# Vi-Sri/CerebralSignalNetworks

Measured on AMD Instinct MI355X. Metric: EEG-segments/sec training (128ch x 500, hidden=768), higher is better.
Workload: dtype bf16

## Files before the change

### cerebralsignalnetworks_amd/cabi.py

```python
import ctypes
import os

import torch

_HERE = os.path.dirname(os.path.abspath(__file__))
LIB_PATH = os.environ.get("CSN_LIB_PATH") or os.path.join(_HERE, "lib", "libcsn_hip.so")

CSN_F32, CSN_BF16 = 0, 1
STATUS_TIMEOUT, STATUS_NONFINITE, STATUS_STALE_SLOT = 1, 2, 4
ABI_VERSION = 6
LSTM_STATE = 0x100
GRAD_OVERWRITE, GRAD_ACCUMULATE = 0, 1

_c_void_p, _c_int, _c_i64, _c_size_t, _c_float = (ctypes.c_void_p, ctypes.c_int, ctypes.c_int64,
                                                  ctypes.c_size_t, ctypes.c_float)


class LstmDesc(ctypes.Structure):
    _fields_ = [("B", ctypes.c_int32), ("T", ctypes.c_int32), ("I", ctypes.c_int32),
                ("H", ctypes.c_int32), ("L", ctypes.c_int32), ("dtype", ctypes.c_int32)]


SIGNATURES = {
    "csn_abi_version": (_c_int, []),
    "csn_last_error": (ctypes.c_char_p, []),
    "csn_target_arch": (ctypes.c_char_p, []),
    "csn_eeg_bandpass_znorm": (_c_int, [_c_void_p, _c_int, _c_int, _c_int, ctypes.POINTER(ctypes.c_double), _c_int,
                                        _c_int, _c_void_p, _c_int, _c_int, _c_void_p]),
    "csn_eeg_filtfilt_scratch_bytes": (_c_size_t, [_c_int, _c_int, _c_int, _c_int]),
    "csn_eeg_filtfilt": (_c_int, [_c_void_p, _c_int, _c_int, _c_int, ctypes.POINTER(ctypes.c_double), _c_int,
                                  _c_void_p, _c_void_p, _c_void_p]),
    "csn_lstm_plan_create": (_c_int, [ctypes.POINTER(LstmDesc), _c_int, ctypes.POINTER(_c_void_p)]),
    "csn_lstm_plan_destroy": (None, [_c_void_p]),
    "csn_lstm_plan_workspace_bytes": (_c_size_t, [_c_void_p]),
    "csn_lstm_plan_path": (_c_int, [_c_void_p]),
    "csn_lstm_plan_dgates_copies": (_c_int, [_c_void_p]),
    "csn_lstm_plan_kernel_name": (ctypes.c_char_p, [_c_void_p, _c_int]),
    "csn_lstm_plan_set_grad_callback": (_c_int, [_c_void_p, _c_void_p, _c_void_p]),
    "csn_lstm_plan_set_grad_mode": (_c_int, [_c_void_p, _c_int]),
    "csn_lstm_plan_set_lengths": (_c_int, [_c_void_p, ctypes.POINTER(ctypes.c_int32)]),
    "csn_lstm_workspace_bytes": (_c_size_t, [ctypes.POINTER(LstmDesc), _c_int]),
    "csn_lstm_forward": (_c_int, [_c_void_p, _c_void_p, _c_i64, _c_i64,
                                  ctypes.POINTER(_c_void_p), ctypes.POINTER(_c_void_p),
                                  ctypes.POINTER(_c_void_p), ctypes.POINTER(_c_void_p),
                                  _c_void_p, _c_void_p,
                                  _c_void_p, _c_void_p, _c_void_p,
                                  _c_void_p, _c_void_p, _c_void_p]),
    "csn_lstm_backward": (_c_int, [_c_void_p, _c_void_p, _c_void_p,
                                   _c_void_p, _c_void_p,
                                   _c_void_p,
                                   ctypes.POINTER(_c_void_p), ctypes.POINTER(_c_void_p),
                                   ctypes.POINTER(_c_void_p), ctypes.POINTER(_c_void_p),
                                   _c_void_p, _c_void_p, _c_void_p, _c_void_p]),
    "csn_lstm_workspace_init": (_c_int, [_c_void_p, _c_void_p, _c_void_p]),
    "csn_lstm_status_clear": (_c_int, [_c_void_p, _c_void_p, _c_void_p]),
    "csn_lstm_status_read": (_c_int, [_c_void_p, _c_void_p, ctypes.POINTER(_c_int)]),
    "csn_lstm_status_raise": (_c_int, [_c_void_p, _c_void_p, _c_void_p]),
    "csn_lstm_profile_enable": (_c_int, [_c_void_p, _c_int]),
    "csn_lstm_profile_read": (_c_int, [_c_void_p, ctypes.POINTER(ctypes.c_double), ctypes.POINTER(_c_int),
                                       ctypes.POINTER(_c_int), ctypes.POINTER(ctypes.c_double), ctypes.POINTER(_c_int),
                                       ctypes.POINTER(_c_int)]),
    "csn_gemm_nt": (_c_int, [_c_void_p, _c_void_p, _c_void_p, _c_void_p, _c_i64, _c_i64, _c_i64,
                             _c_int, _c_int, _c_int, _c_void_p]),
    "csn_gemm_tn_scratch_bytes": (_c_size_t, [_c_i64, _c_i64, _c_i64]),
    "csn_gemm_tn": (_c_int, [_c_void_p, _c_void_p, _c_void_p, _c_i64, _c_i64, _c_i64, _c_int, _c_void_p, _c_void_p]),
    "csn_lstm_cell_forward": (_c_int, [_c_void_p, _c_void_p, _c_void_p, _c_i64, _c_void_p, _c_void_p, _c_void_p,
                                       _c_void_p, _c_int, _c_int, _c_int, _c_void_p]),
    "csn_lstm_cell_backward": (_c_int, [_c_void_p, _c_void_p, _c_void_p, _c_i64, _c_void_p, _c_void_p, _c_void_p,
                                        _c_void_p, _c_void_p, _c_int, _c_int, _c_int, _c_void_p]),
    "csn_cosine_loss_scratch_bytes": (_c_size_t, [_c_int]),
    "csn_cosine_loss": (_c_int, [_c_void_p, _c_void_p, _c_int, _c_int, _c_void_p, _c_void_p, _c_float, _c_void_p, _c_void_p]),
    "csn_rmsprop_step": (_c_int, [_c_void_p, _c_void_p, _c_void_p, _c_i64, _c_float, _c_float, _c_float, _c_void_p]),
    "csn_barlow_offdiag_sqsum": (_c_int, [_c_void_p, _c_int, _c_void_p, _c_void_p]),
    "csn_l2_topk_scratch_bytes": (_c_size_t, [_c_i64, _c_i64]),
    "csn_l2_topk": (_c_int, [_c_void_p, _c_void_p, _c_i64, _c_i64, _c_int, _c_int, _c_void_p, _c_void_p,
                             _c_void_p, _c_void_p]),
}


GRAD_READY_FN = ctypes.CFUNCTYPE(None, ctypes.c_void_p, ctypes.c_int)


class CsnError(RuntimeError):
    pass


_lib = None


def load():
    global _lib
    if _lib is not None:
        return _lib
    if not os.path.exists(LIB_PATH):
        raise CsnError(f"{LIB_PATH} not found: build it with `python -c 'import __graft_entry__ as g; g.build()'` "
                       "(there is no CPU fallback)")
    lib = ctypes.CDLL(LIB_PATH, mode=ctypes.RTLD_LOCAL)
    for name, (res, args) in SIGNATURES.items():
        fn = getattr(lib, name)
        fn.restype, fn.argtypes = res, args
    if lib.csn_abi_version() != ABI_VERSION:
        raise CsnError(f"libcsn_hip.so ABI {lib.csn_abi_version()} != binding ABI {ABI_VERSION}")
    _lib = lib
    return lib


def _check(rc):
    if rc != 0:
        raise CsnError(f"libcsn_hip status {rc}: {load().csn_last_error().decode()}")


def _ptr(t):
    return None if t is None else ctypes.c_void_p(t.data_ptr())


def _stream():
    return ctypes.c_void_p(torch.cuda.current_stream().cuda_stream)


def _dt(dtype):
    if dtype in (torch.float32, "f32", "float32", CSN_F32):
        return CSN_F32
    if dtype in (torch.bfloat16, "bf16", "bfloat16", CSN_BF16):
        return CSN_BF16
    raise CsnError(f"unsupported dtype {dtype}")


def torch_dtype(code):
    return torch.bfloat16 if code == CSN_BF16 else torch.float32


def _need_cuda(*ts):
    for t in ts:
        if t is not None and not t.is_cuda:
            raise CsnError("libcsn_hip needs device tensors (no CPU fallback)")


def eeg_bandpass_znorm(x_bct, sos, ddof=0, out_dtype=torch.float32, time_major=False):
    import numpy as np
    _need_cuda(x_bct)
    x = x_bct.contiguous()
    if x.dtype != torch.float32:
        raise CsnError("eeg_bandpass_znorm expects float32 input")
    B, C, T = x.shape
    sos = np.ascontiguousarray(np.asarray(sos, dtype=np.float64).reshape(-1, 6)) if sos is not None else np.zeros((0, 6))
    y = torch.empty((T, B, C) if time_major else (B, T, C), dtype=out_dtype, device=x.device)
    with torch.cuda.device(x.device):
        _check(load().csn_eeg_bandpass_znorm(_ptr(x), B, C, T, sos.ctypes.data_as(ctypes.POINTER(ctypes.c_double)),
                                             sos.shape[0], int(ddof), _ptr(y), _dt(out_dtype), int(time_major), _stream()))
    return y


def eeg_filtfilt(x_stc, sos):
    import numpy as np
    _need_cuda(x_stc)
    x = x_stc.float().contiguous()
    S, T, C = x.shape
    sos = np.ascontiguousarray(np.asarray(sos, dtype=np.float64).reshape(-1, 6))
    lib = load()
    scratch = torch.empty(max(1, lib.csn_eeg_filtfilt_scratch_bytes(S, T, C, sos.shape[0])), dtype=torch.uint8,
                          device=x.device)
    y = torch.empty_like(x)
    with torch.cuda.device(x.device):
        _check(lib.csn_eeg_filtfilt(_ptr(x), S, T, C, sos.ctypes.data_as(ctypes.POINTER(ctypes.c_double)), sos.shape[0],
                                    _ptr(y), _ptr(scratch), _stream()))
    return y


def gemm_nt(a, bt, bias=None, out_dtype=torch.float32, out=None, accumulate=False):
    _need_cuda(a, bt)
    a, bt = a.contiguous(), bt.contiguous()
    M, K = a.shape
    N = bt.shape[0]
    assert bt.shape[1] == K and a.dtype == bt.dtype
    c = out if out is not None else torch.empty((M, N), dtype=out_dtype, device=a.device)
    _check(load().csn_gemm_nt(_ptr(a), _ptr(bt), _ptr(bias), _ptr(c), M, N, K, _dt(a.dtype), _dt(c.dtype),
                              int(accumulate), _stream()))
    return c


def gemm_tn(a_km, b_kn):
    _need_cuda(a_km, b_kn)
    a, b = a_km.contiguous(), b_kn.contiguous()
    K, M = a.shape
    N = b.shape[1]
    assert b.shape[0] == K and a.dtype == b.dtype
    lib = load()
    scratch = torch.empty(max(1, lib.csn_gemm_tn_scratch_bytes(M, N, K)), dtype=torch.uint8, device=a.device)
    c = torch.empty((M, N), dtype=torch.float32, device=a.device)
    _check(lib.csn_gemm_tn(_ptr(a), _ptr(b), _ptr(c), M, N, K, _dt(a.dtype), _ptr(scratch), _stream()))
    return c


def lstm_cell_forward(h_prev, w_hh, xproj, c_prev, want_gates=True):
    _need_cuda(w_hh, xproj)
    B, G = xproj.shape
    H = G // 4
    dt = w_hh.dtype
    gates = torch.empty((B, G), dtype=dt, device=xproj.device) if want_gates else None
    c_out = torch.empty((B, H), dtype=torch.float32, device=xproj.device)
    h_out = torch.empty((B, H), dtype=dt, device=xproj.device)
    _check(load().csn_lstm_cell_forward(_ptr(h_prev), _ptr(w_hh), _ptr(xproj), G, _ptr(c_prev), _ptr(gates),
                                        _ptr(c_out), _ptr(h_out), B, H, _dt(dt), _stream()))
    return h_out, c_out, gates


def lstm_cell_backward(dgates_next, w_hh_t, dy, gates, c, c_prev, dc_carry):
    _need_cuda(gates, c, dc_carry)
    B, G = gates.shape
    H = G // 4
    out = torch.empty_like(gates)
    _check(load().csn_lstm_cell_backward(_ptr(dgates_next), _ptr(w_hh_t), _ptr(dy), H, _ptr(gates), _ptr(c),
                                         _ptr(c_prev), _ptr(dc_carry), _ptr(out), B, H, _dt(gates.dtype), _stream()))
    return out


def _ptr_array(tensors):
    arr = (ctypes.c_void_p * len(tensors))()
    for i, t in enumerate(tensors):
        arr[i] = t.data_ptr()
    return arr


class LstmPlan:

    def __init__(self, B, T, I, H, L, dtype, device, training=True, state=False):
        self.desc = LstmDesc(B, T, I, H, L, _dt(dtype))
        self.training = bool(training)
        self.state = bool(state)
        self.device = torch.device(device)
        lib = load()
        handle = _c_void_p()
        with torch.cuda.device(self.device):
            _check(lib.csn_lstm_plan_create(ctypes.byref(self.desc), int(self.training) | (LSTM_STATE if self.state else 0),
                                            ctypes.byref(handle)))
        self._plan = handle
        nbytes = lib.csn_lstm_plan_workspace_bytes(self._plan)
        self.workspace = torch.empty(nbytes + 256, dtype=torch.uint8, device=self.device)
        off = (-self.workspace.data_ptr()) % 256
        self._ws_ptr = ctypes.c_void_p(self.workspace.data_ptr() + off)
        self.busy = False
        with torch.cuda.device(self.device):
            _check(lib.csn_lstm_workspace_init(self._plan, self._ws_ptr, _stream()))

    def __del__(self):
        plan, self._plan = getattr(self, "_plan", None), None
        if plan and _lib is not None:
            _lib.csn_lstm_plan_destroy(plan)

    def key(self):
        d = self.desc
        return (d.B, d.T, d.I, d.H, d.L, d.dtype, self.training) + ((True,) if self.state else ())

    def path(self):
        return load().csn_lstm_plan_path(self._plan)

    def kernel_names(self):
        lib = load()
        return tuple((lib.csn_lstm_plan_kernel_name(self._plan, k) or b"").decode() for k in (0, 1))

    def set_grad_callback(self, fn):
        if getattr(self, "_grad_cb_fn", None) is fn and (fn is None or getattr(self, "_grad_cb", None) is not None):
            return
        self._grad_cb_fn = fn
        self._grad_cb = GRAD_READY_FN(lambda _user, layer: fn(int(layer))) if fn is not None else None
        _check(load().csn_lstm_plan_set_grad_callback(self._plan, ctypes.cast(self._grad_cb, _c_void_p) if fn is not None
                                                      else None, None))

    def set_grad_mode(self, accumulate):
        _check(load().csn_lstm_plan_set_grad_mode(self._plan, GRAD_ACCUMULATE if accumulate else GRAD_OVERWRITE))

    def set_lengths(self, lengths):
        if lengths is None:
            _check(load().csn_lstm_plan_set_lengths(self._plan, None))
            return
        vals = [int(v) for v in (lengths.tolist() if isinstance(lengths, torch.Tensor) else lengths)]
        if len(vals) != self.desc.B:
            raise CsnError(f"LSTM lengths: {len(vals)} entries for a batch of {self.desc.B}")
        _check(load().csn_lstm_plan_set_lengths(self._plan, (ctypes.c_int32 * len(vals))(*vals)))

    def dgates_copies(self):
        return load().csn_lstm_plan_dgates_copies(self._plan)

    def forward(self, x_bti, w_ih, w_hh, b_ih, b_hh, want_all=False, h0=None, c0=None, want_state=False):
        d = self.desc
        _need_cuda(x_bti)
        if x_bti.dtype != torch.float32 or x_bti.stride(2) != 1:
            x_bti = x_bti.float().contiguous()
        assert x_bti.shape == (d.B, d.T, d.I), (tuple(x_bti.shape), (d.B, d.T, d.I))
        y_last = torch.empty((d.B, d.H), dtype=torch.float32, device=x_bti.device)
        y_all = torch.empty((d.B, d.T, d.H), dtype=torch.float32, device=x_bti.device) if want_all else None
        ws = [[p.detach() for p in group] for group in (w_ih, w_hh, b_ih, b_hh)]
        for group in ws:
            for p in group:
                assert p.dtype == torch.float32 and p.is_contiguous() and p.is_cuda
        h0, c0 = self._state_in(h0), self._state_in(c0)
        h_n = torch.empty((d.L, d.B, d.H), dtype=torch.float32, device=x_bti.device) if want_state else None
        c_n = torch.empty((d.L, d.B, d.H), dtype=torch.float32, device=x_bti.device) if want_state else None
        with torch.cuda.device(self.device):
            _check(load().csn_lstm_forward(self._plan, _ptr(x_bti), x_bti.stride(0), x_bti.stride(1),
                                           _ptr_array(ws[0]), _ptr_array(ws[1]), _ptr_array(ws[2]), _ptr_array(ws[3]),
                                           _ptr(h0), _ptr(c0), self._ws_ptr, _ptr(y_last), _ptr(y_all),
                                           _ptr(h_n), _ptr(c_n), _stream()))
        if want_state:
            return y_last, y_all, h_n, c_n
        return y_last, y_all

    def _state_in(self, t):
        if t is None:
            return None
        d = self.desc
        t = t.detach()
        if tuple(t.shape) != (d.L, d.B, d.H):
            raise CsnError(f"LSTM state must be [L, B, H] = {[d.L, d.B, d.H]}, got {list(t.shape)}")
        return t.to(device=self.device, dtype=torch.float32).contiguous()

    def backward(self, dy_last, dy_all, grads, dx=None, dh_n=None, dc_n=None, dh0=None, dc0=None):
        if dy_last is not None:
            dy_last = dy_last.float().contiguous()
        if dy_all is not None:
            dy_all = dy_all.float().contiguous()
        dh_n, dc_n = self._state_in(dh_n), self._state_in(dc_n)
        for out in (dh0, dc0):
            if out is not None:
                assert out.dtype == torch.float32 and out.is_contiguous() and out.shape == (self.desc.L, self.desc.B,
                                                                                            self.desc.H)
        with torch.cuda.device(self.device):
            _check(load().csn_lstm_backward(self._plan, _ptr(dy_last), _ptr(dy_all), _ptr(dh_n), _ptr(dc_n), self._ws_ptr,
                                            _ptr_array(grads[0]), _ptr_array(grads[1]), _ptr_array(grads[2]),
                                            _ptr_array(grads[3]), _ptr(dx), _ptr(dh0), _ptr(dc0), _stream()))

    def clear_status(self):
        with torch.cuda.device(self.device):
            _check(load().csn_lstm_status_clear(self._plan, self._ws_ptr, _stream()))

    def inject_timeout(self):
        with torch.cuda.device(self.device):
            _check(load().csn_lstm_status_raise(self._plan, self._ws_ptr, _stream()))

    def status(self, clear=False):
        out = _c_int(0)
        _check(load().csn_lstm_status_read(self._plan, self._ws_ptr, ctypes.byref(out)))
        if clear and out.value != 0:
            self.clear_status()
        return out.value

    def profile_enable(self, on=True):
        _check(load().csn_lstm_profile_enable(self._plan, int(on)))

    def profile_read(self):
        fm, bm = ctypes.c_double(), ctypes.c_double()
        fl, fc, bl, bc = _c_int(), _c_int(), _c_int(), _c_int()
        _check(load().csn_lstm_profile_read(self._plan, ctypes.byref(fm), ctypes.byref(fl), ctypes.byref(fc),
                                            ctypes.byref(bm), ctypes.byref(bl), ctypes.byref(bc)))
        return dict(fwd_ms=fm.value, fwd_launches=fl.value, fwd_cells=fc.value,
                    bwd_ms=bm.value, bwd_launches=bl.value, bwd_cells=bc.value)


def cosine_loss(student, teacher, want_grad=True, grad_scale=1.0):
    _need_cuda(student, teacher)
    s, t = student.float().contiguous(), teacher.float().contiguous()
    B, D = s.shape
    loss = torch.empty(1, dtype=torch.float32, device=s.device)
    ds = torch.empty_like(s) if want_grad else None
    lib = load()
    scratch = torch.empty(lib.csn_cosine_loss_scratch_bytes(B) // 8, dtype=torch.float64, device=s.device)
    with torch.cuda.device(s.device):
        _check(lib.csn_cosine_loss(_ptr(s), _ptr(t), B, D, _ptr(loss), _ptr(ds), float(grad_scale), _ptr(scratch), _stream()))
    return loss, ds


def rmsprop_step(params_flat, grads_flat, square_avg_flat, lr, alpha=0.99, eps=1e-8):
    _need_cuda(params_flat, grads_flat, square_avg_flat)
    n = params_flat.numel()
    assert grads_flat.numel() == n and square_avg_flat.numel() == n
    assert params_flat.dtype == grads_flat.dtype == square_avg_flat.dtype == torch.float32
    with torch.cuda.device(params_flat.device):
        _check(load().csn_rmsprop_step(_ptr(params_flat), _ptr(grads_flat), _ptr(square_avg_flat), n, float(lr), float(alpha),
                                       float(eps), _stream()))


def barlow_offdiag_sqsum(c):
    _need_cuda(c)
    if c.dim() != 2 or c.shape[0] != c.shape[1]:
        raise CsnError(f"barlow_offdiag_sqsum expects a square matrix, got shape {tuple(c.shape)}")
    c = c.float().contiguous()
    out = torch.empty(2, dtype=torch.float32, device=c.device)
    with torch.cuda.device(c.device):
        _check(load().csn_barlow_offdiag_sqsum(_ptr(c), c.shape[0], _ptr(out), _stream()))
    return out


def l2_topk(gallery, query, k):
    _need_cuda(gallery, query)
    g, q = gallery.float().contiguous(), query.float().contiguous()
    Ng, D = g.shape
    Nq = q.shape[0]
    lib = load()
    scratch = torch.empty(lib.csn_l2_topk_scratch_bytes(Ng, Nq), dtype=torch.uint8, device=g.device)
    idx = torch.empty((Nq, k), dtype=torch.int64, device=g.device)
    dist = torch.empty((Nq, k), dtype=torch.float32, device=g.device)
    _check(lib.csn_l2_topk(_ptr(g), _ptr(q), Ng, Nq, D, k, _ptr(idx), _ptr(dist), _ptr(scratch), _stream()))
    return dist, idx
```

### cerebralsignalnetworks_amd/csrc/csn_common.h

```cpp
#pragma once
#include <hip/hip_runtime.h>
#include <stdint.h>
#include <stdio.h>
#include <stdlib.h>
#include <atomic>
#include <string>

#include "../../include/csn_hip.h"

namespace csn {

typedef __bf16 bf16_t;
typedef __attribute__((ext_vector_type(8))) __bf16 bf16x8;
typedef __attribute__((ext_vector_type(4))) __bf16 bf16x4;
typedef __attribute__((ext_vector_type(4))) float f32x4;
typedef __attribute__((ext_vector_type(4))) short s16x4;

void set_error(const std::string& msg);
int fail(int status, const char* fmt, ...);

#define CSN_HIP_CHECK(expr)                                                              \
  do {                                                                                   \
    hipError_t _e = (expr);                                                              \
    if (_e != hipSuccess)                                                                \
      return ::csn::fail(CSN_ERR_HIP, "%s failed: %s (%s:%d)", #expr, hipGetErrorString(_e), \
                         __FILE__, __LINE__);                                            \
  } while (0)

#define CSN_LAUNCH_CHECK()                                                               \
  do {                                                                                   \
    hipError_t _e = hipGetLastError();                                                   \
    if (_e != hipSuccess)                                                                \
      return ::csn::fail(CSN_ERR_HIP, "kernel launch failed: %s (%s:%d)",                \
                         hipGetErrorString(_e), __FILE__, __LINE__);                     \
  } while (0)

#define CSN_REQUIRE(cond, ...)                                                           \
  do {                                                                                   \
    if (!(cond)) return ::csn::fail(CSN_ERR_INVALID_ARGUMENT, __VA_ARGS__);              \
  } while (0)

struct Options {
  bool cell_v1, no_persist, no_persist_bwd, persist_streams, no_xcd_local, no_rotate, no_fuse_x, no_beside,
      no_side_stream, gemm_slot, fwd_ksplit, fwd_nsplit, fwd_flags, bwd_flags, dpoll_no_hint, fwd_hint, gemm_no_dma, gemm_no_256, gemm_generic, gemm_lds64, tn_no_tr, tn_no_stagger, filter_v1, tags_no_rearm, gemm_no_192;
  int chunk;
  int tn_stages;
  int fwd_nk;
};
static inline Options options_from_env() {
  auto on = [](const char* name) { return getenv(name) != nullptr; };
  auto num = [](const char* name, int dflt) {
    const char* e = getenv(name);
    return e ? atoi(e) : dflt;
  };
  Options o{};
  o.cell_v1 = on("CSN_CELL_V1");
  o.no_persist = on("CSN_NO_PERSIST");
  o.no_persist_bwd = on("CSN_NO_PERSIST_BWD");
  o.persist_streams = on("CSN_PERSIST_STREAMS");
  o.no_xcd_local = on("CSN_NO_XCD_LOCAL");
  o.no_rotate = on("CSN_NO_ROTATE");
  o.no_fuse_x = on("CSN_NO_FUSE_X");
  o.no_beside = on("CSN_NO_BESIDE");
  o.no_side_stream = on("CSN_NO_SIDE_STREAM");
  o.gemm_slot = on("CSN_GEMM_SLOT");
  o.fwd_ksplit = on("CSN_FWD_KSPLIT");
  o.fwd_nsplit = on("CSN_FWD_NSPLIT");
  o.fwd_flags = on("CSN_FWD_FLAGS");
  o.bwd_flags = on("CSN_BWD_FLAGS");
  o.dpoll_no_hint = on("CSN_DPOLL_NO_HINT");
  o.fwd_hint = on("CSN_FWD_HINT");
  o.tn_no_stagger = on("CSN_TN_NO_STAGGER");
  o.gemm_no_dma = on("CSN_GEMM_NO_DMA");
  o.gemm_no_256 = on("CSN_GEMM_NO_256");
  o.gemm_no_192 = on("CSN_GEMM_NO_192");
  o.gemm_generic = on("CSN_GEMM_GENERIC");
  o.gemm_lds64 = on("CSN_GEMM_LDS64");
  o.tn_no_tr = on("CSN_TN_NO_TR");
  o.filter_v1 = on("CSN_FILTER_V1");
#ifdef CSN_SLAB_TAGS
  o.tags_no_rearm = on("CSN_TAGS_NO_REARM");
#endif
  o.chunk = num("CSN_LSTM_CHUNK", 32);
  if (o.chunk < 1) o.chunk = 1;
  o.tn_stages = num("CSN_TN_STAGES", 4);
  o.fwd_nk = num("CSN_FWD_NK", 1);
  return o;
}

static inline hipStream_t as_stream(csnStream_t s) { return reinterpret_cast<hipStream_t>(s); }
template <auto Kernel>
static int ensure_dyn_lds(int bytes) {
  static std::atomic<unsigned> done{0u};
  int dev = 0;
  CSN_HIP_CHECK(hipGetDevice(&dev));
  const unsigned bit = 1u << (dev & 31);
  if ((done.load(std::memory_order_acquire) & bit) == 0u) {
    CSN_HIP_CHECK(hipFuncSetAttribute(reinterpret_cast<const void*>(Kernel), hipFuncAttributeMaxDynamicSharedMemorySize, bytes));
    done.fetch_or(bit, std::memory_order_release);
  }
  return CSN_OK;
}

static inline size_t align_up(size_t v, size_t a) { return (v + a - 1) / a * a; }
static inline size_t dtype_size(int dtype) { return dtype == CSN_BF16 ? 2 : 4; }

__device__ __forceinline__ float to_f32(float v) { return v; }
__device__ __forceinline__ float to_f32(bf16_t v) { return (float)v; }
template <typename T> __device__ __forceinline__ T from_f32(float v);
template <> __device__ __forceinline__ float from_f32<float>(float v) { return v; }
template <> __device__ __forceinline__ bf16_t from_f32<bf16_t>(float v) { return (bf16_t)v; }

__device__ __forceinline__ float sigmoid_f32(float x) { return 1.0f / (1.0f + expf(-x)); }
__device__ __forceinline__ float tanh_f32(float x) { return tanhf(x); }

struct CellFwdOne {
  const void* h_prev; const void* w_hh; const float* xproj; int64_t xproj_ld; const float* c_prev;
  void* gates_out; float* c_out; void* h_out;
};
struct CellFwdBatch { CellFwdOne p[4]; };
struct CellBwdOne {
  const void* dg_next; const void* w_hh_t; const float* dy; int64_t dy_ld; const void* gates; const float* c;
  const float* c_prev; float* dc_carry; void* dg_out;
};
struct CellBwdBatch { CellBwdOne p[4]; };
struct CellMask {
  const int* lengths;
  int t[4];
};
struct CellNoMask {};
template <bool MASK> struct CellMaskArg { typedef CellNoMask type; };
template <> struct CellMaskArg<true> { typedef CellMask type; };
int launch_cell_fwd_batch(const CellFwdBatch& b, int np, int B, int H, int dtype, hipStream_t st);
int launch_cell_bwd_batch(const CellBwdBatch& b, int np, int B, int H, int dtype, hipStream_t st,
                          const CellMask* mask = nullptr);

int launch_cast_strided(const float* src, int64_t s0, int64_t s1, int64_t n0, int64_t n1, int64_t n2,
                        void* dst, int dtype, hipStream_t st);
int launch_transpose_cast(const float* src, int64_t R, int64_t C, void* dst, int dtype, hipStream_t st);
int launch_cast(const float* src, void* dst, int64_t n, int dtype, hipStream_t st);
int launch_upcast(const void* src, int dtype, float* dst, int64_t n, hipStream_t st);
int launch_add_vec(const float* a, const float* b, float* out, int64_t n, hipStream_t st);
int launch_reduce_slabs(const float* slabs, int64_t stride, int S, float* out, float* out2, int64_t n, int accumulate,
                        hipStream_t st);
size_t colsum_scratch_bytes(int64_t N);
int launch_colsum(const void* X, int64_t R, int64_t N, int dtype, float* out, float* out2, int accumulate, void* scratch,
                  hipStream_t st);
int colsum_chunks();
int launch_colsum_partial(const void* X, int64_t R, int64_t N, int dtype, void* scratch, hipStream_t st);
int launch_gemm_nt_beside(const void* A, const void* Bt, const float* bias, float* C, int64_t M, int64_t N, int64_t K,
                          int max_wgs, hipStream_t st);
int launch_gemm_tn_slabs(const void* A, const void* B, float* slabs, int64_t M, int64_t N, int64_t K, int dtype,
                         hipStream_t st, int* S_out, float* colsum, int* colsum_done, const Options& opt);
int gemm_nt(const void* A, const void* Bt, const float* bias, void* C, int64_t M, int64_t N, int64_t K, int dtype,
            int out_dtype, int accumulate, hipStream_t st, const Options& opt);
size_t gemm_tn_scratch_bytes(int64_t M, int64_t N, int64_t K, const Options& opt);

}
```

### cerebralsignalnetworks_amd/csrc/lstm.hip

```cpp
#include <algorithm>
#include <cstring>
#include <vector>

#include "csn_common.h"
#include "lstm_cell_blk.h"
#include "lstm_cell_common.h"
#include "lstm_f32_persist.h"

namespace csn {

int launch_cell_fwd(const void* h_prev, const void* w_hh, const float* xproj, int64_t xproj_ld, const float* c_prev,
                    void* gates_out, float* c_out, void* h_out, int B, int H, int dtype, hipStream_t st);
int launch_cell_bwd(const void* dg_next, const void* w_hh_t, const float* dy, int64_t dy_ld, const void* gates,
                    const float* c, const float* c_prev, float* dc_carry, void* dg_out, int B, int H, int dtype,
                    hipStream_t st);

struct LayerWs {
  size_t wih, whh, whht, wiht, whh_blk, whht_blk, bias, xproj, gates, c_all, h_all, dgates, dx, dc_carry, hblk[2],
      dgblk[2], h_blk_all, counters, dg_blk_all, bflags;
};
struct WsLayout {
  LayerWs layer[8];
  size_t x_c, x_blk, wih0_blk, dy_tm, tn_scratch, colsum, status, agree, agree_b, zeros_bh, f32_bias_part, total;
  size_t zero_fwd, zero_fwd_bytes, zero_bwd, zero_bwd_bytes;
  bool fuse_x;
  bool il, persist, persist_bwd;
  bool fwd_ns;
  bool f32_persist;
};

static bool whole_chip() {
  int dev = 0, cus = 0;
  if (hipGetDevice(&dev) != hipSuccess) return false;
  return hipDeviceGetAttribute(&cus, hipDeviceAttributeMultiprocessorCount, dev) == hipSuccess && cus >= 256;
}

static WsLayout make_layout(const csnLstmDesc& d, int training, const Options& opt) {
  WsLayout w{};
  w.il = cell_blk_supported(d.H, d.dtype, opt);
  const bool slabs_fit = ((size_t)d.T + 1) * (((size_t)d.B + 63) / 64 * 64) * (size_t)d.H * 8 < ((size_t)1 << 32);
  w.fwd_ns = w.il && fwd_ns_supported(d.B, d.H, d.dtype, opt) && d.L <= 4;
  w.persist = w.fwd_ns || (w.il && slabs_fit && fwd_persist_supported(d.B, d.H, d.dtype, opt) && d.L <= 4);
  w.persist_bwd = w.persist && slabs_fit && training && bwd_persist_supported(d.B, d.H, d.dtype, opt);
  size_t off = 0;
  const size_t es = dtype_size(d.dtype);
  auto take = [&](size_t bytes) {
    size_t o = off;
    off += align_up(bytes, 256);
    return o;
  };
  const size_t TB = (size_t)d.T * d.B, H = d.H, G = 4 * (size_t)d.H;
  const size_t Bpad = ((size_t)d.B + 63) / 64 * 64;
  size_t tn_bytes = 0;
  for (int l = 0; l < d.L; ++l) {
    const size_t I = l == 0 ? d.I : d.H;
    LayerWs& L = w.layer[l];
    L.wih = take(G * I * es);
    L.wiht = take(G * I * es);
    L.bias = take(G * 4);
    if (w.il) {
      L.whh_blk = take(G * H * 2);
      L.whht_blk = take(G * H * 2);
      L.hblk[0] = take(Bpad * H * 2);
      L.hblk[1] = take(Bpad * H * 2);
      if (w.persist) L.h_blk_all = take(((size_t)(d.T < 3 ? 3 : d.T) + 1) * Bpad * H * 2);
    } else {
      L.whh = take(G * H * es);
      L.whht = take(G * H * es);
    }
    L.xproj = take(TB * G * 4);
    L.gates = take(TB * G * es);
    L.c_all = take((TB + d.B) * H * 4);
    L.h_all = take((TB + d.B) * H * es);
    if (training) {
      L.dgates = take(TB * G * es);
      L.dx = take(TB * I * 4);
      if (!w.persist_bwd) L.dc_carry = take((size_t)d.B * H * 4);
      if (w.il) {
        L.dgblk[0] = take(Bpad * G * 2);
        L.dgblk[1] = take(Bpad * G * 2);
      }
      if (w.persist_bwd) L.dg_blk_all = take((size_t)(d.T < 4 ? 4 : d.T) * Bpad * G * 2);
    }
    size_t a = gemm_tn_scratch_bytes(G, I, TB, opt), b = gemm_tn_scratch_bytes(G, H, TB, opt);
    if (a > tn_bytes) tn_bytes = a;
    if (b > tn_bytes) tn_bytes = b;
  }
  w.x_c = take(TB * d.I * es);
  w.status = take(256);
  w.fuse_x = w.persist && !opt.no_fuse_x &&
             (w.fwd_ns ? d.I == 128 : (d.I % 32 == 0 && d.I <= 128 && d.H != 512));
  if (w.fuse_x) {
    w.x_blk = take((size_t)d.T * Bpad * d.I * 2);
    w.wih0_blk = take(G * d.I * 2);
  }
  if (w.persist_bwd) w.zeros_bh = take((size_t)d.B * H * 4);
  w.f32_persist = !w.il && d.dtype == CSN_F32 && !opt.no_persist && !opt.cell_v1 && f32_persist_supported(d.B, d.H) && whole_chip();
  if (w.f32_persist) {
    const size_t MTt = Bpad / 64;
    w.zero_fwd = off;
    for (int l = 0; l < d.L; ++l) w.layer[l].counters = take(((size_t)d.T + 1) * MTt * kF32FlagLine * 4);
    w.zero_fwd_bytes = off - w.zero_fwd;
    for (int l = 0; l < d.L; ++l) w.layer[l].h_blk_all = take(((size_t)d.T + 1) * Bpad * H * 4);
    if (training) {
      for (int l = 0; l < d.L; ++l) w.layer[l].dg_blk_all = take((size_t)d.T * Bpad * G * 4);
      w.zeros_bh = take((size_t)d.B * H * 4);
      w.f32_bias_part = take(MTt * 4 * G * 4);
      w.zero_bwd = off;
      for (int l = 0; l < d.L; ++l) w.layer[l].bflags = take((size_t)d.T * MTt * kF32FlagLine * 4);
      w.zero_bwd_bytes = off - w.zero_bwd;
    }
  }
  if (w.persist) {
    w.zero_fwd = off;
    for (int l = 0; l < d.L; ++l) w.layer[l].counters = take(((size_t)d.T + 1) * (Bpad / 64) * 4 * kPersistFlagLine * 4);
    w.agree = take(((size_t)d.T + 8) * 8 * sizeof(unsigned long long));
    w.zero_fwd_bytes = off - w.zero_fwd;
  }
  if (w.persist_bwd) {
    w.zero_bwd = off;
    for (int l = 0; l < d.L; ++l) {
      w.layer[l].dc_carry = take((size_t)d.B * H * 4);
      w.layer[l].bflags = take((size_t)d.T * (Bpad / 64) * kPersistFlagLine * 4);
    }
    w.agree_b = take(((size_t)d.T + 8) * 8 * sizeof(unsigned long long));
    w.zero_bwd_bytes = off - w.zero_bwd;
  }
  if (training) {
    w.dy_tm = take(TB * H * 4);
    w.tn_scratch = take(tn_bytes);
    w.colsum = take(colsum_scratch_bytes(G));
  }
  w.total = off;
  return w;
}

static int check_desc(const char* fn, const csnLstmDesc* d) {
  CSN_REQUIRE(d != nullptr, "%s: null descriptor", fn);
  CSN_REQUIRE(d->B > 0 && d->T > 0 && d->I > 0 && d->H > 0, "%s: bad shape B=%d T=%d I=%d H=%d", fn, d->B, d->T,
              d->I, d->H);
  CSN_REQUIRE(d->L >= 1 && d->L <= 8, "%s: L=%d outside 1..8", fn, d->L);
  CSN_REQUIRE(d->H % 32 == 0, "%s: H=%d must be a multiple of 32", fn, d->H);
  CSN_REQUIRE(d->dtype == CSN_F32 || d->dtype == CSN_BF16, "%s: bad dtype %d", fn, d->dtype);
  return CSN_OK;
}

template <typename T>
__global__ void gather_y_all_kernel(const T* __restrict__ h_all, float* __restrict__ y, int B, int Tn, int H) {
  const int64_t total = (int64_t)B * Tn * H;
  const int64_t stride = (int64_t)gridDim.x * blockDim.x;
  for (int64_t i = (int64_t)blockIdx.x * blockDim.x + threadIdx.x; i < total; i += stride) {
    const int64_t h = i % H, r = i / H, t = r % Tn, b = r / Tn;
    y[i] = to_f32(h_all[((t + 1) * B + b) * (int64_t)H + h]);
  }
}

__global__ void bt_to_tb_kernel(const float* __restrict__ src, float* __restrict__ dst, int B, int Tn, int H) {
  const int64_t total = (int64_t)B * Tn * H;
  const int64_t stride = (int64_t)gridDim.x * blockDim.x;
  for (int64_t i = (int64_t)blockIdx.x * blockDim.x + threadIdx.x; i < total; i += stride) {
    const int64_t h = i % H, r = i / H, b = r % B, t = r / B;
    dst[i] = src[(b * Tn + t) * (int64_t)H + h];
  }
}

__global__ void tb_to_bt_kernel(const float* __restrict__ src, float* __restrict__ dst, int B, int Tn, int H) {
  const int64_t total = (int64_t)B * Tn * H;
  const int64_t stride = (int64_t)gridDim.x * blockDim.x;
  for (int64_t i = (int64_t)blockIdx.x * blockDim.x + threadIdx.x; i < total; i += stride) {
    const int64_t h = i % H, r = i / H, t = r % Tn, b = r / Tn;
    dst[i] = src[(t * B + b) * (int64_t)H + h];
  }
}

__global__ void add_rows_kernel(const float* __restrict__ src, float* __restrict__ dst, int64_t n) {
  const int64_t stride = (int64_t)gridDim.x * blockDim.x;
  for (int64_t i = (int64_t)blockIdx.x * blockDim.x + threadIdx.x; i < n; i += stride) dst[i] += src[i];
}

template <typename T>
__global__ void mask_tm_kernel(T* __restrict__ buf, const int* __restrict__ len, int B, int Tn, int W) {
  const int64_t total = (int64_t)B * Tn * W;
  const int64_t stride = (int64_t)gridDim.x * blockDim.x;
  for (int64_t i = (int64_t)blockIdx.x * blockDim.x + threadIdx.x; i < total; i += stride) {
    const int64_t r = i / W, b = r % B, t = r / B;
    if (t >= len[b]) buf[i] = from_f32<T>(0.f);
  }
}
__global__ void mask_x_blk_kernel(bf16_t* __restrict__ x_blk, const int* __restrict__ len, int B, int64_t Bpad, int Tn, int I) {
  const int64_t per_t = Bpad * I / 8, kblocks = I >> 5;
  const int64_t stride = (int64_t)gridDim.x * blockDim.x;
  for (int64_t ci = (int64_t)blockIdx.x * blockDim.x + threadIdx.x; ci < per_t * Tn; ci += stride) {
    const int64_t t = ci / per_t, c = ci % per_t, blk = c >> 6, lane = c & 63;
    const int64_t r = (blk / kblocks) * 16 + (lane & 15);
    if (r < B && t >= len[r]) *reinterpret_cast<uint4*>(x_blk + ci * 8) = make_uint4(0u, 0u, 0u, 0u);
  }
}
template <typename T>
__global__ void gather_state_kernel(const T* __restrict__ all, const int* __restrict__ len, float* __restrict__ out, int B, int H) {
  const int64_t total = (int64_t)B * H;
  const int64_t stride = (int64_t)gridDim.x * blockDim.x;
  for (int64_t i = (int64_t)blockIdx.x * blockDim.x + threadIdx.x; i < total; i += stride) {
    const int64_t b = i / H;
    out[i] = to_f32(all[(int64_t)len[b] * B * H + i]);
  }
}
template <typename T>
__global__ void gather_y_all_len_kernel(const T* __restrict__ h_all, float* __restrict__ y, const int* __restrict__ len, int B, int Tn, int H) {
  const int64_t total = (int64_t)B * Tn * H;
  const int64_t stride = (int64_t)gridDim.x * blockDim.x;
  for (int64_t i = (int64_t)blockIdx.x * blockDim.x + threadIdx.x; i < total; i += stride) {
    const int64_t h = i % H, r = i / H, t = r % Tn, b = r / Tn;
    y[i] = t < len[b] ? to_f32(h_all[((t + 1) * B + b) * (int64_t)H + h]) : 0.f;
  }
}
__global__ void bt_to_tb_len_kernel(const float* __restrict__ src, float* __restrict__ dst, const int* __restrict__ len, int B, int Tn, int Te, int H) {
  const int64_t total = (int64_t)B * Te * H;
  const int64_t stride = (int64_t)gridDim.x * blockDim.x;
  for (int64_t i = (int64_t)blockIdx.x * blockDim.x + threadIdx.x; i < total; i += stride) {
    const int64_t h = i % H, r = i / H, b = r % B, t = r / B;
    dst[i] = (src != nullptr && t < len[b]) ? src[(b * Tn + t) * (int64_t)H + h] : 0.f;
  }
}
__global__ void add_at_end_kernel(const float* __restrict__ src, float* __restrict__ dst_tm, const int* __restrict__ len, int t_lo, int t_hi, int B, int H) {
  const int64_t total = (int64_t)B * H;
  const int64_t stride = (int64_t)gridDim.x * blockDim.x;
  for (int64_t i = (int64_t)blockIdx.x * blockDim.x + threadIdx.x; i < total; i += stride) {
    const int t = len[i / H] - 1;
    if (t >= t_lo && t <= t_hi) dst_tm[(int64_t)t * B * H + i] += src[i];
  }
}
__global__ void add_rows_len0_kernel(const float* __restrict__ src, float* __restrict__ dst, const int* __restrict__ len, int B, int H) {
  const int64_t total = (int64_t)B * H;
  const int64_t stride = (int64_t)gridDim.x * blockDim.x;
  for (int64_t i = (int64_t)blockIdx.x * blockDim.x + threadIdx.x; i < total; i += stride)
    if (len[i / H] == 0) dst[i] += src[i];
}
__global__ void tb_to_bt_len_kernel(const float* __restrict__ src, float* __restrict__ dst, int B, int Tn, int Te, int H) {
  const int64_t total = (int64_t)B * Tn * H;
  const int64_t stride = (int64_t)gridDim.x * blockDim.x;
  for (int64_t i = (int64_t)blockIdx.x * blockDim.x + threadIdx.x; i < total; i += stride) {
    const int64_t h = i % H, r = i / H, t = r % Tn, b = r / Tn;
    dst[i] = t < Te ? src[(t * B + b) * (int64_t)H + h] : 0.f;
  }
}

template <typename T, bool BLK>
__global__ void __launch_bounds__(256) lstm_dh0_kernel(const T* __restrict__ dg, const T* __restrict__ wt, int B, int H,
                                                       float* __restrict__ out) {
  __shared__ float As[32][33];
  __shared__ float Ws[32][65];
  const int64_t G = 4 * (int64_t)H;
  const int tx = threadIdx.x & 15, ty = threadIdx.x >> 4;
  const int b0 = blockIdx.y * 32, j0 = blockIdx.x * 64;
  float acc[2][4] = {{0.f, 0.f, 0.f, 0.f}, {0.f, 0.f, 0.f, 0.f}};
  for (int64_t k0 = 0; k0 < G; k0 += 32) {
    for (int i = threadIdx.x; i < 32 * 32; i += 256) {
      const int r = i >> 5, k = i & 31;
      As[r][k] = b0 + r < B ? to_f32(dg[(int64_t)(b0 + r) * G + k0 + k]) : 0.f;
    }
    for (int i = threadIdx.x; i < 64 * 32; i += 256) {
      const int j = i >> 5, k = i & 31;
      float v = 0.f;
      if (j0 + j < H) v = to_f32(wt[BLK ? blk_offset(j0 + j, k0 + k, G) : (int64_t)(j0 + j) * G + k0 + k]);
      Ws[k][j] = v;
    }
    __syncthreads();
#pragma unroll 8
    for (int k = 0; k < 32; ++k) {
      const float a0 = As[ty][k], a1 = As[ty + 16][k];
#pragma unroll
      for (int c = 0; c < 4; ++c) {
        const float wv = Ws[k][tx + 16 * c];
        acc[0][c] = fmaf(a0, wv, acc[0][c]);
        acc[1][c] = fmaf(a1, wv, acc[1][c]);
      }
    }
    __syncthreads();
  }
#pragma unroll
  for (int r = 0; r < 2; ++r)
#pragma unroll
    for (int c = 0; c < 4; ++c) {
      const int b = b0 + ty + 16 * r, j = j0 + tx + 16 * c;
      if (b < B && j < H) out[(int64_t)b * H + j] = acc[r][c];
    }
}

__global__ void sum_rows_kernel(const float* __restrict__ part, int P, int64_t n, float* out, float* out2, int accumulate) {
  const int64_t i = (int64_t)blockIdx.x * blockDim.x + threadIdx.x;
  if (i >= n) return;
  float s = 0.f;
  for (int p = 0; p < P; ++p) s += part[(int64_t)p * n + i];
  out[i] = accumulate ? out[i] + s : s;
  out2[i] = accumulate ? out2[i] + s : s;
}

static inline unsigned grid_for(int64_t n) {
  int64_t g = (n + 255) / 256;
  return (unsigned)(g < 1 ? 1 : (g > 2048 ? 2048 : g));
}

struct SideCtx {
  hipStream_t side = nullptr;
  hipStream_t layer[8] = {nullptr};
  std::vector<hipEvent_t> events;
  size_t next = 0;
};

static int side_ctx(SideCtx& c) {
  if (c.side == nullptr) {
    CSN_HIP_CHECK(hipStreamCreateWithFlags(&c.side, hipStreamNonBlocking));
    for (int l = 1; l < 8; ++l) CSN_HIP_CHECK(hipStreamCreateWithFlags(&c.layer[l], hipStreamNonBlocking));
  }
  c.next = 0;
  return CSN_OK;
}
static int next_event(SideCtx* c, hipEvent_t* ev) {
  if (c->next == c->events.size()) {
    hipEvent_t e;
    CSN_HIP_CHECK(hipEventCreateWithFlags(&e, hipEventDisableTiming));
    c->events.push_back(e);
  }
  *ev = c->events[c->next++];
  return CSN_OK;
}
static int hand_off(SideCtx* c, hipStream_t from, hipStream_t to) {
  hipEvent_t ev;
  if (int rc = next_event(c, &ev)) return rc;
  CSN_HIP_CHECK(hipEventRecord(ev, from));
  CSN_HIP_CHECK(hipStreamWaitEvent(to, ev, 0));
  return CSN_OK;
}

struct Prof {
  bool on = false;
  hipEvent_t ev[4] = {nullptr, nullptr, nullptr, nullptr};
  int launches[2] = {0, 0}, cells[2] = {0, 0};
  bool have[2] = {false, false};
  std::vector<hipEvent_t> pair[2];
  size_t pairs_used[2] = {0, 0};
};
static int prof_mark(Prof& g_prof, int which, hipStream_t st) {
  if (!g_prof.on) return CSN_OK;
  if ((which & 1) == 0) g_prof.pairs_used[which >> 1] = 0;
  if (g_prof.ev[which] == nullptr) CSN_HIP_CHECK(hipEventCreate(&g_prof.ev[which]));
  CSN_HIP_CHECK(hipEventRecord(g_prof.ev[which], st));
  return CSN_OK;
}

static int prof_pair(Prof& g_prof, int k, bool end, hipStream_t st) {
  if (!g_prof.on) return CSN_OK;
  const size_t i = 2 * g_prof.pairs_used[k] + (end ? 1 : 0);
  while (g_prof.pair[k].size() <= i) {
    hipEvent_t e;
    CSN_HIP_CHECK(hipEventCreate(&e));
    g_prof.pair[k].push_back(e);
  }
  CSN_HIP_CHECK(hipEventRecord(g_prof.pair[k][i], st));
  if (end) ++g_prof.pairs_used[k];
  return CSN_OK;
}

}

struct csnLstmPlan {
  csnLstmDesc d;
  int training;
  int state;
  bool state_seen = false;
  int device;
  csn::Options opt;
  csn::WsLayout w;
  csn::SideCtx sc;
  csn::Prof prof;
  int dgates_copies = 0;
  csnGradReadyFn grad_cb = nullptr;
  void* grad_cb_user = nullptr;
  int grad_accumulate = 0;
  std::vector<int32_t> lengths;
  int t_eff = 0;
  int T_full = 0;
  const int* dlen = nullptr;
  int32_t* len_dev = nullptr;
  int32_t* len_pin = nullptr;
  hipEvent_t len_ev = nullptr;
  void grads_ready(int layer) const {
    if (grad_cb != nullptr) grad_cb(grad_cb_user, layer);
  }
};

using namespace csn;
typedef csnLstmPlan Plan;

extern "C" int csn_lstm_plan_create(const csnLstmDesc* d, int training, csnLstmPlan** out) {
  if (int rc = check_desc("csn_lstm_plan_create", d)) return rc;
  CSN_REQUIRE(out != nullptr, "csn_lstm_plan_create: null output pointer");
  Plan* P = new Plan();
  P->d = *d;
  P->state = (training & CSN_LSTM_STATE) != 0;
  P->training = (training & ~CSN_LSTM_STATE) != 0;
  if (hipGetDevice(&P->device) != hipSuccess) {
    delete P;
    return fail(CSN_ERR_HIP, "csn_lstm_plan_create: hipGetDevice failed");
  }
  P->opt = options_from_env();
  if (P->state && d->dtype == CSN_F32) P->opt.no_persist = true;
  {
    const unsigned long long Bp = ((unsigned long long)d->B + 63) / 64 * 64;
    const unsigned long long per_step = std::max({(unsigned long long)d->B * d->H * 16ull, Bp * (unsigned long long)d->I * 2ull, Bp * (unsigned long long)d->H * 2ull});
    const unsigned long long cmax = ((1ull << 32) - 1ull) / per_step;
    if (cmax >= 3 && (unsigned long long)P->opt.chunk > cmax - 2) P->opt.chunk = (int)(cmax - 2);
  }
  P->w = make_layout(*d, P->training, P->opt);
  P->T_full = d->T;
  *out = P;
  return CSN_OK;
}

extern "C" void csn_lstm_plan_destroy(csnLstmPlan* P) {
  if (P == nullptr) return;
  int cur = 0;
  const bool switched = hipGetDevice(&cur) == hipSuccess && cur != P->device && hipSetDevice(P->device) == hipSuccess;
  for (hipEvent_t e : P->sc.events) (void)hipEventDestroy(e);
  if (P->sc.side) (void)hipStreamDestroy(P->sc.side);
  for (int l = 1; l < 8; ++l)
    if (P->sc.layer[l]) (void)hipStreamDestroy(P->sc.layer[l]);
  for (int i = 0; i < 4; ++i)
    if (P->prof.ev[i]) (void)hipEventDestroy(P->prof.ev[i]);
  for (int k = 0; k < 2; ++k)
    for (hipEvent_t e : P->prof.pair[k]) (void)hipEventDestroy(e);
  if (P->len_ev) (void)hipEventDestroy(P->len_ev);
  if (P->len_pin) (void)hipHostFree(P->len_pin);
  if (P->len_dev) (void)hipFree(P->len_dev);
  if (switched) (void)hipSetDevice(cur);
  delete P;
}

extern "C" size_t csn_lstm_plan_workspace_bytes(const csnLstmPlan* P) { return P ? P->w.total : 0; }

extern "C" int csn_lstm_plan_path(const csnLstmPlan* P) {
  if (P == nullptr) return -1;
  return P->w.f32_persist ? 4 : (P->w.persist_bwd ? 3 : (P->w.persist ? 2 : (P->w.il ? 1 : 0)));
}

extern "C" int csn_lstm_plan_dgates_copies(const csnLstmPlan* P) { return P == nullptr ? -1 : P->dgates_copies; }

static bool bwd_grouped(const csnLstmPlan* P) {
  if (!P->w.persist_bwd) return false;
  const int MTg = (P->d.B + 63) / 64, nchg = (P->d.T + P->opt.chunk - 1) / P->opt.chunk;
  const int slots = P->d.L < nchg ? P->d.L : nchg;
  return slots <= 4 && slots * MTg <= 8 && !P->opt.persist_streams;
}

extern "C" const char* csn_lstm_plan_kernel_name(const csnLstmPlan* P, int which) {
  if (P == nullptr) return nullptr;
  const bool ks = (P->d.dtype == CSN_F32 ? P->d.H % 128 == 0 : P->d.H % 256 == 0);
  if (P->w.f32_persist) return which == 0 ? "lstm_fwd_f32_persist_kernel" : (which == 1 ? "lstm_bwd_f32_persist_kernel" : nullptr);
  if (which == 0) {
    if (P->w.fwd_ns) return "lstm_fwd_ns_kernel";
    if (P->w.persist) return "lstm_fwd_persist_kernel";
    if (P->w.il) return "lstm_cell_fwd_il_kernel";
    return ks ? "lstm_cell_fwd_ks_kernel" : "lstm_cell_fwd_kernel";
  }
  if (which == 1) {
    if (bwd_grouped(P)) return "lstm_bwd_persist_kernel";
    if (P->w.il) return "lstm_cell_bwd_il_kernel";
    return ks ? "lstm_cell_bwd_ks_kernel" : "lstm_cell_bwd_kernel";
  }
  return nullptr;
}

extern "C" int csn_lstm_plan_set_grad_callback(csnLstmPlan* P, csnGradReadyFn fn, void* user) {
  CSN_REQUIRE(P != nullptr, "csn_lstm_plan_set_grad_callback: null plan");
  P->grad_cb = fn;
  P->grad_cb_user = fn ? user : nullptr;
  return CSN_OK;
}

extern "C" int csn_lstm_plan_set_grad_mode(csnLstmPlan* P, int mode) {
  CSN_REQUIRE(P != nullptr, "csn_lstm_plan_set_grad_mode: null plan");
  CSN_REQUIRE(mode == CSN_GRAD_OVERWRITE || mode == CSN_GRAD_ACCUMULATE, "csn_lstm_plan_set_grad_mode: unknown mode %d", mode);
  P->grad_accumulate = mode == CSN_GRAD_ACCUMULATE;
  return CSN_OK;
}

extern "C" int csn_lstm_plan_set_lengths(csnLstmPlan* P, const int32_t* lengths) {
  CSN_REQUIRE(P != nullptr, "csn_lstm_plan_set_lengths: null plan");
  CSN_REQUIRE(P->state, "csn_lstm_plan_set_lengths: the plan was created without CSN_LSTM_STATE");
  if (lengths == nullptr) {
    P->lengths.clear();
    P->t_eff = 0;
    return CSN_OK;
  }
  int longest = 0;
  for (int b = 0; b < P->d.B; ++b) {
    CSN_REQUIRE(lengths[b] >= 0 && lengths[b] <= P->d.T, "csn_lstm_plan_set_lengths: lengths[%d] = %d outside [0, %d]", b,
                (int)lengths[b], P->d.T);
    longest = std::max(longest, (int)lengths[b]);
  }
  P->lengths.assign(lengths, lengths + P->d.B);
  P->t_eff = longest;
  return CSN_OK;
}

struct EffectiveT {
  csnLstmDesc& d;
  const int T;
  EffectiveT(csnLstmDesc& d_, int Te) : d(d_), T(d_.T) { d.T = Te; }
  ~EffectiveT() { d.T = T; }
};
static int upload_lengths(csnLstmPlan* P, hipStream_t st) {
  P->dlen = nullptr;
  if (P->lengths.empty()) return CSN_OK;
  const size_t bytes = (size_t)P->d.B * 4;
  if (P->len_pin == nullptr) {
    CSN_HIP_CHECK(hipMalloc((void**)&P->len_dev, bytes));
    CSN_HIP_CHECK(hipHostMalloc((void**)&P->len_pin, bytes, hipHostMallocDefault));
    CSN_HIP_CHECK(hipEventCreateWithFlags(&P->len_ev, hipEventDisableTiming));
  } else {
    CSN_HIP_CHECK(hipEventSynchronize(P->len_ev));
  }
  memcpy(P->len_pin, P->lengths.data(), bytes);
  CSN_HIP_CHECK(hipMemcpyAsync(P->len_dev, P->len_pin, bytes, hipMemcpyHostToDevice, st));
  CSN_HIP_CHECK(hipEventRecord(P->len_ev, st));
  P->dlen = P->len_dev;
  return CSN_OK;
}
static int emit_dx(const csnLstmPlan& P, const float* dx_tm, float* dx, int64_t I, hipStream_t st) {
  const int B = P.d.B, T = P.d.T;
  if (P.dlen != nullptr) tb_to_bt_len_kernel<<<csn::grid_for((int64_t)P.T_full * B * I), 256, 0, st>>>(dx_tm, dx, B, P.T_full, T, (int)I);
  else csn::tb_to_bt_kernel<<<csn::grid_for((int64_t)T * B * I), 256, 0, st>>>(dx_tm, dx, B, T, (int)I);
  CSN_LAUNCH_CHECK();
  return CSN_OK;
}
static int add_dh_n_rows(const csnLstmPlan& P, const float* dh_below, float* dx_tm, int t_lo, int t_hi, hipStream_t st) {
  const int B = P.d.B, H = P.d.H, T = P.d.T;
  if (P.dlen != nullptr) {
    add_at_end_kernel<<<csn::grid_for((int64_t)B * H), 256, 0, st>>>(dh_below, dx_tm, P.dlen, t_lo, t_hi, B, H);
  } else {
    if (t_hi != T - 1) return CSN_OK;
    csn::add_rows_kernel<<<csn::grid_for((int64_t)B * H), 256, 0, st>>>(dh_below, dx_tm + (size_t)(T - 1) * B * H, (int64_t)B * H);
  }
  CSN_LAUNCH_CHECK();
  return CSN_OK;
}

extern "C" int csn_lstm_profile_enable(csnLstmPlan* P, int on) {
  CSN_REQUIRE(P != nullptr, "csn_lstm_profile_enable: null plan");
  P->prof.on = on != 0;
  P->prof.have[0] = P->prof.have[1] = false;
  return CSN_OK;
}

extern "C" int csn_lstm_profile_read(csnLstmPlan* P, double* fwd_ms, int* fwd_launches, int* fwd_cells, double* bwd_ms,
                                     int* bwd_launches, int* bwd_cells) {
  CSN_REQUIRE(P && fwd_ms && fwd_launches && fwd_cells && bwd_ms && bwd_launches && bwd_cells,
              "csn_lstm_profile_read: null pointer");
  Prof& g_prof = P->prof;
  *fwd_ms = *bwd_ms = 0.0;
  *fwd_launches = *fwd_cells = *bwd_launches = *bwd_cells = 0;
  for (int k = 0; k < 2; ++k) {
    if (!g_prof.have[k]) continue;
    float ms = 0.f;
    CSN_HIP_CHECK(hipEventSynchronize(g_prof.ev[2 * k + 1]));
    if (g_prof.pairs_used[k] > 0) {
      for (size_t i = 0; i < g_prof.pairs_used[k]; ++i) {
        float one = 0.f;
        CSN_HIP_CHECK(hipEventElapsedTime(&one, g_prof.pair[k][2 * i], g_prof.pair[k][2 * i + 1]));
        ms += one;
      }
    } else {
      CSN_HIP_CHECK(hipEventElapsedTime(&ms, g_prof.ev[2 * k], g_prof.ev[2 * k + 1]));
    }
    (k == 0 ? *fwd_ms : *bwd_ms) = ms;
    (k == 0 ? *fwd_launches : *bwd_launches) = g_prof.launches[k];
    (k == 0 ? *fwd_cells : *bwd_cells) = g_prof.cells[k];
  }
  return CSN_OK;
}

extern "C" int csn_lstm_workspace_init(const csnLstmPlan* P, void* workspace, csnStream_t stream) {
  CSN_REQUIRE(P && workspace, "csn_lstm_workspace_init: null pointer");
  CSN_REQUIRE((reinterpret_cast<uintptr_t>(workspace) & 255) == 0, "csn_lstm_workspace_init: workspace must be 256-B aligned");
  hipStream_t st = as_stream(stream);
  char* ws = (char*)workspace;
  const WsLayout& w = P->w;
  const size_t es = dtype_size(P->d.dtype);
  CSN_HIP_CHECK(hipMemsetAsync(ws + w.status, 0, 256, st));
  for (int l = 0; l < P->d.L; ++l) {
    CSN_HIP_CHECK(hipMemsetAsync(ws + w.layer[l].h_all, 0, (size_t)P->d.B * P->d.H * es, st));
    CSN_HIP_CHECK(hipMemsetAsync(ws + w.layer[l].c_all, 0, (size_t)P->d.B * P->d.H * 4, st));
  }
  if (w.persist_bwd || (w.f32_persist && P->training))
    CSN_HIP_CHECK(hipMemsetAsync(ws + w.zeros_bh, 0, (size_t)P->d.B * P->d.H * 4, st));
  return CSN_OK;
}

extern "C" int csn_lstm_status_clear(const csnLstmPlan* P, void* workspace, csnStream_t stream) {
// ... 363 lines not shown
      CSN_HIP_CHECK(hipMemsetAsync(ws + L.c_all, 0, (size_t)B * H * 4, st));
      if (h0) {
        if ((rc = launch_blockify_x(h0 + (size_t)l * B * H, H, 0, B, 1, H, ws + L.hblk[0], st))) return rc;
        if ((rc = launch_cast(h0 + (size_t)l * B * H, ws + L.h_all, (int64_t)B * H, CSN_BF16, st))) return rc;
      }
      if (c0)
        CSN_HIP_CHECK(hipMemcpyAsync(ws + L.c_all, c0 + (size_t)l * B * H, (size_t)B * H * 4, hipMemcpyDeviceToDevice, st));
    }
  }
  if (w.fuse_x) {
    job(kPrepBlockifyX, x, nullptr, ws + w.x_blk, B, T, d->I, xsb, xst, (int64_t)Bpad, 0, 0, (int64_t)T * Bpad * d->I / 8);
    job(kPrepBlockify, w_ih[0], nullptr, ws + w.wih0_blk, G, d->I, 0, d->I, 1, H, 1, 0, G * d->I / 8);
  }
  if (prep_rc != CSN_OK) return prep_rc;
  if ((rc = launch_prep_multi(pa, st))) return rc;
  if ((rc = mask_x(P, ws, st))) return rc;
  if (!w.fuse_x) {
    if ((rc = gemm_nt(ws + w.x_c, ws + w.layer[0].wih, (const float*)(ws + w.layer[0].bias), ws + w.layer[0].xproj,
                          TB, G, d->I, CSN_BF16, CSN_F32, 0, st, P.opt)))
      return rc;
  }
  if (w.persist) return forward_persist(P, ws, h0, c0, training, st, sc, side);
  if (NL > 1 && (rc = hand_off(sc, st, side))) return rc;

  const int nch = (T + Cz - 1) / Cz;
  std::vector<hipEvent_t> xproj_ready((size_t)NL * nch, nullptr);
  const int D = T + lag * (NL - 1);
  int n_launch = 0, n_cells = 0;
  if ((rc = prof_mark(g_prof, 0, st))) return rc;
  for (int dg = 0; dg < D; ++dg) {
    CellFwdArgs a{};
    a.B = B;
    a.H = H;
    int np = 0;
    for (int l = 0; l < NL; ++l) {
      const int t = dg - lag * l;
      if (t < 0 || t >= T) continue;
      const LayerWs& L = w.layer[l];
      if (np == 4) {
        if ((rc = launch_cell_fwd_il(a, np, st, P.opt.fwd_nk))) return rc;
        ++n_launch;
        n_cells += np;
        np = 0;
      }
      if (l > 0 && t % Cz == 0) CSN_HIP_CHECK(hipStreamWaitEvent(st, xproj_ready[(size_t)l * nch + t / Cz], 0));
      CellFwdProb& P = a.p[np++];
      P.h_prev_blk = (t == 0 && !h0) ? nullptr : (const bf16_t*)(ws + L.hblk[t & 1]);
      P.w_blk = (const bf16_t*)(ws + L.whh_blk);
      P.xproj = (const float*)(ws + L.xproj) + (size_t)t * B * G;
      P.c_prev = (t == 0 && !c0) ? nullptr : (const float*)(ws + L.c_all) + (size_t)t * B * H;
      P.gates_out = training ? (bf16_t*)(ws + L.gates) + (size_t)t * B * G : nullptr;
      P.c_out = (float*)(ws + L.c_all) + (size_t)(t + 1) * B * H;
      P.h_out = (bf16_t*)(ws + L.h_all) + (size_t)(t + 1) * B * H;
      P.h_out_blk = (bf16_t*)(ws + L.hblk[(t + 1) & 1]);
    }
    if (np == 0) continue;
    if ((rc = launch_cell_fwd_il(a, np, st, P.opt.fwd_nk))) return rc;
    ++n_launch;
    n_cells += np;
    for (int l = 0; l + 1 < NL; ++l) {
      const int t = dg - lag * l;
      if (t < 0 || t >= T) continue;
      if ((t + 1) % Cz != 0 && t != T - 1) continue;
      const int c = t / Cz, t0 = c * Cz, nsteps = t - t0 + 1;
      if ((rc = hand_off(sc, st, side))) return rc;
      const LayerWs& Ln = w.layer[l + 1];
      rc = gemm_nt((const bf16_t*)(ws + w.layer[l].h_all) + (size_t)(t0 + 1) * B * H, ws + Ln.wih,
                       (const float*)(ws + Ln.bias), (float*)(ws + Ln.xproj) + (size_t)t0 * B * G,
                       (int64_t)nsteps * B, G, H, CSN_BF16, CSN_F32, 0, side, P.opt);
      if (rc) return rc;
      hipEvent_t ev;
      if ((rc = next_event(sc, &ev))) return rc;
      CSN_HIP_CHECK(hipEventRecord(ev, side));
      xproj_ready[(size_t)(l + 1) * nch + c] = ev;
    }
  }
  if ((rc = prof_mark(g_prof, 1, st))) return rc;
  g_prof.launches[0] = n_launch;
  g_prof.cells[0] = n_cells;
  g_prof.have[0] = g_prof.on;
  return CSN_OK;
}

static int forward_persist(Plan& P, char* ws, const float* h0, const float* c0, int training, hipStream_t st, SideCtx* sc,
                           hipStream_t side) {
  const csnLstmDesc* d = &P.d;
  const WsLayout& w = P.w;
  Prof& g_prof = P.prof;
  const int B = d->B, T = d->T, H = d->H, NL = d->L;
  const int64_t G = 4 * (int64_t)H;
  const int Bpad = (B + 63) / 64 * 64, MT = Bpad / 64;
  const int Cz = P.opt.chunk;
  const int nch = (T + Cz - 1) / Cz;
  int rc;
  CSN_HIP_CHECK(hipMemsetAsync(ws + w.zero_fwd, 0, w.zero_fwd_bytes, st));
  auto fill_slot = [&](PersistFwdSlot& S, int l, int c) {
    const LayerWs& L = w.layer[l];
    S.w_blk = (const bf16_t*)(ws + L.whh_blk);
    S.xproj = (const float*)(ws + L.xproj);
    S.gates = training ? (bf16_t*)(ws + L.gates) : nullptr;
    S.c_all = (float*)(ws + L.c_all);
    S.h_all = (bf16_t*)(ws + L.h_all);
    S.h_blk_all = (bf16_t*)(ws + L.h_blk_all);
    S.flags = (unsigned*)(ws + L.counters);
    S.x_blk = nullptr;
    S.wih_blk = nullptr;
    S.bias = nullptr;
    S.I = 0;
    if (l == 0 && w.fuse_x) {
      S.x_blk = (const bf16_t*)(ws + w.x_blk);
      S.wih_blk = (const bf16_t*)(ws + w.wih0_blk);
      S.bias = (const float*)(ws + L.bias);
      S.I = d->I;
    }
    S.t0 = c * Cz;
    S.nsteps = (S.t0 + Cz <= T) ? Cz : T - S.t0;
  };
  auto xproj_gemm = [&](int l, int c, hipStream_t on) {
    const LayerWs& L = w.layer[l];
    const LayerWs& Ln = w.layer[l + 1];
    const int t0 = c * Cz, nsteps = (t0 + Cz <= T) ? Cz : T - t0;
    return gemm_nt((const bf16_t*)(ws + L.h_all) + (size_t)(t0 + 1) * B * H, ws + Ln.wih,
                       (const float*)(ws + Ln.bias), (float*)(ws + Ln.xproj) + (size_t)t0 * B * G,
                       (int64_t)nsteps * B, G, H, CSN_BF16, CSN_F32, 0, on, P.opt);
  };
  PersistFwdArgs a{};
  a.error_flag = (unsigned*)(ws + w.status);
  a.B = B; a.H = H; a.T = T; a.Bpad = Bpad; a.MT = MT;
  a.rotate = !P.opt.no_rotate;
  a.data_polls = (!w.fwd_ns && !P.opt.fwd_flags) ? (P.opt.fwd_hint && !P.opt.dpoll_no_hint ? 1 : 2) : 0;
#ifdef CSN_SLAB_TAGS
  if (a.data_polls && P.opt.tags_no_rearm) a.data_polls |= 4;
#endif
  if (a.data_polls)
    for (int l = 0; l < NL; ++l)
      CSN_HIP_CHECK(hipMemsetAsync(ws + w.layer[l].h_blk_all, 0xff, (size_t)4 * Bpad * H * 2, st));
  a.state = (h0 || c0) ? 1 : 0;
  if (a.state) P.state_seen = true;
  for (int l = 0; l < NL && P.state_seen; ++l) {
    const LayerWs& L = w.layer[l];
    if (h0) {
      if ((rc = launch_blockify_x(h0 + (size_t)l * B * H, H, 0, B, 1, H, ws + L.h_blk_all, st))) return rc;
      if ((rc = launch_cast(h0 + (size_t)l * B * H, ws + L.h_all, (int64_t)B * H, CSN_BF16, st))) return rc;
    } else {
      if (a.state) CSN_HIP_CHECK(hipMemsetAsync(ws + L.h_blk_all, 0, (size_t)Bpad * H * 2, st));
      CSN_HIP_CHECK(hipMemsetAsync(ws + L.h_all, 0, (size_t)B * H * 2, st));
    }
    if (c0)
      CSN_HIP_CHECK(hipMemcpyAsync(ws + L.c_all, c0 + (size_t)l * B * H, (size_t)B * H * 4, hipMemcpyDeviceToDevice, st));
    else
      CSN_HIP_CHECK(hipMemsetAsync(ws + L.c_all, 0, (size_t)B * H * 4, st));
  }
  int n_launch = 0;

  const int max_slots = NL < nch ? NL : nch;
  const int fwd_slices = w.fwd_ns ? fwd_ns_slices(H) : fwd_persist_slices(H);
  auto launch_fwd = [&](const PersistFwdArgs& args, hipStream_t on) {
    return w.fwd_ns ? launch_fwd_ns(args, on) : launch_fwd_persist(args, on);
  };
  const bool grouped = max_slots <= 4 && max_slots * MT <= 8 && fwd_slices <= 32 &&
                       !P.opt.persist_streams;
  if (grouped) {
    const int ndiag = nch + NL - 1;
    const bool try_local = !P.opt.no_xcd_local;
    if ((rc = prof_mark(g_prof, 0, st))) return rc;
    for (int dg = 0; dg < ndiag; ++dg) {
      int lay[4], chk[4], ns = 0;
      for (int l = 0; l < NL; ++l) {
        const int c = dg - l;
        if (c < 0 || c >= nch) continue;
        lay[ns] = l;
        chk[ns] = c;
        fill_slot(a.slot[ns], l, c);
        ++ns;
      }
      a.nslots = ns;
      a.xcd_groups = 1;
      a.agree = try_local ? (unsigned long long*)(ws + w.agree) + (size_t)dg * 8 : nullptr;
      if ((rc = prof_pair(g_prof, 0, false, st))) return rc;
      if ((rc = launch_fwd(a, st))) return rc;
      if ((rc = prof_pair(g_prof, 0, true, st))) return rc;
      ++n_launch;
      for (int i = 0; i < ns; ++i)
        if (lay[i] + 1 < NL && (rc = xproj_gemm(lay[i], chk[i], st))) return rc;
    }
    if ((rc = prof_mark(g_prof, 1, st))) return rc;
    g_prof.launches[0] = n_launch;
    g_prof.cells[0] = T * NL;
    g_prof.have[0] = g_prof.on;
    return CSN_OK;
  }

  if (NL * fwd_slices * MT > 256) side = st;
  hipStream_t ls[8];
  ls[0] = st;
  for (int l = 1; l < NL; ++l) {
    ls[l] = (side == st) ? st : sc->layer[l];
    if (ls[l] != st && (rc = hand_off(sc, st, ls[l]))) return rc;
  }
  if (side != st && (rc = hand_off(sc, st, side))) return rc;
  const bool gemm_slot = P.opt.gemm_slot;
  if ((rc = prof_mark(g_prof, 0, st))) return rc;
  a.nslots = 1;
  a.xcd_groups = 0;
  a.agree = nullptr;
  for (int c = 0; c < nch; ++c) {
    for (int l = 0; l < NL; ++l) {
      fill_slot(a.slot[0], l, c);
      if ((rc = launch_fwd(a, ls[l]))) return rc;
      ++n_launch;
      if (l + 1 < NL) {
        if ((rc = hand_off(sc, ls[l], side))) return rc;
        if ((rc = xproj_gemm(l, c, side))) return rc;
        if (side != ls[l + 1] && (rc = hand_off(sc, side, ls[l + 1]))) return rc;
        if (gemm_slot && side != ls[l] && (rc = hand_off(sc, side, ls[l]))) return rc;
      }
    }
  }
  for (int l = 1; l < NL; ++l)
    if (ls[l] != st && (rc = hand_off(sc, ls[l], st))) return rc;
  if (side != st && (rc = hand_off(sc, side, st))) return rc;
  if ((rc = prof_mark(g_prof, 1, st))) return rc;
  g_prof.launches[0] = n_launch;
  g_prof.cells[0] = T * NL;
  g_prof.have[0] = g_prof.on;
  return CSN_OK;
}

static int backward_persist(Plan& P, char* ws, const float* dy_last, const float* dy_tm, const float* dh_n,
                            const float* dc_n, float* const* dw_ih, float* const* dw_hh, float* const* db_ih,
                            float* const* db_hh, float* dx, hipStream_t st);

static int backward_il(Plan& P, char* ws, const float* dy_last, const float* dy_tm, const float* dh_n, const float* dc_n,
                       float* const* dw_ih, float* const* dw_hh, float* const* db_ih, float* const* db_hh, float* dx,
                       csnStream_t stream) {
  const csnLstmDesc* d = &P.d;
  const WsLayout& w = P.w;
  Prof& g_prof = P.prof;
  hipStream_t st = as_stream(stream);
  if (bwd_grouped(&P)) return backward_persist(P, ws, dy_last, dy_tm, dh_n, dc_n, dw_ih, dw_hh, db_ih, db_hh, dx, st);
  SideCtx* sc = &P.sc;
  int rc;
  if ((rc = side_ctx(P.sc))) return rc;
  hipStream_t side = P.opt.no_side_stream ? st : sc->side;
  const int B = d->B, T = d->T, H = d->H, NL = d->L;
  const int64_t G = 4 * (int64_t)H, TB = (int64_t)T * B;
  const size_t Bpad = ((size_t)B + 63) / 64 * 64;
  const int Cz = P.opt.chunk, lag = 2 * Cz;
  const int nch = (T + Cz - 1) / Cz;
  const bool state = P.state != 0;

  for (int l = 0; l < NL; ++l) {
    const LayerWs& L = w.layer[l];
    if (dc_n)
      CSN_HIP_CHECK(hipMemcpyAsync(ws + L.dc_carry, dc_n + (size_t)l * B * H, (size_t)B * H * 4, hipMemcpyDeviceToDevice, st));
    else
      CSN_HIP_CHECK(hipMemsetAsync(ws + L.dc_carry, 0, (size_t)B * H * 4, st));
    CSN_HIP_CHECK(hipMemsetAsync(ws + L.dgblk[0], 0, Bpad * G * 2, st));
    CSN_HIP_CHECK(hipMemsetAsync(ws + L.dgblk[1], 0, Bpad * G * 2, st));
  }
  if ((rc = hand_off(sc, st, side))) return rc;

  auto weight_grads = [&](int l) -> int {
    const LayerWs& L = w.layer[l];
    const int64_t I = l == 0 ? d->I : H;
    const void* inp = l == 0 ? (const void*)(ws + w.x_c)
                             : (const void*)((const bf16_t*)(ws + w.layer[l - 1].h_all) + (size_t)B * H);
    float* slabs = (float*)(ws + w.tn_scratch);
    const int acc = P.grad_accumulate;
    int S = 1, r;
    int cs_done = 0, S_cs = 1;
    if ((r = launch_gemm_tn_slabs(ws + L.dgates, ws + L.h_all, slabs, G, H, TB, CSN_BF16, side, &S, (float*)(ws + w.colsum), &cs_done, P.opt))) return r;
    S_cs = S;
    if ((r = launch_reduce_slabs_unperm(slabs, G * H, S, H, H, dw_hh[l], nullptr, acc, side))) return r;
    if ((r = launch_gemm_tn_slabs(ws + L.dgates, inp, slabs, G, I, TB, CSN_BF16, side, &S, nullptr, nullptr, P.opt))) return r;
    if ((r = launch_reduce_slabs_unperm(slabs, G * I, S, H, I, dw_ih[l], nullptr, acc, side))) return r;
    if (!cs_done) {
      if ((r = launch_colsum_partial(ws + L.dgates, TB, G, CSN_BF16, ws + w.colsum, side))) return r;
      S_cs = colsum_chunks();
    }
    if ((r = launch_reduce_slabs_unperm((const float*)(ws + w.colsum), G, S_cs, H, 1, db_ih[l], db_hh[l], acc, side)))
      return r;
    return CSN_OK;
  };

  std::vector<hipEvent_t> dx_ready((size_t)NL * nch, nullptr);
  const int D = T + lag * (NL - 1);
  int n_launch = 0, n_cells = 0;
  if ((rc = prof_mark(g_prof, 2, st))) return rc;
  for (int dg = 0; dg < D; ++dg) {
    CellBwdArgs a{};
    a.B = B;
    a.H = H;
    CellMask mask{P.dlen, {0, 0, 0, 0}};
    const CellMask* mk = P.dlen ? &mask : nullptr;
    int np = 0;
    for (int l = NL - 1; l >= 0; --l) {
      const int r = dg - lag * (NL - 1 - l);
      if (r < 0 || r >= T) continue;
      const int t = T - 1 - r;
      const LayerWs& L = w.layer[l];
      const bool top = (l == NL - 1);
      if (np == 4) {
        if ((rc = launch_cell_bwd_il(a, np, st, mk))) return rc;
        ++n_launch;
        n_cells += np;
        np = 0;
      }
      mask.t[np] = t;
      if (!top && r % Cz == 0) CSN_HIP_CHECK(hipStreamWaitEvent(st, dx_ready[(size_t)(l + 1) * nch + r / Cz], 0));
      CellBwdProb& P = a.p[np++];
      P.dg_next_blk = (t == T - 1) ? nullptr : (const bf16_t*)(ws + L.dgblk[(t + 1) & 1]);
      P.wt_blk = (const bf16_t*)(ws + L.whht_blk);
      if (top) {
        P.dy = dy_tm ? dy_tm + (size_t)t * B * H : (t == T - 1 ? dy_last : nullptr);
      } else {
        P.dy = (const float*)(ws + w.layer[l + 1].dx) + (size_t)t * B * H;
      }
      P.dy_ld = H;
      P.gates = (const bf16_t*)(ws + L.gates) + (size_t)t * B * G;
      P.c = (const float*)(ws + L.c_all) + (size_t)(t + 1) * B * H;
      P.c_prev = (t == 0 && !state) ? nullptr : (const float*)(ws + L.c_all) + (size_t)t * B * H;
      P.dc_carry = (float*)(ws + L.dc_carry);
      P.dg_out = (bf16_t*)(ws + L.dgates) + (size_t)t * B * G;
      P.dg_out_blk = (bf16_t*)(ws + L.dgblk[t & 1]);
    }
    if (np == 0) continue;
    if ((rc = launch_cell_bwd_il(a, np, st, mk))) return rc;
    ++n_launch;
    n_cells += np;
    for (int l = NL - 1; l >= 0; --l) {
      const int r = dg - lag * (NL - 1 - l);
      if (r < 0 || r >= T) continue;
      const bool chunk_end = ((r + 1) % Cz == 0) || r == T - 1;
      if (!chunk_end) continue;
      const LayerWs& L = w.layer[l];
      const int64_t I = l == 0 ? d->I : H;
      const int cr = r / Cz;
      const int t_lo = T - 1 - r, t_hi = T - 1 - cr * Cz;
      const bool last = (r == T - 1);
      if (l > 0 || last) {
        if ((rc = hand_off(sc, st, side))) return rc;
      }
      if (l > 0) {
        rc = gemm_nt((const bf16_t*)(ws + L.dgates) + (size_t)t_lo * B * G, ws + L.wiht, nullptr,
                         (float*)(ws + L.dx) + (size_t)t_lo * B * I, (int64_t)(t_hi - t_lo + 1) * B, I, G, CSN_BF16,
                         CSN_F32, 0, side, P.opt);
        if (rc) return rc;
        if (dh_n && (rc = add_dh_n_rows(P, dh_n + (size_t)(l - 1) * B * H, (float*)(ws + L.dx), t_lo, t_hi, side))) return rc;
        hipEvent_t ev;
        if ((rc = next_event(sc, &ev))) return rc;
        CSN_HIP_CHECK(hipEventRecord(ev, side));
        dx_ready[(size_t)l * nch + cr] = ev;
      } else if (last && dx != nullptr) {
        rc = gemm_nt(ws + L.dgates, ws + L.wiht, nullptr, ws + L.dx, TB, I, G, CSN_BF16, CSN_F32, 0,
                         side, P.opt);
        if (rc) return rc;
        if ((rc = emit_dx(P, (const float*)(ws + L.dx), dx, I, side))) return rc;
      }
      if (last && (rc = weight_grads(l))) return rc;
    }
  }
  if ((rc = prof_mark(g_prof, 3, st))) return rc;
  g_prof.launches[1] = n_launch;
  g_prof.cells[1] = n_cells;
  g_prof.have[1] = g_prof.on;
  if ((rc = hand_off(sc, side, st))) return rc;
  for (int l = NL - 1; l >= 0; --l) P.grads_ready(l);
  return CSN_OK;
}

static int backward_persist(Plan& P, char* ws, const float* dy_last, const float* dy_tm, const float* dh_n,
                            const float* dc_n, float* const* dw_ih, float* const* dw_hh, float* const* db_ih,
                            float* const* db_hh, float* dx, hipStream_t st) {
  const csnLstmDesc* d = &P.d;
  const WsLayout& w = P.w;
  Prof& g_prof = P.prof;
  const int B = d->B, T = d->T, H = d->H, NL = d->L;
  const int64_t G = 4 * (int64_t)H, TB = (int64_t)T * B;
  const int Bpad = (B + 63) / 64 * 64, MT = Bpad / 64;
  const int Cz = P.opt.chunk;
  const int nch = (T + Cz - 1) / Cz;
  const bool beside = NL > 1 && NL <= 4 && bwd_persist_slices(H) <= 28 && G % 64 == 0 && !P.opt.no_beside;
  const int lag = beside ? 2 : 1;
  const int ndiag = nch + lag * (NL - 1);
  int rc;
  CSN_HIP_CHECK(hipMemsetAsync(ws + w.zero_bwd, 0, w.zero_bwd_bytes, st));
  if (dc_n)
    for (int l = 0; l < NL; ++l)
      CSN_HIP_CHECK(hipMemcpyAsync(ws + w.layer[l].dc_carry, dc_n + (size_t)l * B * H, (size_t)B * H * 4,
                                   hipMemcpyDeviceToDevice, st));
  struct DhAdd { int l, t_lo, t_hi; };
  auto add_dh_n = [&](const DhAdd& q) -> int {
    return add_dh_n_rows(P, dh_n + (size_t)(q.l - 1) * B * H, (float*)(ws + w.layer[q.l].dx), q.t_lo, q.t_hi, st);
  };
  const bool try_local = !P.opt.no_xcd_local;

  auto weight_grads = [&](int l) -> int {
    const LayerWs& L = w.layer[l];
    const int64_t I = l == 0 ? d->I : H;
    const void* inp = l == 0 ? (const void*)(ws + w.x_c)
                             : (const void*)((const bf16_t*)(ws + w.layer[l - 1].h_all) + (size_t)B * H);
    float* slabs = (float*)(ws + w.tn_scratch);
    const int acc = P.grad_accumulate;
    int S = 1, r;
    int cs_done = 0, S_cs = 1;
    if ((r = launch_gemm_tn_slabs(ws + L.dgates, ws + L.h_all, slabs, G, H, TB, CSN_BF16, st, &S, (float*)(ws + w.colsum), &cs_done, P.opt))) return r;
    S_cs = S;
    if ((r = launch_reduce_slabs_unperm(slabs, G * H, S, H, H, dw_hh[l], nullptr, acc, st))) return r;
    if ((r = launch_gemm_tn_slabs(ws + L.dgates, inp, slabs, G, I, TB, CSN_BF16, st, &S, nullptr, nullptr, P.opt))) return r;
    if ((r = launch_reduce_slabs_unperm(slabs, G * I, S, H, I, dw_ih[l], nullptr, acc, st))) return r;
    if (!cs_done) {
      if ((r = launch_colsum_partial(ws + L.dgates, TB, G, CSN_BF16, ws + w.colsum, st))) return r;
      S_cs = colsum_chunks();
    }
    if ((r = launch_reduce_slabs_unperm((const float*)(ws + w.colsum), G, S_cs, H, 1, db_ih[l], db_hh[l], acc, st))) return r;
    return CSN_OK;
  };
  PersistBwdArgs a{};
  a.error_flag = (unsigned*)(ws + w.status);
  a.B = B; a.H = H; a.T = T; a.Bpad = Bpad; a.MT = MT;
  a.xcd_groups = 1;
  a.grid_slices = 32;
  a.rotate = !P.opt.no_rotate;
  a.data_polls = P.opt.bwd_flags ? 0 : (P.opt.dpoll_no_hint ? 2 : 1);
#ifdef CSN_SLAB_TAGS
  if (a.data_polls && P.opt.tags_no_rearm) a.data_polls |= 4;
#endif
  P.dgates_copies = 2;
  if (a.data_polls)
    for (int l = 0; l < NL; ++l) CSN_HIP_CHECK(hipMemsetAsync(ws + w.layer[l].dg_blk_all, 0xff, (size_t)4 * Bpad * G * 2, st));
  int n_launch = 0;
  BesideGemm pending[3];
  DhAdd pending_add[3] = {{0, 0, 0}, {0, 0, 0}, {0, 0, 0}};
  int npending = 0;
  if ((rc = prof_mark(g_prof, 2, st))) return rc;
  for (int dg = 0; dg < ndiag; ++dg) {
    int lay[4], chk[4], ns = 0;
    for (int l = NL - 1; l >= 0; --l) {
      const int c = dg - lag * (NL - 1 - l);
      if (c < 0 || c >= nch) continue;
      const LayerWs& L = w.layer[l];
      PersistBwdSlot& S = a.slot[ns];
      S.wt_blk = (const bf16_t*)(ws + L.whht_blk);
      S.gates = (const bf16_t*)(ws + L.gates);
      S.c_all = (const float*)(ws + L.c_all);
      if (l == NL - 1) {
        S.dy = dy_tm;
        S.dy_last = dy_tm ? nullptr : dy_last;
      } else {
        S.dy = (const float*)(ws + w.layer[l + 1].dx);
        S.dy_last = nullptr;
      }
      S.zeros = (const float*)(ws + w.zeros_bh);
      S.dc_carry = (float*)(ws + L.dc_carry);
      S.dgates = (bf16_t*)(ws + L.dgates);
      S.dg_blk_all = (bf16_t*)(ws + L.dg_blk_all);
      S.flags = (unsigned*)(ws + L.bflags);
      S.t_hi = T - 1 - c * Cz;
      S.nsteps = (c * Cz + Cz <= T) ? Cz : T - c * Cz;
      lay[ns] = l;
      chk[ns] = c;
      ++ns;
    }
    if (ns == 0) {
      for (int i = 0; i < npending; ++i) {
        const BesideGemm& g = pending[i];
        if ((rc = gemm_nt(g.A, g.Bt, nullptr, g.C, g.M, g.N, g.K, CSN_BF16, CSN_F32, 0, st, P.opt))) return rc;
        if (pending_add[i].l && (rc = add_dh_n(pending_add[i]))) return rc;
      }
      npending = 0;
      continue;
    }
    a.nslots = ns;
    a.ngemm = npending;
    DhAdd launch_adds[3];
    int nadds = 0;
    for (int i = 0; i < npending; ++i) {
      a.gemm[i] = pending[i];
      if (pending_add[i].l) launch_adds[nadds++] = pending_add[i];
    }
    npending = 0;
    a.agree = try_local ? (unsigned long long*)(ws + w.agree_b) + (size_t)dg * 8 : nullptr;
    if ((rc = prof_pair(g_prof, 1, false, st))) return rc;
    if ((rc = launch_bwd_persist(a, st, P.dlen))) return rc;
    if ((rc = prof_pair(g_prof, 1, true, st))) return rc;
    ++n_launch;
    for (int i = 0; i < nadds; ++i)
      if ((rc = add_dh_n(launch_adds[i]))) return rc;
    for (int i = 0; i < ns; ++i) {
      const int l = lay[i];
      if (l == 0) continue;
      const LayerWs& L = w.layer[l];
      const int t_hi = T - 1 - chk[i] * Cz, t_lo = t_hi - a.slot[i].nsteps + 1;
      const bf16_t* Ag = (const bf16_t*)(ws + L.dgates) + (size_t)t_lo * B * G;
      float* Cg = (float*)(ws + L.dx) + (size_t)t_lo * B * H;
      const int64_t Mg = (int64_t)(t_hi - t_lo + 1) * B;
      const DhAdd add{(dh_n && (chk[i] == 0 || P.dlen)) ? l : 0, t_lo, t_hi};
      if (beside) {
        pending_add[npending] = add;
        pending[npending++] = BesideGemm{Ag, (const bf16_t*)(ws + L.wiht), Cg, (int)Mg, H, (int)G};
      } else {
        if ((rc = gemm_nt(Ag, ws + L.wiht, nullptr, Cg, Mg, H, G, CSN_BF16, CSN_F32, 0, st, P.opt))) return rc;
        if (add.l && (rc = add_dh_n(add))) return rc;
      }
    }
  }
  if ((rc = prof_mark(g_prof, 3, st))) return rc;
  g_prof.launches[1] = n_launch;
  g_prof.cells[1] = T * NL;
  g_prof.have[1] = g_prof.on;

  if (dx != nullptr) {
    const LayerWs& L = w.layer[0];
    if ((rc = gemm_nt(ws + L.dgates, ws + L.wiht, nullptr, ws + L.dx, TB, d->I, G, CSN_BF16, CSN_F32, 0,
                          st, P.opt)))
      return rc;
    if ((rc = emit_dx(P, (const float*)(ws + L.dx), dx, d->I, st))) return rc;
  }
  for (int l = NL - 1; l >= 0; --l) {
    if ((rc = weight_grads(l))) return rc;
    P.grads_ready(l);
  }
  return CSN_OK;
}

static int check_state_args(const Plan& P, const char* fn, const void* const* ptrs, const char* const* names, int n) {
  for (int i = 0; i < n; ++i) {
    if (ptrs[i] == nullptr) continue;
    CSN_REQUIRE(P.state, "%s: %s given, but the plan was created without CSN_LSTM_STATE", fn, names[i]);
    CSN_REQUIRE((reinterpret_cast<uintptr_t>(ptrs[i]) & 15) == 0, "%s: %s must be 16-B aligned", fn, names[i]);
  }
  return CSN_OK;
}

extern "C" int csn_lstm_forward(csnLstmPlan* Pp, const float* x, int64_t x_stride_b, int64_t x_stride_t,
                                const float* const* w_ih, const float* const* w_hh, const float* const* b_ih,
                                const float* const* b_hh, const float* h0, const float* c0, void* workspace,
                                float* y_last, float* y_all, float* h_n, float* c_n, csnStream_t stream) {
  CSN_REQUIRE(Pp != nullptr, "csn_lstm_forward: null plan");
  Plan& P = *Pp;
  const csnLstmDesc* d = &P.d;
  CSN_REQUIRE(x && w_ih && w_hh && b_ih && b_hh && workspace, "csn_lstm_forward: null pointer");
  CSN_REQUIRE((reinterpret_cast<uintptr_t>(workspace) & 255) == 0, "csn_lstm_forward: workspace must be 256-B aligned");
  CSN_REQUIRE(y_last || y_all || h_n || c_n, "csn_lstm_forward: no output requested");
  {
    const void* ptrs[4] = {h0, c0, h_n, c_n};
    const char* names[4] = {"h0", "c0", "h_n", "c_n"};
    if (int rc = check_state_args(P, "csn_lstm_forward", ptrs, names, 4)) return rc;
  }
  for (int l = 0; l < d->L; ++l)
    CSN_REQUIRE(w_ih[l] && w_hh[l] && b_ih[l] && b_hh[l], "csn_lstm_forward: null parameter pointer, layer %d", l);
  int dev = -1;
  CSN_HIP_CHECK(hipGetDevice(&dev));
  CSN_REQUIRE(dev == P.device, "csn_lstm_forward: plan was created on device %d, current device is %d", P.device, dev);
  hipStream_t st = as_stream(stream);
  const WsLayout& w = P.w;
  const int training = P.training;
  char* ws = (char*)workspace;
  const int B = d->B, T = d->T, H = d->H, dt = d->dtype;
  const size_t es = dtype_size(dt);
  int rc;
  if ((rc = upload_lengths(Pp, st))) return rc;
  if (P.dlen != nullptr) {
    if (P.t_eff > 0) {
      EffectiveT scope(P.d, P.t_eff);
      rc = w.il ? forward_il(P, ws, x, x_stride_b, x_stride_t, w_ih, w_hh, b_ih, b_hh, h0, c0, training, stream)
                : forward_v1(P, ws, x, x_stride_b, x_stride_t, w_ih, w_hh, b_ih, b_hh, h0, c0, training, stream);
      if (rc) return rc;
    } else {
      for (int l = 0; l < d->L; ++l) {
        const LayerWs& L = w.layer[l];
        if (h0) {
          if ((rc = launch_cast(h0 + (size_t)l * B * H, ws + L.h_all, (int64_t)B * H, dt, st))) return rc;
        } else {
          CSN_HIP_CHECK(hipMemsetAsync(ws + L.h_all, 0, (size_t)B * H * es, st));
        }
        if (c0)
          CSN_HIP_CHECK(hipMemcpyAsync(ws + L.c_all, c0 + (size_t)l * B * H, (size_t)B * H * 4, hipMemcpyDeviceToDevice, st));
        else
          CSN_HIP_CHECK(hipMemsetAsync(ws + L.c_all, 0, (size_t)B * H * 4, st));
      }
      if (h0 || c0) P.state_seen = true;
      P.prof.have[0] = false;
    }
    const unsigned gbh = grid_for((int64_t)B * H);
    auto gather_h = [&](const LayerWs& L, float* out) {
      if (dt == CSN_BF16) gather_state_kernel<bf16_t><<<gbh, 256, 0, st>>>((const bf16_t*)(ws + L.h_all), P.dlen, out, B, H);
      else gather_state_kernel<float><<<gbh, 256, 0, st>>>((const float*)(ws + L.h_all), P.dlen, out, B, H);
    };
    for (int l = 0; l < d->L; ++l) {
      const LayerWs& L = w.layer[l];
      if (h_n) gather_h(L, h_n + (size_t)l * B * H);
      if (c_n) gather_state_kernel<float><<<gbh, 256, 0, st>>>((const float*)(ws + L.c_all), P.dlen, c_n + (size_t)l * B * H, B, H);
    }
    const LayerWs& top = w.layer[d->L - 1];
    if (y_last) gather_h(top, y_last);
    if (y_all) {
      const int64_t n = (int64_t)T * B * H;
      if (dt == CSN_BF16)
        gather_y_all_len_kernel<bf16_t><<<grid_for(n), 256, 0, st>>>((const bf16_t*)(ws + top.h_all), y_all, P.dlen, B, T, H);
      else
        gather_y_all_len_kernel<float><<<grid_for(n), 256, 0, st>>>((const float*)(ws + top.h_all), y_all, P.dlen, B, T, H);
    }
    CSN_LAUNCH_CHECK();
    return CSN_OK;
  }
  if (w.il)
    rc = forward_il(P, ws, x, x_stride_b, x_stride_t, w_ih, w_hh, b_ih, b_hh, h0, c0, training, stream);
  else if (w.f32_persist)
    rc = forward_f32p(P, ws, x, x_stride_b, x_stride_t, w_ih, w_hh, b_ih, b_hh, training, stream);
  else
    rc = forward_v1(P, ws, x, x_stride_b, x_stride_t, w_ih, w_hh, b_ih, b_hh, h0, c0, training, stream);
  if (rc) return rc;
  for (int l = 0; l < d->L && (h_n || c_n); ++l) {
    const LayerWs& L = w.layer[l];
    if (h_n && (rc = launch_upcast(ws + L.h_all + (size_t)T * B * H * es, dt, h_n + (size_t)l * B * H, (int64_t)B * H, st)))
      return rc;
    if (c_n)
      CSN_HIP_CHECK(hipMemcpyAsync(c_n + (size_t)l * B * H, ws + L.c_all + (size_t)T * B * H * 4, (size_t)B * H * 4,
                                   hipMemcpyDeviceToDevice, st));
  }
  const LayerWs& top = w.layer[d->L - 1];
  if (y_last)
    if ((rc = launch_upcast(ws + top.h_all + (size_t)T * B * H * es, dt, y_last, (int64_t)B * H, st))) return rc;
  if (y_all) {
    const int64_t n = (int64_t)T * B * H;
    if (dt == CSN_BF16)
// ... 151 lines not shown
```

### cerebralsignalnetworks_amd/csrc/lstm_bwd_persist.hip

```cpp
#include "csn_common.h"
#include "lstm_cell_common.h"
#include "lstm_cell_blk.h"
#include "gemm_beside.h"

#ifdef CSN_PSTAMPS
#ifndef CSN_STAMP_BLOCK
#define CSN_STAMP_BLOCK 11
#endif
__device__ unsigned long long g_bstamps[16];
#define CSN_BSTAMP(i)                                                          \
  do {                                                                         \
    __builtin_amdgcn_sched_barrier(0);                                         \
    if (tid == 0 && blockIdx.x == CSN_STAMP_BLOCK) {                           \
      const unsigned long long now_ = wall_clock64();                          \
      atomicAdd(&g_bstamps[i], now_ - last_);                                  \
      last_ = now_;                                                            \
    }                                                                          \
    __builtin_amdgcn_sched_barrier(0);                                         \
  } while (0)
#else
#define CSN_BSTAMP(i)
#endif

namespace csn {

typedef __attribute__((ext_vector_type(4))) unsigned u32x4;

static constexpr unsigned long long kBwdSpinTimeoutTicks = 20000000ull;

static constexpr int kBwdRedTile = 68;
__device__ __forceinline__ int bwd_red_pos(int r, int q) { return (r >> 1) + 8 * (r & 1) + 17 * q; }

typedef __attribute__((ext_vector_type(4))) unsigned bu32x4;

__device__ __forceinline__ bf16x8 bload_sc1_b128(__amdgpu_buffer_rsrc_t rsrc, unsigned byte_off, int soff = 0) {
  bu32x4 v = __builtin_amdgcn_raw_buffer_load_b128(rsrc, (int)byte_off, soff, 16);
  union { bu32x4 u; bf16x8 b; } cvt;
  cvt.u = v;
  return cvt.b;
}
template <bool WT>
__device__ __forceinline__ void bstore_b128(__amdgpu_buffer_rsrc_t rsrc, unsigned byte_off, const bf16x8& v, int soff = 0) {
  union { bu32x4 u; bf16x8 b; } cvt;
  cvt.b = v;
  __builtin_amdgcn_raw_buffer_store_b128(cvt.u, rsrc, (int)byte_off, soff, WT ? 16 : 0);
}

struct PersistLens { const int* lengths; };
struct PersistNoLens {};
template <bool MASK> struct PersistLensArg { typedef PersistNoLens type; };
template <> struct PersistLensArg<true> { typedef PersistLens type; };

template <int NUT, int KS, bool DPOLL, bool MASK = false>
__global__ void __launch_bounds__(256) lstm_bwd_persist_kernel(PersistBwdArgs a, typename PersistLensArg<MASK>::type lens) {
#ifndef CSN_BWD_RING
#define CSN_BWD_RING 5
#endif
  constexpr int RING = KS >= 32 ? 3 : (KS < CSN_BWD_RING ? KS : CSN_BWD_RING);
  constexpr int NT = 4 * NUT;
  constexpr int QPR = 4 * NUT;
  constexpr int NPAIR = 64 * QPR;
  constexpr int NPASS = NPAIR / 256;
  static_assert(NPAIR % 256 == 0, "tile must split evenly over the 256 threads");
  extern __shared__ __attribute__((aligned(16))) float4 red[];
  const int B = a.B, H = a.H, MT = a.MT, T = a.T;
  const int tid = threadIdx.x, lane = tid & 63, wave = tid >> 6;
#ifdef CSN_PSTAMPS
  const unsigned long long t_entry_ = wall_clock64();
#endif
  const int nslices = H / (16 * NUT);
  int grp, slice;
  if (a.xcd_groups) {
    grp = blockIdx.x & 7;
    slice = blockIdx.x >> 3;
    const int ngroups = a.nslots * MT, gs = a.grid_slices;
    if (grp >= ngroups || slice >= nslices) {
      if (a.ngemm > 0) {
        const int idle_here = gs - nslices;
        const unsigned base = grp <= ngroups ? (unsigned)(grp * idle_here)
                                             : (unsigned)(ngroups * idle_here + (grp - ngroups) * gs);
        const unsigned worker = base + (unsigned)(grp < ngroups ? slice - nslices : slice);
        const unsigned nworkers = (unsigned)(ngroups * idle_here + (8 - ngroups) * gs);
        for (int i = 0; i < a.ngemm; ++i) beside_gemm_tiles(a.gemm[i], reinterpret_cast<char*>(red), worker, nworkers);
      }
      return;
    }
  } else {
    grp = blockIdx.x / nslices;
    slice = blockIdx.x % nslices;
  }
  const PersistBwdSlot& S = a.slot[grp / MT];
  const int mt = grp % MT;
  const int u0 = slice * 16 * NUT, m0 = mt * 64;
  const int K = 4 * H, kblocks = K >> 5;
  const int ks_beg = wave * KS;
  const size_t slab = (size_t)a.Bpad * K;
  const bf16_t* const wt_blk = S.wt_blk;
  const bf16_t* const gates = S.gates;
  const float* const c_all = S.c_all;
  const float* const dy = S.dy;
  const float* const dy_last = S.dy_last;
  bf16_t* const dgates = S.dgates;
  bf16_t* const dg_blk_all = S.dg_blk_all;
  unsigned* const flags = S.flags + (size_t)mt * kPersistFlagLine;
  const size_t flag_step = (size_t)MT * kPersistFlagLine;
  const int t_hi = S.t_hi, nsteps = S.nsteps;
  constexpr bool dpoll = DPOLL;

  bool local = false;
  if (a.xcd_groups && a.agree != nullptr) {
    if (tid == 0) {
      const unsigned xcc = __builtin_amdgcn_s_getreg(6164) & 7u;
      const unsigned long long mine = 1ull | (1ull << (8 + 6 * xcc));
      __hip_atomic_fetch_add(a.agree + grp, mine, __ATOMIC_RELAXED, __HIP_MEMORY_SCOPE_AGENT);
      const unsigned long long t_begin = wall_clock64();
      unsigned long long v;
      while (((v = __hip_atomic_load(a.agree + grp, __ATOMIC_RELAXED, __HIP_MEMORY_SCOPE_AGENT)) & 0xffull) <
             (unsigned long long)nslices) {
        __builtin_amdgcn_s_sleep(1);
        if (__hip_atomic_load(a.error_flag, __ATOMIC_RELAXED, __HIP_MEMORY_SCOPE_AGENT) != 0u) break;
        if (wall_clock64() - t_begin > kBwdSpinTimeoutTicks) {
          __hip_atomic_store(a.error_flag, 1u, __ATOMIC_RELAXED, __HIP_MEMORY_SCOPE_AGENT);
          break;
        }
      }
      ((__attribute__((address_space(3))) int*)(__attribute__((address_space(3))) void*)red)[0] = (int)(((v >> (8 + 6 * xcc)) & 63ull) == (unsigned long long)nslices);
    }
    __syncthreads();
    local = ((__attribute__((address_space(3))) int*)(__attribute__((address_space(3))) void*)red)[0] != 0;
    __syncthreads();
  }

  const int rot = a.rotate ? (slice * KS) / nslices : 0;
  bf16x8 wreg[KS][NUT];
#pragma unroll
  for (int kb = 0; kb < KS; ++kb) {
    const int kk = (kb + rot) % KS;
#pragma unroll
    for (int ut = 0; ut < NUT; ++ut)
      wreg[kb][ut] = *reinterpret_cast<const bf16x8*>(wt_blk + ((int64_t)((u0 >> 4) + ut) * kblocks + ks_beg + kk) * 512 + lane * 8);
  }

  int prow[NPASS], puq[NPASS], prl[NPASS], pjq[NPASS];
  bool pok[NPASS];
  float4 dcn[NPASS], cc[NPASS];
  int plen[NPASS];
#pragma unroll
  for (int ps = 0; ps < NPASS; ++ps) {
    const int p = tid + ps * 256;
    prl[ps] = p / QPR;
    pjq[ps] = p % QPR;
    prow[ps] = m0 + prl[ps];
    puq[ps] = u0 + 4 * pjq[ps];
    pok[ps] = prow[ps] < B;
    dcn[ps] = make_float4(0.f, 0.f, 0.f, 0.f);
    cc[ps] = make_float4(0.f, 0.f, 0.f, 0.f);
    plen[ps] = 0;
    if constexpr (MASK) {
      if (pok[ps]) plen[ps] = lens.lengths[prow[ps]];
    }
    if (pok[ps]) {
      dcn[ps] = *reinterpret_cast<const float4*>(S.dc_carry + (size_t)prow[ps] * H + puq[ps]);
      cc[ps] = *reinterpret_cast<const float4*>(c_all + ((size_t)(t_hi + 1) * B + prow[ps]) * H + puq[ps]);
    }
  }

  bf16x8 gt_n[NPASS][2];
  float4 cpv_n[NPASS], dy_n[NPASS];
  auto request_saved = [&](int t) {
#pragma unroll
    for (int ps = 0; ps < NPASS; ++ps) {
      cpv_n[ps] = make_float4(0.f, 0.f, 0.f, 0.f);
      dy_n[ps] = make_float4(0.f, 0.f, 0.f, 0.f);
      if (pok[ps]) {
        const bf16x8* gp = reinterpret_cast<const bf16x8*>(gates + ((size_t)t * B + prow[ps]) * K + 4 * (size_t)puq[ps]);
        gt_n[ps][0] = nt_load(gp);
        gt_n[ps][1] = nt_load(gp + 1);
        cpv_n[ps] = nt_load(reinterpret_cast<const float4*>(c_all + ((size_t)t * B + prow[ps]) * H + puq[ps]));
        const float* dsrc = dy != nullptr ? dy + (size_t)t * B * H : ((dy_last != nullptr && t == T - 1) ? dy_last : S.zeros);
        dy_n[ps] = nt_load(reinterpret_cast<const float4*>(dsrc + (size_t)prow[ps] * H + puq[ps]));
      }
    }
  };
  request_saved(t_hi);
  const __amdgpu_buffer_rsrc_t ring_rsrc = __builtin_amdgcn_make_buffer_rsrc(
      (void*)dg_blk_all, 0, (int)((size_t)4 * slab * 2), 0x00020000);
  const int slab_bytes = (int)(slab * 2);
#ifdef CSN_PSTAMPS
  unsigned long long last_ = wall_clock64();
  if (tid == 0 && blockIdx.x == CSN_STAMP_BLOCK) atomicAdd(&g_bstamps[6], last_ - t_entry_);
#endif

  auto arm_region = [&](int arm_off) {
    const bf16x8 sent = __builtin_bit_cast(bf16x8, (u32x4){0xffffffffu, 0xffffffffu, 0xffffffffu, 0xffffffffu});
#pragma unroll
    for (int ps = 0; ps < NPASS; ++ps) {
      const unsigned o0 = (unsigned)(blk_offset(prow[ps], 4 * (int64_t)puq[ps], K) * 2);
      const unsigned o1 = (unsigned)(blk_offset(prow[ps], 4 * (int64_t)puq[ps] + 8, K) * 2);
      if (local) {
        bstore_b128<false>(ring_rsrc, o0, sent, arm_off);
        bstore_b128<false>(ring_rsrc, o1, sent, arm_off);
      } else {
        bstore_b128<true>(ring_rsrc, o0, sent, arm_off);
        bstore_b128<true>(ring_rsrc, o1, sent, arm_off);
      }
    }
  };
  for (int s = 0; s < nsteps; ++s) {
    const int t = t_hi - s;
    bf16x8 gt[NPASS][2];
    float4 cpv[NPASS], dyv[NPASS];
#pragma unroll
    for (int ps = 0; ps < NPASS; ++ps) {
      gt[ps][0] = gt_n[ps][0];
      gt[ps][1] = gt_n[ps][1];
      cpv[ps] = cpv_n[ps];
      dyv[ps] = dy_n[ps];
    }

    f32x4 acc[4][NUT];
#pragma unroll
    for (int rg = 0; rg < 4; ++rg)
#pragma unroll
      for (int ut = 0; ut < NUT; ++ut) acc[rg][ut] = (f32x4){0.f, 0.f, 0.f, 0.f};

    if (t < T - 1) {
      {
        const int npw = nslices >> 2;
        const unsigned* fl;
        if constexpr (dpoll) {
          const int pi = lane < 4 * npw ? lane >> 2 : 0, pw = lane & 3;
          const int pp = 64 * pw + 63 + (NPASS - 1) * 256;
          const int64_t prow_w = m0 + pp / QPR, pcol_w = 4 * (int64_t)((wave * npw + pi) * 16 * NUT + 4 * (pp % QPR)) + 8;
          fl = reinterpret_cast<const unsigned*>(dg_blk_all + (size_t)((t + 1) & 3) * slab + blk_offset(prow_w, pcol_w, K));
        } else {
          fl = flags + (size_t)(t + 1) * flag_step + wave * npw + (lane < npw ? lane : 0);
        }
        const unsigned not_yet = dpoll ? 0xffffffffu : 0u;
        const unsigned long long t_begin = wall_clock64();
        while (!(dpoll && CSN_DPOLL_MODE(a.data_polls) == 2) && !__all(__hip_atomic_load(fl, __ATOMIC_RELAXED, __HIP_MEMORY_SCOPE_AGENT) != not_yet)) {
          __builtin_amdgcn_s_sleep(1);
          if (__hip_atomic_load(a.error_flag, __ATOMIC_RELAXED, __HIP_MEMORY_SCOPE_AGENT) != 0u) break;
          if (wall_clock64() - t_begin > kBwdSpinTimeoutTicks) {
            __hip_atomic_store(a.error_flag, 1u, __ATOMIC_RELAXED, __HIP_MEMORY_SCOPE_AGENT);
            break;
          }
        }
      }
      CSN_BSTAMP(0);
      const __amdgpu_buffer_rsrc_t slabs_rsrc = dpoll ? ring_rsrc : __builtin_amdgcn_make_buffer_rsrc(
          (void*)(dg_blk_all + (size_t)(t + 1) * slab), 0, slab_bytes, 0x00020000);
      const int src_off = dpoll ? __builtin_amdgcn_readfirstlane(((t + 1) & 3) * slab_bytes) : 0;
      int rot_t = rot;
      asm volatile("" : "+s"(rot_t));
      const unsigned base = (unsigned)((((size_t)(m0 >> 4) * kblocks + ks_beg) * 512 + lane * 8) * 2);
      const unsigned long long t_phase = wall_clock64();
      bool again = false;
      int redone = 0;
      bool proven = false;
      do {
        if (again) {
          __builtin_amdgcn_s_sleep(1);
#pragma unroll
          for (int rg = 0; rg < 4; ++rg)
#pragma unroll
            for (int ut = 0; ut < NUT; ++ut) acc[rg][ut] = (f32x4){0.f, 0.f, 0.f, 0.f};
        }
        bf16x8 df[RING][4];
        int kbo = rot_t * 1024;
        auto issue_group = [&](int slot) {
#pragma unroll
          for (int rg = 0; rg < 4; ++rg)
            df[slot][rg] = bload_sc1_b128(slabs_rsrc, base + (unsigned)(rg * kblocks) * 1024u, src_off + kbo);
          kbo = kbo + 1024 == KS * 1024 ? 0 : kbo + 1024;
        };
#pragma unroll
        for (int kb = 0; kb < RING; ++kb) {
          issue_group(kb);
          __builtin_amdgcn_sched_barrier(0);
        }
#ifdef CSN_SLAB_TAGS
        bool stale = false;
#ifdef CSN_SLAB_TAGS_DUMP
        int stale_kb = -1;
        unsigned stale_u0 = 0;
#endif
#endif
#pragma unroll
        for (int kb = 0; kb < KS; ++kb) {
#ifdef CSN_SLAB_TAGS
          if constexpr (dpoll) {
            const unsigned want = (unsigned)(((t + 1) >> 2) & 1);
#pragma unroll
            for (int rg = 0; rg < 4; ++rg) {
              const u32x4 u = __builtin_bit_cast(u32x4, df[kb % RING][rg]);
              const bool bad = u[0] != 0xffffffffu && (u[0] & 1u) != want;
#ifdef CSN_SLAB_TAGS_DUMP
              if (bad && stale_kb < 0) { stale_kb = kb * 4 + rg; stale_u0 = u[0]; }
#endif
              stale |= bad;
            }
          }
#endif
#pragma unroll
          for (int rg = 0; rg < 4; ++rg)
#pragma unroll
            for (int ut = 0; ut < NUT; ++ut)
              acc[rg][ut] = __builtin_amdgcn_mfma_f32_16x16x32_bf16(wreg[kb][ut], df[kb % RING][rg], acc[rg][ut], 0, 0, 0);
          __builtin_amdgcn_sched_barrier(0);
          if (kb + RING < KS) {
            issue_group(kb % RING);
            __builtin_amdgcn_sched_barrier(0);
          }
        }
#ifdef CSN_SLAB_TAGS
        if (__any(stale) && lane == 0) __hip_atomic_store(a.error_flag + 2, 1u, __ATOMIC_RELAXED, __HIP_MEMORY_SCOPE_AGENT);
#ifdef CSN_SLAB_TAGS_DUMP
        if (stale) {
          if (atomicCAS(a.error_flag + 7, 0u, 1u) == 0u) {
            unsigned* dbg = a.error_flag + 8;
            dbg[0] = (unsigned)t; dbg[1] = (unsigned)s; dbg[2] = (unsigned)grp; dbg[3] = (unsigned)slice; dbg[4] = (unsigned)wave;
            dbg[5] = (unsigned)lane; dbg[6] = (unsigned)stale_kb; dbg[7] = stale_u0; dbg[8] = (unsigned)local; dbg[9] = (unsigned)redone;
            dbg[10] = 0u; dbg[11] = (unsigned)(((t + 1) >> 2) & 1); dbg[12] = (unsigned)rot_t; dbg[13] = (unsigned)nsteps;
            dbg[14] = __builtin_amdgcn_s_getreg(6164) & 7u; dbg[15] = (unsigned)__popcll(__ballot(stale));
          }
        }
#endif
#endif
        again = false;
        if constexpr (dpoll) {
          float chk = 0.f;
#pragma unroll
          for (int rg = 0; rg < 4; ++rg)
#pragma unroll
            for (int ut = 0; ut < NUT; ++ut) chk += (acc[rg][ut][0] + acc[rg][ut][1]) + (acc[rg][ut][2] + acc[rg][ut][3]);
          if (__builtin_expect(!__all(chk == chk), 0)) {
#ifdef CSN_PSTAMPS
            if (lane == 0) atomicAdd(&g_bstamps[8 + wave], 1ull);
#endif
            if (proven) {
              if (lane == 0) __hip_atomic_store(a.error_flag + 1, 1u, __ATOMIC_RELAXED, __HIP_MEMORY_SCOPE_AGENT);
            } else {
              if (++redone >= 2) {
                bool sentinel = false;
                int kbo2 = rot_t * 1024;
#pragma unroll 1
                for (int kb = 0; kb < KS; ++kb) {
#pragma unroll
                  for (int rg = 0; rg < 4; ++rg) {
                    const u32x4 u = __builtin_bit_cast(u32x4, bload_sc1_b128(slabs_rsrc, base + (unsigned)(rg * kblocks) * 1024u, src_off + kbo2));
                    sentinel |= (u[0] == 0xffffffffu) | (u[3] == 0xffffffffu);
                  }
                  kbo2 = kbo2 + 1024 == KS * 1024 ? 0 : kbo2 + 1024;
                }
                proven = !__any(sentinel);
              }
              again = __hip_atomic_load(a.error_flag, __ATOMIC_RELAXED, __HIP_MEMORY_SCOPE_AGENT) == 0u;
              if (wall_clock64() - t_phase > kBwdSpinTimeoutTicks) {
                __hip_atomic_store(a.error_flag, 1u, __ATOMIC_RELAXED, __HIP_MEMORY_SCOPE_AGENT);
                again = false;
              }
            }
          }
        }
      } while (again);
    }
    if (s + 1 < nsteps) request_saved(t - 1);
    __builtin_amdgcn_sched_barrier(0);
    CSN_BSTAMP(1);

#pragma unroll
    for (int rg = 0; rg < 4; ++rg)
#pragma unroll
      for (int ut = 0; ut < NUT; ++ut)
        red[(wave * NT + rg * NUT + ut) * kBwdRedTile + bwd_red_pos(lane & 15, lane >> 4)] = make_float4(acc[rg][ut][0], acc[rg][ut][1], acc[rg][ut][2], acc[rg][ut][3]);
    __syncthreads();
    CSN_BSTAMP(2);

    if (dpoll && !CSN_DPOLL_NO_REARM(a.data_polls)) {
      arm_region(__builtin_amdgcn_readfirstlane(((t + 2) & 3) * slab_bytes));
      __builtin_amdgcn_sched_barrier(0);
    }

    const __amdgpu_buffer_rsrc_t slabs_rsrc = dpoll ? ring_rsrc : __builtin_amdgcn_make_buffer_rsrc(
        (void*)(dg_blk_all + (size_t)t * slab), 0, slab_bytes, 0x00020000);
    const int dst_off = dpoll ? __builtin_amdgcn_readfirstlane((t & 3) * slab_bytes) : 0;
#pragma unroll
    for (int ps = 0; ps < NPASS; ++ps) {
      if (!pok[ps]) {
        if (dpoll) {
#ifdef CSN_SLAB_TAGS
          const unsigned ztag = (unsigned)((t >> 2) & 1);
#else
          const unsigned ztag = 0u;
#endif
          const bf16x8 z = __builtin_bit_cast(bf16x8, (u32x4){ztag, 0u, 0u, 0u});
          const unsigned z0 = (unsigned)(blk_offset(prow[ps], 4 * (int64_t)puq[ps], K) * 2);
          const unsigned z1 = (unsigned)(blk_offset(prow[ps], 4 * (int64_t)puq[ps] + 8, K) * 2);
          if (local) {
            bstore_b128<false>(slabs_rsrc, z0, z, dst_off);
            bstore_b128<false>(slabs_rsrc, z1, z, dst_off);
          } else {
            bstore_b128<true>(slabs_rsrc, z0, z, dst_off);
            bstore_b128<true>(slabs_rsrc, z1, z, dst_off);
          }
        }
        continue;
      }
      const int rl = prl[ps], jq = pjq[ps], row = prow[ps], uq = puq[ps];
      const int idx = ((rl >> 4) * NUT + (jq >> 2)) * kBwdRedTile + bwd_red_pos(rl & 15, jq & 3);
      float4 sm = red[idx];
#pragma unroll
      for (int w2 = 1; w2 < 4; ++w2) {
        const float4 v = red[w2 * NT * kBwdRedTile + idx];
        sm.x += v.x; sm.y += v.y; sm.z += v.z; sm.w += v.w;
      }
      const float dh[4] = {sm.x + dyv[ps].x, sm.y + dyv[ps].y, sm.z + dyv[ps].z, sm.w + dyv[ps].w};
      const float cv[4] = {cc[ps].x, cc[ps].y, cc[ps].z, cc[ps].w};
      const float cpr[4] = {cpv[ps].x, cpv[ps].y, cpv[ps].z, cpv[ps].w};
      const float dcv[4] = {dcn[ps].x, dcn[ps].y, dcn[ps].z, dcn[ps].w};
      float out[16], dcarry[4];
#pragma unroll
      for (int q = 0; q < 4; ++q) {
        const bf16x8& g8 = gt[ps][q >> 1];
        const float gi = (float)g8[(q & 1) * 4 + 0], gf = (float)g8[(q & 1) * 4 + 1];
        const float gg = (float)g8[(q & 1) * 4 + 2], go = (float)g8[(q & 1) * 4 + 3];
        const float tc = fast_tanh(cv[q]);
        const float d_o = dh[q] * tc;
        const float dc = dh[q] * go * (1.0f - tc * tc) + dcv[q];
        out[4 * q + 0] = dc * gg * gi * (1.0f - gi);
        out[4 * q + 1] = dc * cpr[q] * gf * (1.0f - gf);
        out[4 * q + 2] = dc * gi * (1.0f - gg * gg);
        out[4 * q + 3] = d_o * go * (1.0f - go);
        dcarry[q] = dc * gf;
      }
      if constexpr (MASK) {
        const bool dead = t >= plen[ps];
#pragma unroll
        for (int e = 0; e < 16; ++e) out[e] = dead ? 0.f : out[e];
#pragma unroll
        for (int q = 0; q < 4; ++q) dcarry[q] = dead ? dcv[q] : dcarry[q];
      }
      bf16x8 lo, hi;
#pragma unroll
      for (int e = 0; e < 8; ++e) { lo[e] = (bf16_t)out[e]; hi[e] = (bf16_t)out[8 + e]; }
      const unsigned o0 = (unsigned)(blk_offset(row, 4 * (int64_t)uq, K) * 2);
      const unsigned o1 = (unsigned)(blk_offset(row, 4 * (int64_t)uq + 8, K) * 2);
#ifdef CSN_SLAB_TAGS
      {
        u32x4 ul = __builtin_bit_cast(u32x4, lo), uh = __builtin_bit_cast(u32x4, hi);
        const unsigned tag = (unsigned)((t >> 2) & 1);
        ul[0] = (ul[0] & ~1u) | tag;
        uh[0] = (uh[0] & ~1u) | tag;
        lo = __builtin_bit_cast(bf16x8, ul);
        hi = __builtin_bit_cast(bf16x8, uh);
      }
#endif
      if (local) {
        bstore_b128<false>(slabs_rsrc, o0, lo, dst_off);
        bstore_b128<false>(slabs_rsrc, o1, hi, dst_off);
      } else {
        bstore_b128<true>(slabs_rsrc, o0, lo, dst_off);
        bstore_b128<true>(slabs_rsrc, o1, hi, dst_off);
      }
      bf16x8* op = reinterpret_cast<bf16x8*>(dgates + ((size_t)t * B + row) * K + 4 * (size_t)uq);
      nt_store(op, lo);
      nt_store(op + 1, hi);
      dcn[ps] = make_float4(dcarry[0], dcarry[1], dcarry[2], dcarry[3]);
      cc[ps] = cpv[ps];
    }
    CSN_BSTAMP(3);
    if (!dpoll) asm volatile("s_waitcnt vmcnt(0)" ::: "memory");
    __syncthreads();
    CSN_BSTAMP(4);
    if (!dpoll && tid == 0) {
      unsigned* fl = flags + (size_t)t * flag_step + slice;
      if (local) *fl = 1u;
      else __hip_atomic_store(fl, 1u, __ATOMIC_RELAXED, __HIP_MEMORY_SCOPE_AGENT);
    }
    CSN_BSTAMP(5);
  }

#pragma unroll
  for (int ps = 0; ps < NPASS; ++ps)
    if (pok[ps]) *reinterpret_cast<float4*>(S.dc_carry + (size_t)prow[ps] * H + puq[ps]) = dcn[ps];
}

bool bwd_persist_supported(int B, int H, int dtype, const Options& opt) {
  if (dtype != CSN_BF16 || opt.no_persist || opt.no_persist_bwd) return false;
  return H == 128 || H == 256 || H == 384 || H == 512 || H == 768 || H == 1024;
}
int bwd_persist_slices(int H) { return H / 32; }

template <int NUT, int KS>
static int launch_bwd_persist_t(const PersistBwdArgs& a, hipStream_t st, const int* lengths) {
  size_t lds = (size_t)4 * 4 * NUT * kBwdRedTile * sizeof(float4);
  if (lengths != nullptr) {
    if (int rc = ensure_dyn_lds<&lstm_bwd_persist_kernel<NUT, KS, false, true>>((int)kBesideLdsBytes)) return rc;
    if (int rc = ensure_dyn_lds<&lstm_bwd_persist_kernel<NUT, KS, true, true>>((int)kBesideLdsBytes)) return rc;
  } else {
    if (int rc = ensure_dyn_lds<&lstm_bwd_persist_kernel<NUT, KS, false>>((int)kBesideLdsBytes)) return rc;
    if (int rc = ensure_dyn_lds<&lstm_bwd_persist_kernel<NUT, KS, true>>((int)kBesideLdsBytes)) return rc;
  }
  const unsigned nslices = (unsigned)(a.H / (16 * NUT));
  PersistBwdArgs b = a;
  if (b.xcd_groups) {
    if (b.ngemm > 0) {
      lds = kBesideLdsBytes;
      if (b.grid_slices < (int)nslices) b.grid_slices = (int)nslices;
    } else {
      b.grid_slices = (int)nslices;
    }
  }
  const unsigned grid = b.xcd_groups ? 8u * (unsigned)b.grid_slices : nslices * (unsigned)(b.MT * b.nslots);
  if (lengths != nullptr) {
    const PersistLens pl{lengths};
    if (b.data_polls) lstm_bwd_persist_kernel<NUT, KS, true, true><<<dim3(grid), 256, lds, st>>>(b, pl);
    else lstm_bwd_persist_kernel<NUT, KS, false, true><<<dim3(grid), 256, lds, st>>>(b, pl);
  } else if (b.data_polls) lstm_bwd_persist_kernel<NUT, KS, true><<<dim3(grid), 256, lds, st>>>(b, PersistNoLens{});
  else lstm_bwd_persist_kernel<NUT, KS, false><<<dim3(grid), 256, lds, st>>>(b, PersistNoLens{});
  CSN_LAUNCH_CHECK();
  return CSN_OK;
}

int launch_bwd_persist(const PersistBwdArgs& a, hipStream_t st, const int* lengths) {
  CSN_REQUIRE(a.nslots >= 1 && a.nslots <= 4 && a.MT >= 1, "launch_bwd_persist: bad slot count");
  const int ns = bwd_persist_slices(a.H);
  CSN_REQUIRE(ns % 4 == 0 && ns <= kPersistFlagLine, "launch_bwd_persist: H=%d gives %d slices", a.H, ns);
  if (a.xcd_groups) CSN_REQUIRE(a.nslots * a.MT <= 8, "launch_bwd_persist: groups do not fit 8 XCDs");
  CSN_REQUIRE(a.ngemm >= 0 && a.ngemm <= 3 && (a.ngemm == 0 || a.xcd_groups), "launch_bwd_persist: bad GEMM list");
  for (int i = 0; i < a.ngemm; ++i)
    CSN_REQUIRE(a.gemm[i].K % 64 == 0 && a.gemm[i].N % 4 == 0 && a.gemm[i].M > 0, "launch_bwd_persist: GEMM %d shape", i);
  switch (a.H) {
    case 1024: return launch_bwd_persist_t<2, 32>(a, st, lengths);
    case 768: return launch_bwd_persist_t<2, 24>(a, st, lengths);
    case 512: return launch_bwd_persist_t<2, 16>(a, st, lengths);
    case 384: return launch_bwd_persist_t<2, 12>(a, st, lengths);
    case 256: return launch_bwd_persist_t<2, 8>(a, st, lengths);
    case 128: return launch_bwd_persist_t<2, 4>(a, st, lengths);
  }
  return fail(CSN_ERR_UNSUPPORTED, "launch_bwd_persist: no kernel for H=%d", a.H);
}

}

#ifdef CSN_PSTAMPS
extern "C" int csn_debug_read_bstamps(unsigned long long* out) {
  unsigned long long z[16] = {0};
  if (hipMemcpyFromSymbol(out, HIP_SYMBOL(g_bstamps), sizeof(z)) != hipSuccess) return 1;
  if (hipMemcpyToSymbol(HIP_SYMBOL(g_bstamps), z, sizeof(z)) != hipSuccess) return 1;
  return 0;
}
#endif
```

### cerebralsignalnetworks_amd/csrc/lstm_cell_blk.h

```cpp
#pragma once
#include "csn_common.h"

#ifdef CSN_SLAB_TAGS
#define CSN_DPOLL_MODE(x) ((x) & 3)
#define CSN_DPOLL_NO_REARM(x) (((x) & 4) != 0)
#else
#define CSN_DPOLL_MODE(x) (x)
#define CSN_DPOLL_NO_REARM(x) false
#endif

namespace csn {

struct CellFwdProb {
  const bf16_t* h_prev_blk;
  const bf16_t* w_blk;
  const float* xproj;
  const float* c_prev;
  bf16_t* gates_out;
  float* c_out;
  bf16_t* h_out;
  bf16_t* h_out_blk;
};
struct CellFwdArgs {
  CellFwdProb p[4];
  int B, H;
};

struct CellBwdProb {
  const bf16_t* dg_next_blk;
  const bf16_t* wt_blk;
  const float* dy;
  int64_t dy_ld;
  const bf16_t* gates;
  const float* c;
  const float* c_prev;
  float* dc_carry;
  bf16_t* dg_out;
  bf16_t* dg_out_blk;
};
struct CellBwdArgs {
  CellBwdProb p[4];
  int B, H;
};

struct PersistFwdSlot {
  const bf16_t* w_blk;
  const float* xproj;
  bf16_t* gates;
  float* c_all;
  bf16_t* h_all;
  bf16_t* h_blk_all;
  unsigned* flags;
  const bf16_t* x_blk;
  const bf16_t* wih_blk;
  const float* bias;
  int I;
  int t0, nsteps;
};
struct BesideGemm {
  const bf16_t* A;
  const bf16_t* Bt;
  float* C;
  int M, N, K;
};
static constexpr int kPersistFlagLine = 32;
struct PersistFwdArgs {
  PersistFwdSlot slot[4];
  int nslots;
  int data_polls;
  int xcd_groups;
  int rotate;
  unsigned long long* agree;
  unsigned* error_flag;
  int B, H, T, Bpad, MT;
  int state;
};
bool fwd_persist_supported(int B, int H, int dtype, const Options& opt);
bool fwd_ns_supported(int B, int H, int dtype, const Options& opt);
int fwd_ns_slices(int H);
int launch_fwd_ns(const PersistFwdArgs& a, hipStream_t st);
int fwd_persist_slices(int H);
int launch_fwd_persist(const PersistFwdArgs& a, hipStream_t st);

struct PersistBwdSlot {
  const bf16_t* wt_blk;
  const bf16_t* gates;
  const float* c_all;
  const float* dy;
  const float* dy_last;
  const float* zeros;
  float* dc_carry;
  bf16_t* dgates;
  bf16_t* dg_blk_all;
  unsigned* flags;
  int t_hi, nsteps;
};
struct PersistBwdArgs {
  PersistBwdSlot slot[4];
  int nslots;
  BesideGemm gemm[3];
  int ngemm;
  int grid_slices;
  int xcd_groups;
  int rotate;
  int data_polls;
  unsigned long long* agree;
  unsigned* error_flag;
  int B, H, T, Bpad, MT;
};
bool bwd_persist_supported(int B, int H, int dtype, const Options& opt);
int bwd_persist_slices(int H);
int launch_bwd_persist(const PersistBwdArgs& a, hipStream_t st, const int* lengths = nullptr);

enum { kPrepBlockify = 0, kPrepPermRows, kPrepTransPerm, kPrepBias, kPrepCastX, kPrepBlockifyX };
static constexpr int kPrepMaxJobs = 32;
struct PrepJob {
  int kind;
  const float* a;
  const float* b;
  void* dst;
  int64_t n0, n1, n2, s0, s1, H;
  int perm_r, perm_k;
  int64_t work;
  unsigned blk_begin, blk_count;
};
struct PrepArgs {
  PrepJob job[kPrepMaxJobs];
  int njobs;
};
int launch_prep_multi(PrepArgs& A, hipStream_t st);

bool cell_blk_supported(int H, int dtype, const Options& opt);
int launch_cell_fwd_il(const CellFwdArgs& a, int nprob, hipStream_t st, int max_nk);
int launch_cell_bwd_il(const CellBwdArgs& a, int nprob, hipStream_t st, const CellMask* mask = nullptr);
int launch_blockify_x(const float* x, int64_t xsb, int64_t xst, int B, int T, int I, void* dst, hipStream_t st);
int launch_blockify(const float* src, int64_t ld_r, int64_t ld_k, int64_t R, int64_t K, int perm_r, int perm_k,
                    int64_t H, void* dst, hipStream_t st);
int launch_permute_rows_cast(const float* src, int64_t H, int64_t I, void* dst, hipStream_t st);
int launch_transpose_perm_cast(const float* src, int64_t H, int64_t I, void* dst, hipStream_t st);
int launch_bias_perm_sum(const float* a, const float* b, int64_t H, float* dst, hipStream_t st);
int launch_reduce_slabs_unperm(const float* slabs, int64_t slab_stride, int S, int64_t H, int64_t C, float* out,
                               float* out2, int accumulate, hipStream_t st);

}
```

### cerebralsignalnetworks_amd/csrc/lstm_fwd_ns.hip

```cpp
#include <algorithm>

#include "csn_common.h"
#include "lstm_cell_common.h"
#include "lstm_cell_blk.h"
#include "lstm_ns_util.h"

#ifdef CSN_PSTAMPS
#ifndef CSN_STAMP_BLOCK
#define CSN_STAMP_BLOCK 11
#endif
__device__ unsigned long long g_nstamps[16];
#define CSN_NSTAMP(i)                                                          \
  do {                                                                         \
    __builtin_amdgcn_sched_barrier(0);                                         \
    if (tid == 0 && blockIdx.x == CSN_STAMP_BLOCK) {                           \
      const unsigned long long now_ = wall_clock64();                          \
      atomicAdd(&g_nstamps[i], now_ - last_);                                  \
      last_ = now_;                                                            \
    }                                                                          \
    __builtin_amdgcn_sched_barrier(0);                                         \
  } while (0)
#else
#define CSN_NSTAMP(i)
#endif
// ... 276 lines not shown
#pragma unroll
      for (int rg = 0; rg < 4; ++rg)
#pragma unroll
        for (int j = 0; j < 2; ++j) {
          const f32x4 v = acc[rg][j];
          const float gi = fast_sigmoid(v[0]), gf = fast_sigmoid(v[1]), gg = fast_tanh(v[2]), go = fast_sigmoid(v[3]);
          const int row = rg * 16 + (lane & 15), unit = 8 * wave + 4 * j + (lane >> 4);
          float cprev;
          if constexpr (CLDS) cprev = *reinterpret_cast<const float*>(sc + row * 144 + unit * 4);
          else cprev = cst[rg][j];
          const float cn = gf * cprev + gi * gg;
          const float hn = go * fast_tanh(cn);
          if constexpr (!CLDS) cst[rg][j] = cn;
          *reinterpret_cast<bf16x4*>(sg + row * 288 + unit * 8) = (bf16x4){(bf16_t)gi, (bf16_t)gf, (bf16_t)gg, (bf16_t)go};
          *reinterpret_cast<float*>(sc + row * 144 + unit * 4) = cn;
          *reinterpret_cast<bf16_t*>(sh + row * 80 + unit * 2) = (bf16_t)hn;
        }
      CSN_NSTAMP(2);
      __syncthreads();
      {
        const int rg = tid >> 6, r15 = tid & 15, q = (tid >> 4) & 3;
        const nu32x4 v = *reinterpret_cast<const nu32x4*>(sh + (rg * 16 + r15) * 80 + q * 16);
        const unsigned hoff = (unsigned)(((size_t)(t + 1 - t_first) * slab + ((size_t)((m0 >> 4) + rg) * KB + slice) * 512) * 2) + (unsigned)(tid & 63) * 16u;
        if (local) ns_store_b128<false>(hdst_rsrc, hoff, v);
        else ns_store_b128<true>(hdst_rsrc, hoff, v);
      }
      {
        const int row = tid >> 2, q = tid & 3;
        if (m0 + row < B)
          nt_store(reinterpret_cast<nu32x4*>(h_all + ((size_t)(t + 1) * B + m0 + row) * H + u0 + 8 * q),
                   *reinterpret_cast<const nu32x4*>(sh + row * 80 + q * 16));
      }
#pragma unroll
      for (int k = 0; k < 2; ++k) {
        const int idx = tid + 256 * k, row = idx >> 3, ch = idx & 7;
        if (m0 + row < B)
          nt_store(reinterpret_cast<nu32x4*>(c_all + ((size_t)(t + 1) * B + m0 + row) * H + u0 + 4 * ch),
                   *reinterpret_cast<const nu32x4*>(sc + row * 144 + ch * 16));
      }
      if (gates != nullptr) {
#pragma unroll
        for (int k = 0; k < 4; ++k) {
          const int idx = tid + 256 * k, row = idx >> 4, ch = idx & 15;
          if (m0 + row < B)
            nt_store(reinterpret_cast<nu32x4*>(gates + ((size_t)t * B + m0 + row) * 4 * H + 4 * (size_t)u0 + 8 * ch),
                     *reinterpret_cast<const nu32x4*>(sg + row * 288 + ch * 16));
        }
      }
    }
    CSN_NSTAMP(3);
    asm volatile("s_waitcnt vmcnt(0)" ::: "memory");
    __syncthreads();
    CSN_NSTAMP(4);
    if (tid == 0) {
      unsigned* fl = flags + (size_t)(t + 1) * flag_step + slice;
      if (local) *fl = 1u;
      else __hip_atomic_store(fl, 1u, __ATOMIC_RELAXED, __HIP_MEMORY_SCOPE_AGENT);
    }
    CSN_NSTAMP(5);
    if constexpr (FUSED) {
      if (s + 1 < nsteps) start_from_x();
      CSN_NSTAMP(9);
    }
  }
}

template <int KB, bool FUSE>
__global__ void __launch_bounds__(256) lstm_fwd_ns_kernel(PersistFwdArgs a) {
  extern __shared__ __attribute__((aligned(16))) char smem[];
  const int H = a.H, MT = a.MT;
  const int tid = threadIdx.x;
#ifdef CSN_PSTAMPS
  const unsigned long long t_entry_ = wall_clock64();
#endif
  const int nslices = H >> 5;
  int grp, slice;
  if (a.xcd_groups) {
    grp = blockIdx.x & 7;
    slice = blockIdx.x >> 3;
    if (grp >= a.nslots * MT) return;
  } else {
    grp = blockIdx.x / nslices;
    slice = blockIdx.x % nslices;
  }
  const PersistFwdSlot& S = a.slot[grp / MT];
  const int mt = grp % MT;

  bool local = false;
  if (a.xcd_groups && a.agree != nullptr) {
    if (tid == 0) {
      const unsigned xcc = __builtin_amdgcn_s_getreg(6164) & 7u;
      const unsigned long long mine = 1ull | (1ull << (8 + 6 * xcc));
      __hip_atomic_fetch_add(a.agree + grp, mine, __ATOMIC_RELAXED, __HIP_MEMORY_SCOPE_AGENT);
      const unsigned long long t_begin = wall_clock64();
      unsigned long long v;
      while (((v = __hip_atomic_load(a.agree + grp, __ATOMIC_RELAXED, __HIP_MEMORY_SCOPE_AGENT)) & 0xffull) <
             (unsigned long long)nslices) {
        __builtin_amdgcn_s_sleep(1);
        if (__hip_atomic_load(a.error_flag, __ATOMIC_RELAXED, __HIP_MEMORY_SCOPE_AGENT) != 0u) break;
        if (wall_clock64() - t_begin > kNsSpinTimeoutTicks) {
          __hip_atomic_store(a.error_flag, 1u, __ATOMIC_RELAXED, __HIP_MEMORY_SCOPE_AGENT);
          break;
        }
      }
      ((__attribute__((address_space(3))) int*)(__attribute__((address_space(3))) void*)smem)[0] = (int)(((v >> (8 + 6 * xcc)) & 63ull) == (unsigned long long)nslices);
    }
    __syncthreads();
    local = ((__attribute__((address_space(3))) int*)(__attribute__((address_space(3))) void*)smem)[0] != 0;
    __syncthreads();
  }
#ifdef CSN_PSTAMPS
  if (tid == 0 && blockIdx.x == CSN_STAMP_BLOCK) atomicAdd(&g_nstamps[6], wall_clock64() - t_entry_);
#endif
  bool done = false;
  if constexpr (FUSE) {
    if (__builtin_amdgcn_readfirstlane((int)(S.x_blk != nullptr)) != 0) {
      ns_recurrence<KB, true>(a, S, smem, slice, mt, local);
      done = true;
    }
  }
  if (!done) ns_recurrence<KB, false>(a, S, smem, slice, mt, local);
}

static bool ns_device_has_256_cus() {
  int dev = 0, cus = 0;
  if (hipGetDevice(&dev) != hipSuccess) return false;
  return hipDeviceGetAttribute(&cus, hipDeviceAttributeMultiprocessorCount, dev) == hipSuccess && cus >= 256;
}

bool fwd_ns_supported(int B, int H, int dtype, const Options& opt) {
  if (dtype != CSN_BF16 || opt.no_persist || opt.fwd_ksplit) return false;
  if (!(H == 128 || H == 256 || H == 384 || H == 512 || H == 768 || H == 1024)) return false;
  if (H != 1024 && !opt.fwd_nsplit) return false;
  if (H == 768) return false;
  if (!ns_device_has_256_cus()) return false;
  return fwd_ns_slices(H) * ((B + 63) / 64) <= 128;
}

template <int KB, bool FUSE>
static int launch_ns_t(const PersistFwdArgs& a, hipStream_t st) {
  const size_t lds = (size_t)KB * 4096 + kNsStageBytes;
  if (int rc = ensure_dyn_lds<&lstm_fwd_ns_kernel<KB, FUSE>>((int)lds)) return rc;
  const unsigned nslices = (unsigned)(a.H / 32);
  const unsigned grid = a.xcd_groups ? 8u * nslices : nslices * (unsigned)(a.MT * a.nslots);
  lstm_fwd_ns_kernel<KB, FUSE><<<dim3(grid), 256, lds, st>>>(a);
  CSN_LAUNCH_CHECK();
  return CSN_OK;
}

int fwd_ns_slices(int H) { return H / 32; }

int launch_fwd_ns(const PersistFwdArgs& a, hipStream_t st) {
  CSN_REQUIRE(a.nslots >= 1 && a.nslots <= 4 && a.MT >= 1, "launch_fwd_ns: bad slot count");
  const int ns = fwd_ns_slices(a.H);
  CSN_REQUIRE(ns <= kPersistFlagLine, "launch_fwd_ns: H=%d gives %d slices", a.H, ns);
  if (a.xcd_groups) CSN_REQUIRE(a.nslots * a.MT <= 8, "launch_fwd_ns: groups do not fit 8 XCDs");
  bool fused = false;
  for (int i = 0; i < a.nslots; ++i) {
    fused = fused || a.slot[i].x_blk != nullptr;
    CSN_REQUIRE(a.slot[i].x_blk == nullptr || a.slot[i].I == 128, "launch_fwd_ns: the fused input projection takes I = 128");
    const unsigned long long n = (unsigned long long)a.slot[i].nsteps;
    const unsigned long long worst = std::max({n * (unsigned long long)a.B * a.H * 16ull,
                                               n * (unsigned long long)a.Bpad * (unsigned long long)a.slot[i].I * 2ull,
                                               (n + 1ull) * (unsigned long long)a.Bpad * a.H * 2ull});
    CSN_REQUIRE(worst < (1ull << 32), "launch_fwd_ns: %llu steps per launch at B=%d H=%d address %llu bytes from the launch's base "
                "(32-bit offsets): lower CSN_LSTM_CHUNK", n, a.B, a.H, worst);
  }
#define CSN_NS_CASE(KBV)                                                   \
  case KBV * 32:                                                           \
    return fused ? launch_ns_t<KBV, true>(a, st) : launch_ns_t<KBV, false>(a, st)
  switch (a.H) {
    CSN_NS_CASE(4);
    CSN_NS_CASE(8);
    CSN_NS_CASE(12);
    CSN_NS_CASE(16);
    CSN_NS_CASE(32);
  }
#undef CSN_NS_CASE
  return fail(CSN_ERR_UNSUPPORTED, "launch_fwd_ns: no kernel for H=%d", a.H);
}

}

#ifdef CSN_PSTAMPS
extern "C" int csn_debug_read_nstamps(unsigned long long* out) {
  unsigned long long z[16] = {0};
  if (hipMemcpyFromSymbol(out, HIP_SYMBOL(g_nstamps), sizeof(z)) != hipSuccess) return 1;
  if (hipMemcpyToSymbol(HIP_SYMBOL(g_nstamps), z, sizeof(z)) != hipSuccess) return 1;
  return 0;
}
#endif
```

### cerebralsignalnetworks_amd/csrc/lstm_fwd_persist.hip

```cpp
#include "csn_common.h"
#include "lstm_cell_common.h"
#include "lstm_cell_blk.h"

#ifdef CSN_PSTAMPS
#ifndef CSN_STAMP_BLOCK
#define CSN_STAMP_BLOCK 11
#endif
__device__ unsigned long long g_pstamps[16];
__device__ unsigned long long g_span[5] = {~0ull, 0ull, ~0ull, 0ull, 0ull};
__device__ unsigned long long g_grp_alive[32];
#define CSN_PSTAMP(i)                                                          \
  do {                                                                         \
    __builtin_amdgcn_sched_barrier(0);                                         \
    if (tid == 0 && blockIdx.x == CSN_STAMP_BLOCK) {                           \
      const unsigned long long now_ = wall_clock64();                          \
      atomicAdd(&g_pstamps[i], now_ - last_);                                  \
      last_ = now_;                                                            \
    }                                                                          \
    __builtin_amdgcn_sched_barrier(0);                                         \
  } while (0)
#else
#define CSN_PSTAMP(i)
#endif
#ifdef CSN_PSTAMPS
__device__ __forceinline__ void span_exit(unsigned long long t_entry) {
  if (threadIdx.x != 0) return;
  const unsigned long long t_exit = wall_clock64();
  atomicMin(&g_span[0], t_entry);
  atomicMax(&g_span[1], t_entry);
  atomicMin(&g_span[2], t_exit);
  atomicMax(&g_span[3], t_exit);
  __threadfence();
  if (atomicAdd(&g_span[4], 1ull) + 1ull == (unsigned long long)gridDim.x) {
    __threadfence();
    const unsigned long long e0 = atomicAdd(&g_span[0], 0ull), e1 = atomicAdd(&g_span[1], 0ull);
    const unsigned long long x0 = atomicAdd(&g_span[2], 0ull), x1 = atomicAdd(&g_span[3], 0ull);
    atomicAdd(&g_pstamps[10], x1 - e0);
    atomicAdd(&g_pstamps[11], e1 - e0);
    atomicAdd(&g_pstamps[12], x1 - x0);
    atomicAdd(&g_pstamps[13], 1ull);
    g_span[0] = ~0ull; g_span[1] = 0ull; g_span[2] = ~0ull; g_span[3] = 0ull; g_span[4] = 0ull;
    __threadfence();
  }
}
#endif


namespace csn {

static constexpr int kRedTile = 71;
static constexpr unsigned long long kSpinTimeoutTicks = 20000000ull;

typedef __attribute__((ext_vector_type(4))) unsigned u32x4;
typedef __attribute__((ext_vector_type(2))) float f32x2;

__device__ __forceinline__ bf16x8 load_sc1_b128(__amdgpu_buffer_rsrc_t rsrc, int byte_off, int soff = 0) {
  u32x4 v = __builtin_amdgcn_raw_buffer_load_b128(rsrc, byte_off, soff, 16);
  union { u32x4 u; bf16x8 b; } cvt;
  cvt.u = v;
  return cvt.b;
}

__device__ __forceinline__ unsigned long long pack_h_piece(const float (&v)[4], int tag) {
  union { bf16x4 b; unsigned long long u; } cvt;
  cvt.b = (bf16x4){(bf16_t)v[0], (bf16_t)v[1], (bf16_t)v[2], (bf16_t)v[3]};
#ifdef CSN_SLAB_TAGS
  cvt.u = (cvt.u & ~1ull) | (unsigned long long)(tag & 1);
#endif
  return cvt.u;
}

__device__ __forceinline__ void store_wt_b64(bf16_t* p, const float (&v)[4], int tag) {
  __hip_atomic_store(reinterpret_cast<unsigned long long*>(p), pack_h_piece(v, tag), __ATOMIC_RELAXED, __HIP_MEMORY_SCOPE_AGENT);
}

__device__ __forceinline__ void store_plain_b64(bf16_t* p, const float (&v)[4], int tag) {
  *reinterpret_cast<unsigned long long*>(p) = pack_h_piece(v, tag);
}

template <typename T, typename Pred>
__device__ __forceinline__ T bounded_poll(const T* p, unsigned* error_flag, Pred done) {
  const unsigned long long t_begin = wall_clock64();
  T v;
  while (!done(v = __hip_atomic_load(p, __ATOMIC_RELAXED, __HIP_MEMORY_SCOPE_AGENT))) {
    __builtin_amdgcn_s_sleep(1);
    if (__hip_atomic_load(error_flag, __ATOMIC_RELAXED, __HIP_MEMORY_SCOPE_AGENT) != 0u) break;
    if (wall_clock64() - t_begin > kSpinTimeoutTicks) {
      __hip_atomic_store(error_flag, 1u, __ATOMIC_RELAXED, __HIP_MEMORY_SCOPE_AGENT);
      break;
    }
  }
  return v;
}

#ifndef CSN_FWD_RING
#define CSN_FWD_RING 4
#endif
template <int NQ, int KS, bool DPOLL>
__global__ void __launch_bounds__(256) lstm_fwd_persist_kernel(PersistFwdArgs a) {
  constexpr int NT = 4 * NQ;
  constexpr int NPAIR = 64 * NQ;
  constexpr int NPASS = (NPAIR + 255) / 256;
  constexpr bool HALFQ = (NPAIR % 256) == 128;
  constexpr int NFULL = NPAIR / 256;
  extern __shared__ __attribute__((aligned(16))) float4 red[];
  const int B = a.B, H = a.H, MT = a.MT;
  const int tid = threadIdx.x, lane = tid & 63, wave = tid >> 6;
#ifdef CSN_PSTAMPS
  const unsigned long long t_entry_ = wall_clock64();
#endif
  const int nslices = H / (4 * NQ);
  int grp, slice;
  if (a.xcd_groups) {
    grp = blockIdx.x & 7;
    slice = blockIdx.x >> 3;
    if (grp >= a.nslots * MT) {
#ifdef CSN_PSTAMPS
      span_exit(t_entry_);
#endif
      return;
    }
  } else {
    grp = blockIdx.x / nslices;
    slice = blockIdx.x % nslices;
  }
  const PersistFwdSlot& S = a.slot[grp / MT];
  const int mt = grp % MT;
  const int u0 = slice * 4 * NQ, m0 = mt * 64;
  const int kblocks = H >> 5;
  const int ks_beg = wave * KS;
  const size_t slab = (size_t)a.Bpad * H;
  const bf16_t* const w_blk = S.w_blk;
  const float* const xproj = S.xproj;
  bf16_t* const gates = S.gates;
  float* const c_all = S.c_all;
  bf16_t* const h_all = S.h_all;
  bf16_t* const h_blk_all = S.h_blk_all;
  unsigned* const flags = S.flags + (size_t)mt * kPersistFlagLine;
  const size_t flag_step = (size_t)MT * kPersistFlagLine;
  const int t_first = S.t0, nsteps = S.nsteps;
  constexpr bool dpoll = DPOLL;
  const bf16_t* const x_blk = S.x_blk;
  const bool fused = x_blk != nullptr;
  const int xkb = S.I >> 5;
  const bool xwave = fused && __builtin_amdgcn_readfirstlane(wave) < xkb;

  bool local = false;
  if (a.xcd_groups && a.agree != nullptr) {
    if (tid == 0) {
      const unsigned xcc = __builtin_amdgcn_s_getreg(6164) & 7u;
      const unsigned long long mine = 1ull | (1ull << (8 + 6 * xcc));
      __hip_atomic_fetch_add(a.agree + grp, mine, __ATOMIC_RELAXED, __HIP_MEMORY_SCOPE_AGENT);
      const unsigned long long v = bounded_poll(a.agree + grp, a.error_flag, [&](unsigned long long x) {
        return (unsigned)(x & 0xffull) >= (unsigned)nslices;
      });
      ((__attribute__((address_space(3))) int*)(__attribute__((address_space(3))) void*)red)[0] = (int)(((v >> (8 + 6 * xcc)) & 63ull) == (unsigned long long)nslices);
    }
    __syncthreads();
    local = ((__attribute__((address_space(3))) int*)(__attribute__((address_space(3))) void*)red)[0] != 0;
    __syncthreads();
  }

  const int rot = a.rotate ? (slice * KS) / nslices : 0;
  bf16x8 wreg[KS][NQ];
#pragma unroll
  for (int ks = 0; ks < KS; ++ks) {
    const int kk = (ks + rot) % KS;
#pragma unroll
    for (int j = 0; j < NQ; ++j)
      wreg[ks][j] = *reinterpret_cast<const bf16x8*>(w_blk + ((int64_t)((u0 >> 2) + j) * kblocks + ks_beg + kk) * 512 + lane * 8);
  }

  static_assert(NQ <= 8 && NPASS * 4 <= 8, "register sets too small");
  f32x4 cur[8], nxt[8];
#pragma unroll
  for (int i = 0; i < 8; ++i) cur[i] = nxt[i] = (f32x4){0.f, 0.f, 0.f, 0.f};
  float* const bias_lds = reinterpret_cast<float*>(red + 4 * NT * kRedTile);
  if (fused) {
    if (xwave) {
#pragma unroll
      for (int j = 0; j < NQ; ++j)
        cur[j] = *reinterpret_cast<const f32x4*>(S.wih_blk + ((int64_t)((u0 >> 2) + j) * xkb + wave) * 512 + lane * 8);
    }
    if (tid < NQ * 4)
      reinterpret_cast<float4*>(bias_lds)[tid] =
          *reinterpret_cast<const float4*>(S.bias + 4 * (size_t)u0 + 16 * (tid >> 2) + 4 * (tid & 3));
    __syncthreads();
  }
  const unsigned xslab = (unsigned)a.Bpad * (unsigned)S.I;

  float4 cst[NPASS];
  int prow[NPASS], puq[NPASS], prl[NPASS], pj[NPASS];
  bool pok[NPASS];
  const int hq = tid & 1;
#pragma unroll
  for (int ps = 0; ps < NPASS; ++ps) {
    const bool hp = HALFQ && ps == NFULL;
    const int p = hp ? NFULL * 256 + (tid >> 1) : tid + ps * 256;
    prl[ps] = p / NQ;
    pj[ps] = p % NQ;
    prow[ps] = m0 + prl[ps];
    puq[ps] = u0 + 4 * pj[ps];
    pok[ps] = p < NPAIR && prow[ps] < B;
    cst[ps] = make_float4(0.f, 0.f, 0.f, 0.f);
    if (pok[ps] && (t_first > 0 || a.state)) {
      const float* cp = c_all + ((size_t)t_first * B + prow[ps]) * H + puq[ps];
      if (hp) {
        const f32x2 c2 = *reinterpret_cast<const f32x2*>(cp + 2 * hq);
        cst[ps] = make_float4(c2[0], c2[1], 0.f, 0.f);
      } else {
        cst[ps] = *reinterpret_cast<const float4*>(cp);
      }
    }
  }

  const __amdgpu_buffer_rsrc_t hsrc =
      __builtin_amdgcn_make_buffer_rsrc((void*)h_blk_all, 0, (int)((size_t)(a.T + 1) * slab * 2), 0x00020000);
#ifdef CSN_PSTAMPS
  unsigned long long last_ = wall_clock64();
  if (tid == 0 && blockIdx.x == CSN_STAMP_BLOCK) atomicAdd(&g_pstamps[6], last_ - t_entry_);
  const unsigned long long t_loop_ = last_;
#endif

  auto request_input = [&](int t) {
    if (fused) {
      if (xwave) {
#pragma unroll
        for (int rg = 0; rg < 4; ++rg)
          nxt[rg] = nt_load(reinterpret_cast<const f32x4*>(x_blk + (size_t)t * xslab + ((size_t)((m0 >> 4) + rg) * xkb + wave) * 512 + lane * 8));
      }
      return;
    }
#pragma unroll
    for (int ps = 0; ps < NPASS; ++ps)
      if (pok[ps]) {
        const f32x4* xr = reinterpret_cast<const f32x4*>(xproj + ((size_t)t * B + prow[ps]) * 4 * H + 4 * (size_t)puq[ps]);
        if (HALFQ && ps == NFULL) {
#pragma unroll
          for (int q = 0; q < 2; ++q) nxt[ps * 4 + q] = nt_load(xr + 2 * hq + q);
        } else {
#pragma unroll
          for (int q = 0; q < 4; ++q) nxt[ps * 4 + q] = nt_load(xr + q);
        }
      }
  };
  request_input(t_first);

  for (int s = 0; s < nsteps; ++s) {
    const int t = t_first + s;
    bf16x8 xf[4];
    if (fused) {
#pragma unroll
      for (int rg = 0; rg < 4; ++rg) xf[rg] = __builtin_bit_cast(bf16x8, nxt[rg]);
    } else {
#pragma unroll
      for (int i = 0; i < 8; ++i) cur[i] = nxt[i];
    }

    const size_t slot_in = dpoll ? (size_t)(t & 3) : (size_t)t;
    const size_t slot_out = dpoll ? (size_t)((t + 1) & 3) : (size_t)(t + 1);

    f32x4 acc[4][NQ];
#pragma unroll
    for (int rg = 0; rg < 4; ++rg)
#pragma unroll
      for (int j = 0; j < NQ; ++j) acc[rg][j] = (f32x4){0.f, 0.f, 0.f, 0.f};
    if (fused && wave == 0) {
#pragma unroll
      for (int j = 0; j < NQ; ++j) {
        const float4 bz = reinterpret_cast<const float4*>(bias_lds)[j * 4 + (lane >> 4)];
#pragma unroll
        for (int rg = 0; rg < 4; ++rg) acc[rg][j] = (f32x4){bz.x, bz.y, bz.z, bz.w};
      }
    }

    if (t > 0 || a.state) {
      const bool wait = t > 0;
      {
        const int npw = nslices >> 2;
        const unsigned* fl;
        if constexpr (dpoll) {
          const int pi = lane < 4 * npw ? lane >> 2 : 0, pw = lane & 3;
          int pp = 64 * pw + 63;
#pragma unroll
          for (int ps = 1; ps < NPASS; ++ps)
            if (64 * pw + 63 + ps * 256 < NPAIR) pp = 64 * pw + 63 + ps * 256;
          if (HALFQ) pp = NFULL * 256 + 32 * pw + 31;
          fl = reinterpret_cast<const unsigned*>(h_blk_all + slot_in * slab +
                                                 blk_offset(m0 + pp / NQ, (wave * npw + pi) * 4 * NQ + 4 * (pp % NQ), H));
        } else {
          fl = flags + (size_t)t * flag_step + wave * npw + (lane < npw ? lane : 0);
        }
        const unsigned not_yet = dpoll ? 0xffffffffu : 0u;
        const unsigned long long t_begin = wall_clock64();
        while (wait && !(dpoll && CSN_DPOLL_MODE(a.data_polls) == 2) && !__all(__hip_atomic_load(fl, __ATOMIC_RELAXED, __HIP_MEMORY_SCOPE_AGENT) != not_yet)) {
          __builtin_amdgcn_s_sleep(1);
          if (__hip_atomic_load(a.error_flag, __ATOMIC_RELAXED, __HIP_MEMORY_SCOPE_AGENT) != 0u) break;
          if (wall_clock64() - t_begin > kSpinTimeoutTicks) {
            __hip_atomic_store(a.error_flag, 1u, __ATOMIC_RELAXED, __HIP_MEMORY_SCOPE_AGENT);
            break;
          }
        }
      }
      CSN_PSTAMP(0);
      const int base = (int)((slot_in * slab + ((size_t)(m0 >> 4) * kblocks + ks_beg) * 512 + lane * 8) * 2);
      constexpr int RING_MAX = (NQ == 8 && KS == 4) ? 2 : ((NQ == 6 && KS == 6 && !DPOLL) ? 3 : CSN_FWD_RING);
      constexpr int RING = KS > RING_MAX ? RING_MAX : KS;
      bf16x8 hf[RING][4];
      int rot_t = rot;
      asm volatile("" : "+s"(rot_t));
      int kbo = rot_t * 1024;
      auto issue_group = [&](int slot) {
#pragma unroll
        for (int rg = 0; rg < 4; ++rg) hf[slot][rg] = load_sc1_b128(hsrc, base + rg * kblocks * 1024, kbo);
        kbo = kbo + 1024 == KS * 1024 ? 0 : kbo + 1024;
      };
#pragma unroll
      for (int ks = 0; ks < RING; ++ks) {
        issue_group(ks);
        __builtin_amdgcn_sched_barrier(0);
      }
#pragma unroll
      for (int ks = 0; ks < KS; ++ks) {
        if (dpoll) {
          auto whole = [&]() {
            bool ok = true;
#pragma unroll
            for (int rg = 0; rg < 4; ++rg) {
              const u32x4 u = __builtin_bit_cast(u32x4, hf[ks % RING][rg]);
              ok = ok && u[0] != 0xffffffffu && u[2] != 0xffffffffu;
            }
            return __all(ok);
          };
          if (wait && __builtin_expect(!whole(), 0)) {
            const unsigned long long t_begin = wall_clock64();
            do {
              __builtin_amdgcn_s_sleep(1);
#pragma unroll
              for (int rg = 0; rg < 4; ++rg) hf[ks % RING][rg] = load_sc1_b128(hsrc, base + (rg * kblocks + (ks + rot) % KS) * 1024);
              if (wall_clock64() - t_begin > kSpinTimeoutTicks) {
                __hip_atomic_store(a.error_flag, 1u, __ATOMIC_RELAXED, __HIP_MEMORY_SCOPE_AGENT);
                break;
              }
            } while (!whole() && __hip_atomic_load(a.error_flag, __ATOMIC_RELAXED, __HIP_MEMORY_SCOPE_AGENT) == 0u);
          }
        }
#ifdef CSN_SLAB_TAGS
        if (dpoll && wait) {
          const unsigned want = (unsigned)(((t - 1) >> 2) & 1);
          bool stale = false;
#pragma unroll
          for (int rg = 0; rg < 4; ++rg) {
            const u32x4 u = __builtin_bit_cast(u32x4, hf[ks % RING][rg]);
            stale |= (u[0] != 0xffffffffu && (u[0] & 1u) != want) | (u[2] != 0xffffffffu && (u[2] & 1u) != want);
          }
          if (__any(stale) && lane == 0) __hip_atomic_store(a.error_flag + 2, 1u, __ATOMIC_RELAXED, __HIP_MEMORY_SCOPE_AGENT);
        }
#endif
#pragma unroll
        for (int rg = 0; rg < 4; ++rg)
#pragma unroll
          for (int j = 0; j < NQ; ++j)
            acc[rg][j] = __builtin_amdgcn_mfma_f32_16x16x32_bf16(wreg[ks][j], hf[ks % RING][rg], acc[rg][j], 0, 0, 0);
        __builtin_amdgcn_sched_barrier(0);
        if (ks + RING < KS) {
          issue_group(ks % RING);
          __builtin_amdgcn_sched_barrier(0);
        }
      }
    }
    if (xwave) {
#pragma unroll
      for (int rg = 0; rg < 4; ++rg)
#pragma unroll
        for (int j = 0; j < NQ; ++j)
          acc[rg][j] = __builtin_amdgcn_mfma_f32_16x16x32_bf16(__builtin_bit_cast(bf16x8, cur[j]), xf[rg], acc[rg][j], 0, 0, 0);
    }
    __builtin_amdgcn_sched_barrier(0);
    if (s + 1 < nsteps) request_input(t + 1);
    __builtin_amdgcn_sched_barrier(0);
    CSN_PSTAMP(1);

#pragma unroll
    for (int rg = 0; rg < 4; ++rg)
#pragma unroll
      for (int j = 0; j < NQ; ++j)
        red[(wave * NT + rg * NQ + j) * kRedTile + lane] = make_float4(acc[rg][j][0], acc[rg][j][1], acc[rg][j][2], acc[rg][j][3]);
    __syncthreads();
    CSN_PSTAMP(2);

    if (dpoll && !CSN_DPOLL_NO_REARM(a.data_polls)) {
#pragma unroll
      for (int ps = 0; ps < NPASS; ++ps) {
        if (HALFQ && ps == NFULL ? hq != 0 : tid + ps * 256 >= NPAIR) continue;
        unsigned long long* sp = reinterpret_cast<unsigned long long*>(
            h_blk_all + (size_t)((t + 3) & 3) * slab + blk_offset(prow[ps], puq[ps], H));
        if (local) *sp = ~0ull;
        else __hip_atomic_store(sp, ~0ull, __ATOMIC_RELAXED, __HIP_MEMORY_SCOPE_AGENT);
      }
      __builtin_amdgcn_sched_barrier(0);
    }


#pragma unroll
    for (int ps = 0; ps < NPASS; ++ps) {
      if (!pok[ps]) {
        if (dpoll && (HALFQ && ps == NFULL ? hq == 0 : tid + ps * 256 < NPAIR)) {
          unsigned long long* zp = reinterpret_cast<unsigned long long*>(h_blk_all + slot_out * slab + blk_offset(prow[ps], puq[ps], H));
#ifdef CSN_SLAB_TAGS
          const unsigned long long zv = (unsigned long long)((t >> 2) & 1);
#else
          const unsigned long long zv = 0ull;
#endif
          if (local) *zp = zv;
          else __hip_atomic_store(zp, zv, __ATOMIC_RELAXED, __HIP_MEMORY_SCOPE_AGENT);
        }
        continue;
      }
      const bool hp = HALFQ && ps == NFULL;
      const int nq = hp ? 2 : 4;
      const int q0 = hp ? 2 * hq : 0;
      const int rl = prl[ps], j = pj[ps], row = prow[ps], uq = puq[ps];
      float gi[4], gf[4], gg[4], go[4], cn[4], hn[4];
      const float cpv[4] = {cst[ps].x, cst[ps].y, cst[ps].z, cst[ps].w};
#pragma unroll
      for (int q = 0; q < 4; ++q) {
        if (q >= nq) continue;
        const int idx = ((rl >> 4) * NQ + j) * kRedTile + (rl & 15) + 16 * (q0 + q);
        float4 sum = red[idx];
#pragma unroll
        for (int w2 = 1; w2 < 4; ++w2) {
          const float4 v = red[w2 * NT * kRedTile + idx];
          sum.x += v.x; sum.y += v.y; sum.z += v.z; sum.w += v.w;
        }
        const f32x4 xq = fused ? (f32x4){0.f, 0.f, 0.f, 0.f} : cur[ps * 4 + q];
        gi[q] = fast_sigmoid(sum.x + xq[0]);
        gf[q] = fast_sigmoid(sum.y + xq[1]);
        gg[q] = fast_tanh(sum.z + xq[2]);
        go[q] = fast_sigmoid(sum.w + xq[3]);
        cn[q] = gf[q] * cpv[q] + gi[q] * gg[q];
        hn[q] = go[q] * fast_tanh(cn[q]);
      }
#ifdef CSN_PSTAMPS
      if (ps == 0) CSN_PSTAMP(8);
#endif
      bf16_t* hdst = h_blk_all + slot_out * slab + blk_offset(row, uq, H);
      if (hp) {
        cst[ps] = make_float4(cn[0], cn[1], 0.f, 0.f);
        union { bf16_t b[2]; unsigned u; } pk;
        pk.b[0] = (bf16_t)hn[0];
        pk.b[1] = (bf16_t)hn[1];
        const unsigned other = (unsigned)__builtin_amdgcn_update_dpp(0, (int)pk.u, 0xB1, 0xf, 0xf, false);
        if (hq == 0) {
          unsigned long long piece = (unsigned long long)pk.u | ((unsigned long long)other << 32);
#ifdef CSN_SLAB_TAGS
          piece = (piece & ~1ull) | (unsigned long long)((t >> 2) & 1);
#endif
          if (local) *reinterpret_cast<unsigned long long*>(hdst) = piece;
          else __hip_atomic_store(reinterpret_cast<unsigned long long*>(hdst), piece, __ATOMIC_RELAXED, __HIP_MEMORY_SCOPE_AGENT);
        }
        if (gates != nullptr) {
          bf16x8 lo = {(bf16_t)gi[0], (bf16_t)gf[0], (bf16_t)gg[0], (bf16_t)go[0], (bf16_t)gi[1], (bf16_t)gf[1], (bf16_t)gg[1], (bf16_t)go[1]};
          __builtin_nontemporal_store(lo, reinterpret_cast<bf16x8*>(gates + ((size_t)t * B + row) * 4 * H + 4 * (size_t)(uq + q0)));
        }
        __builtin_nontemporal_store((f32x2){cn[0], cn[1]}, reinterpret_cast<f32x2*>(c_all + ((size_t)(t + 1) * B + row) * H + uq + q0));
        __builtin_nontemporal_store(pk.u, reinterpret_cast<unsigned*>(h_all + ((size_t)(t + 1) * B + row) * H + uq + q0));
      } else {
        cst[ps] = make_float4(cn[0], cn[1], cn[2], cn[3]);
        if (local) store_plain_b64(hdst, hn, t >> 2);
        else store_wt_b64(hdst, hn, t >> 2);
        if (gates != nullptr) {
          bf16x8 lo = {(bf16_t)gi[0], (bf16_t)gf[0], (bf16_t)gg[0], (bf16_t)go[0], (bf16_t)gi[1], (bf16_t)gf[1], (bf16_t)gg[1], (bf16_t)go[1]};
          bf16x8 hi = {(bf16_t)gi[2], (bf16_t)gf[2], (bf16_t)gg[2], (bf16_t)go[2], (bf16_t)gi[3], (bf16_t)gf[3], (bf16_t)gg[3], (bf16_t)go[3]};
          bf16x8* gp = reinterpret_cast<bf16x8*>(gates + ((size_t)t * B + row) * 4 * H + 4 * (size_t)uq);
          __builtin_nontemporal_store(lo, gp);
          __builtin_nontemporal_store(hi, gp + 1);
        }
        __builtin_nontemporal_store((f32x4){cn[0], cn[1], cn[2], cn[3]},
                                    reinterpret_cast<f32x4*>(c_all + ((size_t)(t + 1) * B + row) * H + uq));
        __builtin_nontemporal_store((bf16x4){(bf16_t)hn[0], (bf16_t)hn[1], (bf16_t)hn[2], (bf16_t)hn[3]},
                                    reinterpret_cast<bf16x4*>(h_all + ((size_t)(t + 1) * B + row) * H + uq));
      }
#ifdef CSN_PSTAMPS
      if (ps == 0) CSN_PSTAMP(9);
#endif
    }
    CSN_PSTAMP(3);
    if (!dpoll) asm volatile("s_waitcnt vmcnt(0)" ::: "memory");
    __syncthreads();
    CSN_PSTAMP(4);
    if (!dpoll && tid == 0) {
      unsigned* fl = flags + (size_t)(t + 1) * flag_step + slice;
      if (local) *fl = 1u;
      else __hip_atomic_store(fl, 1u, __ATOMIC_RELAXED, __HIP_MEMORY_SCOPE_AGENT);
    }
    CSN_PSTAMP(5);
  }
#ifdef CSN_PSTAMPS
  __syncthreads();
  if (tid == 0 && slice == 0) {
    const unsigned long long now_ = wall_clock64();
    atomicAdd(&g_grp_alive[grp & 7], now_ - t_entry_);
    atomicAdd(&g_grp_alive[8 + (grp & 7)], 1ull);
    atomicAdd(&g_grp_alive[16 + (grp & 7)], now_ - t_loop_);
    atomicAdd(&g_grp_alive[24 + (grp & 7)], (unsigned long long)nsteps);
  }
  span_exit(t_entry_);
#endif
}

static bool device_has_256_cus() {
  int dev = 0, cus = 0;
  if (hipGetDevice(&dev) != hipSuccess) return false;
  return hipDeviceGetAttribute(&cus, hipDeviceAttributeMultiprocessorCount, dev) == hipSuccess && cus >= 256;
}

bool fwd_persist_supported(int B, int H, int dtype, const Options& opt) {
  if (dtype != CSN_BF16 || H % 128 != 0 || opt.no_persist) return false;
  if (!device_has_256_cus()) return false;
  const int nq = (H % 24 == 0) ? 6 : 8, ks = H / 128;
  const bool shape = (nq == 6 && (ks == 6 || ks == 3)) || (nq == 8 && (ks == 4 || ks == 2 || ks == 1));
  const int wgs = (H / (4 * nq)) * ((B + 63) / 64);
  return shape && wgs <= 128;
}

int fwd_persist_slices(int H) { return H / (4 * ((H % 24 == 0) ? 6 : 8)); }

template <int NQ, int KS>
static int launch_persist_t(const PersistFwdArgs& a, hipStream_t st) {
  const size_t lds = (size_t)(4 * 4 * NQ * kRedTile + 4 * NQ) * sizeof(float4);
  if (int rc = ensure_dyn_lds<&lstm_fwd_persist_kernel<NQ, KS, false>>((int)lds)) return rc;
  if (int rc = ensure_dyn_lds<&lstm_fwd_persist_kernel<NQ, KS, true>>((int)lds)) return rc;
  const unsigned nslices = (unsigned)(a.H / (4 * NQ));
  const unsigned grid = a.xcd_groups ? 8u * nslices : nslices * (unsigned)(a.MT * a.nslots);
  if (a.data_polls) lstm_fwd_persist_kernel<NQ, KS, true><<<dim3(grid), 256, lds, st>>>(a);
  else lstm_fwd_persist_kernel<NQ, KS, false><<<dim3(grid), 256, lds, st>>>(a);
  CSN_LAUNCH_CHECK();
  return CSN_OK;
}

int launch_fwd_persist(const PersistFwdArgs& a, hipStream_t st) {
  CSN_REQUIRE(a.nslots >= 1 && a.nslots <= 4 && a.MT >= 1, "launch_fwd_persist: bad slot count");
  CSN_REQUIRE(fwd_persist_slices(a.H) % 4 == 0 && fwd_persist_slices(a.H) <= kPersistFlagLine,
              "launch_fwd_persist: H=%d gives %d slices (need a multiple of 4, at most %d)", a.H, fwd_persist_slices(a.H),
              kPersistFlagLine);
  if (a.xcd_groups)
    CSN_REQUIRE(a.nslots * a.MT <= 8 && fwd_persist_slices(a.H) <= 32, "launch_fwd_persist: groups do not fit 8 XCDs");
  const int nq = (a.H % 24 == 0) ? 6 : 8, ks = a.H / 128;
  if (nq == 6 && ks == 6) return launch_persist_t<6, 6>(a, st);
  if (nq == 6 && ks == 3) return launch_persist_t<6, 3>(a, st);
  if (nq == 8 && ks == 4) return launch_persist_t<8, 4>(a, st);
  if (nq == 8 && ks == 2) return launch_persist_t<8, 2>(a, st);
  if (nq == 8 && ks == 1) return launch_persist_t<8, 1>(a, st);
  return fail(CSN_ERR_UNSUPPORTED, "launch_fwd_persist: no kernel for H=%d", a.H);
}

}

#ifdef CSN_PSTAMPS
extern "C" int csn_debug_read_grp_alive(unsigned long long* out) {
  unsigned long long z[32] = {0};
  if (hipMemcpyFromSymbol(out, HIP_SYMBOL(g_grp_alive), sizeof(z)) != hipSuccess) return 1;
  if (hipMemcpyToSymbol(HIP_SYMBOL(g_grp_alive), z, sizeof(z)) != hipSuccess) return 1;
  return 0;
}
extern "C" int csn_debug_read_pstamps(unsigned long long* out) {
  unsigned long long z[16] = {0};
  if (hipMemcpyFromSymbol(out, HIP_SYMBOL(g_pstamps), sizeof(z)) != hipSuccess) return 1;
  if (hipMemcpyToSymbol(HIP_SYMBOL(g_pstamps), z, sizeof(z)) != hipSuccess) return 1;
  return 0;
}
#endif
```

### include/csn_hip.h

```cpp
#ifndef CSN_HIP_H
#define CSN_HIP_H

#include <stddef.h>
#include <stdint.h>

#ifdef __cplusplus
extern "C" {
#endif

typedef void* csnStream_t;

enum csnStatus {
  CSN_OK = 0,
  CSN_ERR_INVALID_ARGUMENT = 1,
  CSN_ERR_HIP = 2,
  CSN_ERR_UNSUPPORTED = 3
};

enum csnDtype { CSN_F32 = 0, CSN_BF16 = 1 };

#define CSN_ABI_VERSION 6
int csn_abi_version(void);
const char* csn_last_error(void);
const char* csn_target_arch(void);

int csn_eeg_bandpass_znorm(const float* x, int B, int C, int T,
                           const double* sos, int nsec, int ddof,
                           void* y, int out_dtype, int time_major, csnStream_t stream);

size_t csn_eeg_filtfilt_scratch_bytes(int S, int T, int C, int nsec);
int csn_eeg_filtfilt(const float* x, int S, int T, int C, const double* sos, int nsec,
                     float* y, void* scratch, csnStream_t stream);

typedef struct csnLstmDesc {
  int32_t B;
  int32_t T;
  int32_t I;
  int32_t H;
  int32_t L;
  int32_t dtype;
} csnLstmDesc;

typedef struct csnLstmPlan csnLstmPlan;
#define CSN_LSTM_STATE 0x100
int csn_lstm_plan_create(const csnLstmDesc* d, int training, csnLstmPlan** out);
void csn_lstm_plan_destroy(csnLstmPlan* plan);
size_t csn_lstm_plan_workspace_bytes(const csnLstmPlan* plan);
int csn_lstm_plan_path(const csnLstmPlan* plan);
int csn_lstm_plan_dgates_copies(const csnLstmPlan* plan);
const char* csn_lstm_plan_kernel_name(const csnLstmPlan* plan, int which);
size_t csn_lstm_workspace_bytes(const csnLstmDesc* d, int training);

int csn_lstm_workspace_init(const csnLstmPlan* plan, void* workspace, csnStream_t stream);

int csn_lstm_forward(csnLstmPlan* plan,
                     const float* x, int64_t x_stride_b, int64_t x_stride_t,
                     const float* const* w_ih, const float* const* w_hh,
                     const float* const* b_ih, const float* const* b_hh,
                     const float* h0, const float* c0,
                     void* workspace, float* y_last, float* y_all,
                     float* h_n, float* c_n, csnStream_t stream);

int csn_lstm_backward(csnLstmPlan* plan,
                      const float* dy_last, const float* dy_all,
                      const float* dh_n, const float* dc_n,
                      void* workspace,
                      float* const* dw_ih, float* const* dw_hh,
                      float* const* db_ih, float* const* db_hh,
                      float* dx, float* dh0, float* dc0, csnStream_t stream);

typedef void (*csnGradReadyFn)(void* user, int layer);
int csn_lstm_plan_set_grad_callback(csnLstmPlan* plan, csnGradReadyFn fn, void* user);

#define CSN_GRAD_OVERWRITE  0
#define CSN_GRAD_ACCUMULATE 1
int csn_lstm_plan_set_grad_mode(csnLstmPlan* plan, int mode);

int csn_lstm_plan_set_lengths(csnLstmPlan* plan, const int32_t* lengths);

#define CSN_STATUS_TIMEOUT 1
#define CSN_STATUS_NONFINITE 2
#define CSN_STATUS_STALE_SLOT 4
int csn_lstm_status_clear(const csnLstmPlan* plan, void* workspace, csnStream_t stream);
int csn_lstm_status_read(const csnLstmPlan* plan, const void* workspace, int* status);
int csn_lstm_status_raise(const csnLstmPlan* plan, void* workspace, csnStream_t stream);

int csn_lstm_profile_enable(csnLstmPlan* plan, int on);
int csn_lstm_profile_read(csnLstmPlan* plan, double* fwd_ms, int* fwd_launches, int* fwd_cells,
                          double* bwd_ms, int* bwd_launches, int* bwd_cells);

int csn_gemm_nt(const void* A, const void* Bt, const float* bias, void* C,
                int64_t M, int64_t N, int64_t K, int dtype, int out_dtype, int accumulate,
                csnStream_t stream);
size_t csn_gemm_tn_scratch_bytes(int64_t M, int64_t N, int64_t K);
int csn_gemm_tn(const void* A, const void* B, float* C,
                int64_t M, int64_t N, int64_t K, int dtype, void* scratch, csnStream_t stream);

int csn_lstm_cell_forward(const void* h_prev, const void* w_hh, const float* xproj, int64_t xproj_ld,
                          const float* c_prev, void* gates_out, float* c_out, void* h_out,
                          int B, int H, int dtype, csnStream_t stream);
int csn_lstm_cell_backward(const void* dgates_next, const void* w_hh_t,
                           const float* dy, int64_t dy_ld,
                           const void* gates, const float* c, const float* c_prev,
                           float* dc_carry, void* dgates_out,
                           int B, int H, int dtype, csnStream_t stream);

size_t csn_cosine_loss_scratch_bytes(int B);
int csn_cosine_loss(const float* student, const float* teacher, int B, int D,
                    float* loss, float* dstudent, float grad_scale, void* scratch, csnStream_t stream);

int csn_rmsprop_step(float* params, const float* grads, float* square_avg, int64_t n,
                     float lr, float alpha, float eps, csnStream_t stream);

int csn_barlow_offdiag_sqsum(const float* c, int D, float* out, csnStream_t stream);

size_t csn_l2_topk_scratch_bytes(int64_t Ng, int64_t Nq);
int csn_l2_topk(const float* gallery, const float* query, int64_t Ng, int64_t Nq, int D, int k,
                int64_t* out_idx, float* out_dist, void* scratch, csnStream_t stream);

#ifdef __cplusplus
}
#endif
#endif
```

Measured before the change: 26310.

## Split persistent LSTM row tiles into 32-row groups to fill idle XCDs

When the grouped persistent forward and backward LSTM kernels would use only a few of the 8 XCD groups, the batch tile of 64 rows is halved to 32 rows. This doubles the number of groups and spreads the recurrent work over more CUs, with separate flag regions in the workspace. It also skips the flag wait on the first step of each launch. The cost is more flag traffic and synchronisation, and half-size MFMA tiles per workgroup.

New measurement: 27060 (median of 6 runs). 1.03x the previous value.

```diff
diff --git a/cerebralsignalnetworks_amd/cabi.py b/cerebralsignalnetworks_amd/cabi.py
--- a/cerebralsignalnetworks_amd/cabi.py
+++ b/cerebralsignalnetworks_amd/cabi.py
@@ -35,6 +35,7 @@
     "csn_lstm_plan_workspace_bytes": (_c_size_t, [_c_void_p]),
     "csn_lstm_plan_path": (_c_int, [_c_void_p]),
     "csn_lstm_plan_dgates_copies": (_c_int, [_c_void_p]),
+    "csn_lstm_plan_half_tile_launches": (_c_int, [_c_void_p, _c_int]),
     "csn_lstm_plan_kernel_name": (ctypes.c_char_p, [_c_void_p, _c_int]),
     "csn_lstm_plan_set_grad_callback": (_c_int, [_c_void_p, _c_void_p, _c_void_p]),
     "csn_lstm_plan_set_grad_mode": (_c_int, [_c_void_p, _c_int]),
@@ -282,6 +283,9 @@
     def dgates_copies(self):
         return load().csn_lstm_plan_dgates_copies(self._plan)
 
+    def half_tile_launches(self, which):
+        return load().csn_lstm_plan_half_tile_launches(self._plan, which)
+
     def forward(self, x_bti, w_ih, w_hh, b_ih, b_hh, want_all=False, h0=None, c0=None, want_state=False):
         d = self.desc
         _need_cuda(x_bti)
diff --git a/cerebralsignalnetworks_amd/csrc/csn_common.h b/cerebralsignalnetworks_amd/csrc/csn_common.h
--- a/cerebralsignalnetworks_amd/csrc/csn_common.h
+++ b/cerebralsignalnetworks_amd/csrc/csn_common.h
@@ -42,7 +42,7 @@
 
 struct Options {
   bool cell_v1, no_persist, no_persist_bwd, persist_streams, no_xcd_local, no_rotate, no_fuse_x, no_beside,
-      no_side_stream, gemm_slot, fwd_ksplit, fwd_nsplit, fwd_flags, bwd_flags, dpoll_no_hint, fwd_hint, gemm_no_dma, gemm_no_256, gemm_generic, gemm_lds64, tn_no_tr, tn_no_stagger, filter_v1, tags_no_rearm, gemm_no_192;
+      no_side_stream, gemm_slot, fwd_ksplit, fwd_nsplit, fwd_flags, bwd_flags, dpoll_no_hint, fwd_hint, gemm_no_dma, gemm_no_256, gemm_generic, gemm_lds64, tn_no_tr, tn_no_stagger, filter_v1, tags_no_rearm, gemm_no_192, no_half_tiles;
   int chunk;
   int tn_stages;
   int fwd_nk;
@@ -62,6 +62,7 @@
   o.no_rotate = on("CSN_NO_ROTATE");
   o.no_fuse_x = on("CSN_NO_FUSE_X");
   o.no_beside = on("CSN_NO_BESIDE");
+  o.no_half_tiles = on("CSN_NO_HALF_TILES");
   o.no_side_stream = on("CSN_NO_SIDE_STREAM");
   o.gemm_slot = on("CSN_GEMM_SLOT");
   o.fwd_ksplit = on("CSN_FWD_KSPLIT");
diff --git a/cerebralsignalnetworks_amd/csrc/lstm.hip b/cerebralsignalnetworks_amd/csrc/lstm.hip
--- a/cerebralsignalnetworks_amd/csrc/lstm.hip
+++ b/cerebralsignalnetworks_amd/csrc/lstm.hip
@@ -121,7 +121,7 @@
     w.zero_bwd = off;
     for (int l = 0; l < d.L; ++l) {
       w.layer[l].dc_carry = take((size_t)d.B * H * 4);
-      w.layer[l].bflags = take((size_t)d.T * (Bpad / 64) * kPersistFlagLine * 4);
+      w.layer[l].bflags = take((size_t)d.T * (Bpad / 64) * 3 * kPersistFlagLine * 4);
     }
     w.agree_b = take(((size_t)d.T + 8) * 8 * sizeof(unsigned long long));
     w.zero_bwd_bytes = off - w.zero_bwd;
@@ -375,6 +375,7 @@
   csn::SideCtx sc;
   csn::Prof prof;
   int dgates_copies = 0;
+  int half_launches[2] = {0, 0};
   csnGradReadyFn grad_cb = nullptr;
   void* grad_cb_user = nullptr;
   int grad_accumulate = 0;
@@ -445,6 +446,10 @@
 }
 
 extern "C" int csn_lstm_plan_dgates_copies(const csnLstmPlan* P) { return P == nullptr ? -1 : P->dgates_copies; }
+
+extern "C" int csn_lstm_plan_half_tile_launches(const csnLstmPlan* P, int which) {
+  return (P == nullptr || which < 0 || which > 1) ? -1 : P->half_launches[which];
+}
 
 static bool bwd_grouped(const csnLstmPlan* P) {
   if (!P->w.persist_bwd) return false;
@@ -1114,6 +1119,7 @@
       CSN_HIP_CHECK(hipMemsetAsync(ws + L.c_all, 0, (size_t)B * H * 4, st));
   }
   int n_launch = 0;
+  P.half_launches[0] = 0;
 
   const int max_slots = NL < nch ? NL : nch;
   const int fwd_slices = w.fwd_ns ? fwd_ns_slices(H) : fwd_persist_slices(H);
@@ -1138,6 +1144,13 @@
       }
       a.nslots = ns;
       a.xcd_groups = 1;
+      const bool half = !w.fwd_ns && !P.opt.no_half_tiles && 2 * ns * MT <= 8;
+      a.half_tiles = half ? 1 : 0;
+      a.MT = half ? 2 * MT : MT;
+      if (half) {
+        for (int i = 0; i < ns; ++i) a.slot[i].flags += ((size_t)T + 1) * MT * kPersistFlagLine;
+        ++P.half_launches[0];
+      }
       a.agree = try_local ? (unsigned long long*)(ws + w.agree) + (size_t)dg * 8 : nullptr;
       if ((rc = prof_pair(g_prof, 0, false, st))) return rc;
       if ((rc = launch_fwd(a, st))) return rc;
@@ -1166,6 +1179,8 @@
   a.nslots = 1;
   a.xcd_groups = 0;
   a.agree = nullptr;
+  a.half_tiles = 0;
+  a.MT = MT;
   for (int c = 0; c < nch; ++c) {
     for (int l = 0; l < NL; ++l) {
       fill_slot(a.slot[0], l, c);
@@ -1393,6 +1408,7 @@
   if (a.data_polls)
     for (int l = 0; l < NL; ++l) CSN_HIP_CHECK(hipMemsetAsync(ws + w.layer[l].dg_blk_all, 0xff, (size_t)4 * Bpad * G * 2, st));
   int n_launch = 0;
+  P.half_launches[1] = 0;
   BesideGemm pending[3];
   DhAdd pending_add[3] = {{0, 0, 0}, {0, 0, 0}, {0, 0, 0}};
   int npending = 0;
@@ -1436,6 +1452,13 @@
     }
     a.nslots = ns;
     a.ngemm = npending;
+    const bool half = !P.opt.no_half_tiles && P.dlen == nullptr && 2 * ns * MT <= 8;
+    a.half_tiles = half ? 1 : 0;
+    a.MT = half ? 2 * MT : MT;
+    if (half) {
+      for (int i = 0; i < ns; ++i) a.slot[i].flags += (size_t)T * MT * kPersistFlagLine;
+      ++P.half_launches[1];
+    }
     DhAdd launch_adds[3];
     int nadds = 0;
     for (int i = 0; i < npending; ++i) {
diff --git a/cerebralsignalnetworks_amd/csrc/lstm_bwd_persist.hip b/cerebralsignalnetworks_amd/csrc/lstm_bwd_persist.hip
--- a/cerebralsignalnetworks_amd/csrc/lstm_bwd_persist.hip
+++ b/cerebralsignalnetworks_amd/csrc/lstm_bwd_persist.hip
@@ -51,15 +51,16 @@
 template <bool MASK> struct PersistLensArg { typedef PersistNoLens type; };
 template <> struct PersistLensArg<true> { typedef PersistLens type; };
 
-template <int NUT, int KS, bool DPOLL, bool MASK = false>
+template <int NUT, int KS, bool DPOLL, bool MASK = false, int RG = 4>
 __global__ void __launch_bounds__(256) lstm_bwd_persist_kernel(PersistBwdArgs a, typename PersistLensArg<MASK>::type lens) {
 #ifndef CSN_BWD_RING
 #define CSN_BWD_RING 5
 #endif
   constexpr int RING = KS >= 32 ? 3 : (KS < CSN_BWD_RING ? KS : CSN_BWD_RING);
-  constexpr int NT = 4 * NUT;
+  static_assert(RG == 4 || RG == 2, "tiles of 64 or 32 rows");
+  constexpr int NT = RG * NUT;
   constexpr int QPR = 4 * NUT;
-  constexpr int NPAIR = 64 * QPR;
+  constexpr int NPAIR = 16 * RG * QPR;
   constexpr int NPASS = NPAIR / 256;
   static_assert(NPAIR % 256 == 0, "tile must split evenly over the 256 threads");
   extern __shared__ __attribute__((aligned(16))) float4 red[];
@@ -91,7 +92,7 @@
   }
   const PersistBwdSlot& S = a.slot[grp / MT];
   const int mt = grp % MT;
-  const int u0 = slice * 16 * NUT, m0 = mt * 64;
+  const int u0 = slice * 16 * NUT, m0 = mt * 16 * RG;
   const int K = 4 * H, kblocks = K >> 5;
   const int ks_beg = wave * KS;
   const size_t slab = (size_t)a.Bpad * K;
@@ -218,9 +219,9 @@
       dyv[ps] = dy_n[ps];
     }
 
-    f32x4 acc[4][NUT];
-#pragma unroll
-    for (int rg = 0; rg < 4; ++rg)
+    f32x4 acc[RG][NUT];
+#pragma unroll
+    for (int rg = 0; rg < RG; ++rg)
 #pragma unroll
       for (int ut = 0; ut < NUT; ++ut) acc[rg][ut] = (f32x4){0.f, 0.f, 0.f, 0.f};
 
@@ -238,7 +239,7 @@
         }
         const unsigned not_yet = dpoll ? 0xffffffffu : 0u;
         const unsigned long long t_begin = wall_clock64();
-        while (!(dpoll && CSN_DPOLL_MODE(a.data_polls) == 2) && !__all(__hip_atomic_load(fl, __ATOMIC_RELAXED, __HIP_MEMORY_SCOPE_AGENT) != not_yet)) {
+        while (!(dpoll && CSN_DPOLL_MODE(a.data_polls) == 2) && (dpoll || s > 0) && !__all(__hip_atomic_load(fl, __ATOMIC_RELAXED, __HIP_MEMORY_SCOPE_AGENT) != not_yet)) {
           __builtin_amdgcn_s_sleep(1);
           if (__hip_atomic_load(a.error_flag, __ATOMIC_RELAXED, __HIP_MEMORY_SCOPE_AGENT) != 0u) break;
           if (wall_clock64() - t_begin > kBwdSpinTimeoutTicks) {
@@ -262,15 +263,15 @@
         if (again) {
           __builtin_amdgcn_s_sleep(1);
 #pragma unroll
-          for (int rg = 0; rg < 4; ++rg)
+          for (int rg = 0; rg < RG; ++rg)
 #pragma unroll
             for (int ut = 0; ut < NUT; ++ut) acc[rg][ut] = (f32x4){0.f, 0.f, 0.f, 0.f};
         }
-        bf16x8 df[RING][4];
+        bf16x8 df[RING][RG];
         int kbo = rot_t * 1024;
         auto issue_group = [&](int slot) {
 #pragma unroll
-          for (int rg = 0; rg < 4; ++rg)
+          for (int rg = 0; rg < RG; ++rg)
             df[slot][rg] = bload_sc1_b128(slabs_rsrc, base + (unsigned)(rg * kblocks) * 1024u, src_off + kbo);
           kbo = kbo + 1024 == KS * 1024 ? 0 : kbo + 1024;
         };
@@ -292,7 +293,7 @@
           if constexpr (dpoll) {
             const unsigned want = (unsigned)(((t + 1) >> 2) & 1);
 #pragma unroll
-            for (int rg = 0; rg < 4; ++rg) {
+            for (int rg = 0; rg < RG; ++rg) {
               const u32x4 u = __builtin_bit_cast(u32x4, df[kb % RING][rg]);
               const bool bad = u[0] != 0xffffffffu && (u[0] & 1u) != want;
 #ifdef CSN_SLAB_TAGS_DUMP
@@ -303,7 +304,7 @@
           }
 #endif
 #pragma unroll
-          for (int rg = 0; rg < 4; ++rg)
+          for (int rg = 0; rg < RG; ++rg)
 #pragma unroll
             for (int ut = 0; ut < NUT; ++ut)
               acc[rg][ut] = __builtin_amdgcn_mfma_f32_16x16x32_bf16(wreg[kb][ut], df[kb % RING][rg], acc[rg][ut], 0, 0, 0);
@@ -331,7 +332,7 @@
         if constexpr (dpoll) {
           float chk = 0.f;
 #pragma unroll
-          for (int rg = 0; rg < 4; ++rg)
+          for (int rg = 0; rg < RG; ++rg)
 #pragma unroll
             for (int ut = 0; ut < NUT; ++ut) chk += (acc[rg][ut][0] + acc[rg][ut][1]) + (acc[rg][ut][2] + acc[rg][ut][3]);
           if (__builtin_expect(!__all(chk == chk), 0)) {
@@ -347,7 +348,7 @@
 #pragma unroll 1
                 for (int kb = 0; kb < KS; ++kb) {
 #pragma unroll
-                  for (int rg = 0; rg < 4; ++rg) {
+                  for (int rg = 0; rg < RG; ++rg) {
                     const u32x4 u = __builtin_bit_cast(u32x4, bload_sc1_b128(slabs_rsrc, base + (unsigned)(rg * kblocks) * 1024u, src_off + kbo2));
                     sentinel |= (u[0] == 0xffffffffu) | (u[3] == 0xffffffffu);
                   }
@@ -370,7 +371,7 @@
     CSN_BSTAMP(1);
 
 #pragma unroll
-    for (int rg = 0; rg < 4; ++rg)
+    for (int rg = 0; rg < RG; ++rg)
 #pragma unroll
       for (int ut = 0; ut < NUT; ++ut)
         red[(wave * NT + rg * NUT + ut) * kBwdRedTile + bwd_red_pos(lane & 15, lane >> 4)] = make_float4(acc[rg][ut][0], acc[rg][ut][1], acc[rg][ut][2], acc[rg][ut][3]);
@@ -494,10 +495,13 @@
 
 template <int NUT, int KS>
 static int launch_bwd_persist_t(const PersistBwdArgs& a, hipStream_t st, const int* lengths) {
-  size_t lds = (size_t)4 * 4 * NUT * kBwdRedTile * sizeof(float4);
+  size_t lds = (size_t)4 * (a.half_tiles ? 2 : 4) * NUT * kBwdRedTile * sizeof(float4);
   if (lengths != nullptr) {
     if (int rc = ensure_dyn_lds<&lstm_bwd_persist_kernel<NUT, KS, false, true>>((int)kBesideLdsBytes)) return rc;
     if (int rc = ensure_dyn_lds<&lstm_bwd_persist_kernel<NUT, KS, true, true>>((int)kBesideLdsBytes)) return rc;
+  } else if (a.half_tiles) {
+    if (int rc = ensure_dyn_lds<&lstm_bwd_persist_kernel<NUT, KS, false, false, 2>>((int)kBesideLdsBytes)) return rc;
+    if (int rc = ensure_dyn_lds<&lstm_bwd_persist_kernel<NUT, KS, true, false, 2>>((int)kBesideLdsBytes)) return rc;
   } else {
     if (int rc = ensure_dyn_lds<&lstm_bwd_persist_kernel<NUT, KS, false>>((int)kBesideLdsBytes)) return rc;
     if (int rc = ensure_dyn_lds<&lstm_bwd_persist_kernel<NUT, KS, true>>((int)kBesideLdsBytes)) return rc;
@@ -517,6 +521,9 @@
     const PersistLens pl{lengths};
     if (b.data_polls) lstm_bwd_persist_kernel<NUT, KS, true, true><<<dim3(grid), 256, lds, st>>>(b, pl);
     else lstm_bwd_persist_kernel<NUT, KS, false, true><<<dim3(grid), 256, lds, st>>>(b, pl);
+  } else if (b.half_tiles) {
+    if (b.data_polls) lstm_bwd_persist_kernel<NUT, KS, true, false, 2><<<dim3(grid), 256, lds, st>>>(b, PersistNoLens{});
+    else lstm_bwd_persist_kernel<NUT, KS, false, false, 2><<<dim3(grid), 256, lds, st>>>(b, PersistNoLens{});
   } else if (b.data_polls) lstm_bwd_persist_kernel<NUT, KS, true><<<dim3(grid), 256, lds, st>>>(b, PersistNoLens{});
   else lstm_bwd_persist_kernel<NUT, KS, false><<<dim3(grid), 256, lds, st>>>(b, PersistNoLens{});
   CSN_LAUNCH_CHECK();
@@ -528,6 +535,9 @@
   const int ns = bwd_persist_slices(a.H);
   CSN_REQUIRE(ns % 4 == 0 && ns <= kPersistFlagLine, "launch_bwd_persist: H=%d gives %d slices", a.H, ns);
   if (a.xcd_groups) CSN_REQUIRE(a.nslots * a.MT <= 8, "launch_bwd_persist: groups do not fit 8 XCDs");
+  CSN_REQUIRE(a.MT * (a.half_tiles ? 32 : 64) == a.Bpad, "launch_bwd_persist: %d tiles of %d rows are not Bpad=%d", a.MT,
+              a.half_tiles ? 32 : 64, a.Bpad);
+  CSN_REQUIRE(!a.half_tiles || (a.xcd_groups && lengths == nullptr), "launch_bwd_persist: 32-row groups need the grouped form and no lengths");
   CSN_REQUIRE(a.ngemm >= 0 && a.ngemm <= 3 && (a.ngemm == 0 || a.xcd_groups), "launch_bwd_persist: bad GEMM list");
   for (int i = 0; i < a.ngemm; ++i)
     CSN_REQUIRE(a.gemm[i].K % 64 == 0 && a.gemm[i].N % 4 == 0 && a.gemm[i].M > 0, "launch_bwd_persist: GEMM %d shape", i);
diff --git a/cerebralsignalnetworks_amd/csrc/lstm_cell_blk.h b/cerebralsignalnetworks_amd/csrc/lstm_cell_blk.h
--- a/cerebralsignalnetworks_amd/csrc/lstm_cell_blk.h
+++ b/cerebralsignalnetworks_amd/csrc/lstm_cell_blk.h
@@ -74,6 +74,7 @@
   unsigned* error_flag;
   int B, H, T, Bpad, MT;
   int state;
+  int half_tiles;
 };
 bool fwd_persist_supported(int B, int H, int dtype, const Options& opt);
 bool fwd_ns_supported(int B, int H, int dtype, const Options& opt);
@@ -107,6 +108,7 @@
   unsigned long long* agree;
   unsigned* error_flag;
   int B, H, T, Bpad, MT;
+  int half_tiles;
 };
 bool bwd_persist_supported(int B, int H, int dtype, const Options& opt);
 int bwd_persist_slices(int H);
diff --git a/cerebralsignalnetworks_amd/csrc/lstm_fwd_ns.hip b/cerebralsignalnetworks_amd/csrc/lstm_fwd_ns.hip
--- a/cerebralsignalnetworks_amd/csrc/lstm_fwd_ns.hip
+++ b/cerebralsignalnetworks_amd/csrc/lstm_fwd_ns.hip
@@ -452,6 +452,7 @@
 
 int launch_fwd_ns(const PersistFwdArgs& a, hipStream_t st) {
   CSN_REQUIRE(a.nslots >= 1 && a.nslots <= 4 && a.MT >= 1, "launch_fwd_ns: bad slot count");
+  CSN_REQUIRE(!a.half_tiles, "launch_fwd_ns: the N-split kernel has no 32-row groups");
   const int ns = fwd_ns_slices(a.H);
   CSN_REQUIRE(ns <= kPersistFlagLine, "launch_fwd_ns: H=%d gives %d slices", a.H, ns);
   if (a.xcd_groups) CSN_REQUIRE(a.nslots * a.MT <= 8, "launch_fwd_ns: groups do not fit 8 XCDs");
diff --git a/cerebralsignalnetworks_amd/csrc/lstm_fwd_persist.hip b/cerebralsignalnetworks_amd/csrc/lstm_fwd_persist.hip
--- a/cerebralsignalnetworks_amd/csrc/lstm_fwd_persist.hip
+++ b/cerebralsignalnetworks_amd/csrc/lstm_fwd_persist.hip
@@ -96,10 +96,11 @@
 #ifndef CSN_FWD_RING
 #define CSN_FWD_RING 4
 #endif
-template <int NQ, int KS, bool DPOLL>
+template <int NQ, int KS, bool DPOLL, int RG = 4>
 __global__ void __launch_bounds__(256) lstm_fwd_persist_kernel(PersistFwdArgs a) {
-  constexpr int NT = 4 * NQ;
-  constexpr int NPAIR = 64 * NQ;
+  static_assert(RG == 4 || RG == 2, "tiles of 64 or 32 rows");
+  constexpr int NT = RG * NQ;
+  constexpr int NPAIR = 16 * RG * NQ;
   constexpr int NPASS = (NPAIR + 255) / 256;
   constexpr bool HALFQ = (NPAIR % 256) == 128;
   constexpr int NFULL = NPAIR / 256;
@@ -126,7 +127,7 @@
   }
   const PersistFwdSlot& S = a.slot[grp / MT];
   const int mt = grp % MT;
-  const int u0 = slice * 4 * NQ, m0 = mt * 64;
+  const int u0 = slice * 4 * NQ, m0 = mt * 16 * RG;
   const int kblocks = H >> 5;
   const int ks_beg = wave * KS;
   const size_t slab = (size_t)a.Bpad * H;
@@ -226,7 +227,7 @@
     if (fused) {
       if (xwave) {
 #pragma unroll
-        for (int rg = 0; rg < 4; ++rg)
+        for (int rg = 0; rg < RG; ++rg)
           nxt[rg] = nt_load(reinterpret_cast<const f32x4*>(x_blk + (size_t)t * xslab + ((size_t)((m0 >> 4) + rg) * xkb + wave) * 512 + lane * 8));
       }
       return;
@@ -248,10 +249,10 @@
 
   for (int s = 0; s < nsteps; ++s) {
     const int t = t_first + s;
-    bf16x8 xf[4];
+    bf16x8 xf[RG];
     if (fused) {
 #pragma unroll
-      for (int rg = 0; rg < 4; ++rg) xf[rg] = __builtin_bit_cast(bf16x8, nxt[rg]);
+      for (int rg = 0; rg < RG; ++rg) xf[rg] = __builtin_bit_cast(bf16x8, nxt[rg]);
     } else {
 #pragma unroll
       for (int i = 0; i < 8; ++i) cur[i] = nxt[i];
@@ -260,9 +261,9 @@
     const size_t slot_in = dpoll ? (size_t)(t & 3) : (size_t)t;
     const size_t slot_out = dpoll ? (size_t)((t + 1) & 3) : (size_t)(t + 1);
 
-    f32x4 acc[4][NQ];
-#pragma unroll
-    for (int rg = 0; rg < 4; ++rg)
+    f32x4 acc[RG][NQ];
+#pragma unroll
+    for (int rg = 0; rg < RG; ++rg)
 #pragma unroll
       for (int j = 0; j < NQ; ++j) acc[rg][j] = (f32x4){0.f, 0.f, 0.f, 0.f};
     if (fused && wave == 0) {
@@ -270,18 +271,18 @@
       for (int j = 0; j < NQ; ++j) {
         const float4 bz = reinterpret_cast<const float4*>(bias_lds)[j * 4 + (lane >> 4)];
 #pragma unroll
-        for (int rg = 0; rg < 4; ++rg) acc[rg][j] = (f32x4){bz.x, bz.y, bz.z, bz.w};
+        for (int rg = 0; rg < RG; ++rg) acc[rg][j] = (f32x4){bz.x, bz.y, bz.z, bz.w};
       }
     }
 
     if (t > 0 || a.state) {
-      const bool wait = t > 0;
+      const bool wait = t > 0 && (dpoll || s > 0);
       {
         const int npw = nslices >> 2;
         const unsigned* fl;
         if constexpr (dpoll) {
           const int pi = lane < 4 * npw ? lane >> 2 : 0, pw = lane & 3;
-          int pp = 64 * pw + 63;
+          int pp = 64 * pw + 63 < NPAIR ? 64 * pw + 63 : NPAIR - 1;
 #pragma unroll
           for (int ps = 1; ps < NPASS; ++ps)
             if (64 * pw + 63 + ps * 256 < NPAIR) pp = 64 * pw + 63 + ps * 256;
@@ -306,13 +307,13 @@
       const int base = (int)((slot_in * slab + ((size_t)(m0 >> 4) * kblocks + ks_beg) * 512 + lane * 8) * 2);
       constexpr int RING_MAX = (NQ == 8 && KS == 4) ? 2 : ((NQ == 6 && KS == 6 && !DPOLL) ? 3 : CSN_FWD_RING);
       constexpr int RING = KS > RING_MAX ? RING_MAX : KS;
-      bf16x8 hf[RING][4];
+      bf16x8 hf[RING][RG];
       int rot_t = rot;
       asm volatile("" : "+s"(rot_t));
       int kbo = rot_t * 1024;
       auto issue_group = [&](int slot) {
 #pragma unroll
-        for (int rg = 0; rg < 4; ++rg) hf[slot][rg] = load_sc1_b128(hsrc, base + rg * kblocks * 1024, kbo);
+        for (int rg = 0; rg < RG; ++rg) hf[slot][rg] = load_sc1_b128(hsrc, base + rg * kblocks * 1024, kbo);
         kbo = kbo + 1024 == KS * 1024 ? 0 : kbo + 1024;
       };
 #pragma unroll
@@ -326,7 +327,7 @@
           auto whole = [&]() {
             bool ok = true;
 #pragma unroll
-            for (int rg = 0; rg < 4; ++rg) {
+            for (int rg = 0; rg < RG; ++rg) {
               const u32x4 u = __builtin_bit_cast(u32x4, hf[ks % RING][rg]);
               ok = ok && u[0] != 0xffffffffu && u[2] != 0xffffffffu;
             }
@@ -337,7 +338,7 @@
             do {
               __builtin_amdgcn_s_sleep(1);
 #pragma unroll
-              for (int rg = 0; rg < 4; ++rg) hf[ks % RING][rg] = load_sc1_b128(hsrc, base + (rg * kblocks + (ks + rot) % KS) * 1024);
+              for (int rg = 0; rg < RG; ++rg) hf[ks % RING][rg] = load_sc1_b128(hsrc, base + (rg * kblocks + (ks + rot) % KS) * 1024);
               if (wall_clock64() - t_begin > kSpinTimeoutTicks) {
                 __hip_atomic_store(a.error_flag, 1u, __ATOMIC_RELAXED, __HIP_MEMORY_SCOPE_AGENT);
                 break;
@@ -350,7 +351,7 @@
           const unsigned want = (unsigned)(((t - 1) >> 2) & 1);
           bool stale = false;
 #pragma unroll
-          for (int rg = 0; rg < 4; ++rg) {
+          for (int rg = 0; rg < RG; ++rg) {
             const u32x4 u = __builtin_bit_cast(u32x4, hf[ks % RING][rg]);
             stale |= (u[0] != 0xffffffffu && (u[0] & 1u) != want) | (u[2] != 0xffffffffu && (u[2] & 1u) != want);
           }
@@ -358,7 +359,7 @@
         }
 #endif
 #pragma unroll
-        for (int rg = 0; rg < 4; ++rg)
+        for (int rg = 0; rg < RG; ++rg)
 #pragma unroll
           for (int j = 0; j < NQ; ++j)
             acc[rg][j] = __builtin_amdgcn_mfma_f32_16x16x32_bf16(wreg[ks][j], hf[ks % RING][rg], acc[rg][j], 0, 0, 0);
@@ -371,7 +372,7 @@
     }
     if (xwave) {
 #pragma unroll
-      for (int rg = 0; rg < 4; ++rg)
+      for (int rg = 0; rg < RG; ++rg)
 #pragma unroll
         for (int j = 0; j < NQ; ++j)
           acc[rg][j] = __builtin_amdgcn_mfma_f32_16x16x32_bf16(__builtin_bit_cast(bf16x8, cur[j]), xf[rg], acc[rg][j], 0, 0, 0);
@@ -382,7 +383,7 @@
     CSN_PSTAMP(1);
 
 #pragma unroll
-    for (int rg = 0; rg < 4; ++rg)
+    for (int rg = 0; rg < RG; ++rg)
 #pragma unroll
       for (int j = 0; j < NQ; ++j)
         red[(wave * NT + rg * NQ + j) * kRedTile + lane] = make_float4(acc[rg][j][0], acc[rg][j][1], acc[rg][j][2], acc[rg][j][3]);
@@ -529,11 +530,17 @@
 template <int NQ, int KS>
 static int launch_persist_t(const PersistFwdArgs& a, hipStream_t st) {
   const size_t lds = (size_t)(4 * 4 * NQ * kRedTile + 4 * NQ) * sizeof(float4);
+  static_assert((4 * 4 * NQ * kRedTile + 4 * NQ) * sizeof(float4) > 80 * 1024, "the LDS request no longer keeps a workgroup alone on its CU");
   if (int rc = ensure_dyn_lds<&lstm_fwd_persist_kernel<NQ, KS, false>>((int)lds)) return rc;
   if (int rc = ensure_dyn_lds<&lstm_fwd_persist_kernel<NQ, KS, true>>((int)lds)) return rc;
   const unsigned nslices = (unsigned)(a.H / (4 * NQ));
   const unsigned grid = a.xcd_groups ? 8u * nslices : nslices * (unsigned)(a.MT * a.nslots);
-  if (a.data_polls) lstm_fwd_persist_kernel<NQ, KS, true><<<dim3(grid), 256, lds, st>>>(a);
+  if (a.half_tiles) {
+    if (int rc = ensure_dyn_lds<&lstm_fwd_persist_kernel<NQ, KS, false, 2>>((int)lds)) return rc;
+    if (int rc = ensure_dyn_lds<&lstm_fwd_persist_kernel<NQ, KS, true, 2>>((int)lds)) return rc;
+    if (a.data_polls) lstm_fwd_persist_kernel<NQ, KS, true, 2><<<dim3(grid), 256, lds, st>>>(a);
+    else lstm_fwd_persist_kernel<NQ, KS, false, 2><<<dim3(grid), 256, lds, st>>>(a);
+  } else if (a.data_polls) lstm_fwd_persist_kernel<NQ, KS, true><<<dim3(grid), 256, lds, st>>>(a);
   else lstm_fwd_persist_kernel<NQ, KS, false><<<dim3(grid), 256, lds, st>>>(a);
   CSN_LAUNCH_CHECK();
   return CSN_OK;
@@ -546,6 +553,9 @@
               kPersistFlagLine);
   if (a.xcd_groups)
     CSN_REQUIRE(a.nslots * a.MT <= 8 && fwd_persist_slices(a.H) <= 32, "launch_fwd_persist: groups do not fit 8 XCDs");
+  CSN_REQUIRE(a.MT * (a.half_tiles ? 32 : 64) == a.Bpad, "launch_fwd_persist: %d tiles of %d rows are not Bpad=%d", a.MT,
+              a.half_tiles ? 32 : 64, a.Bpad);
+  CSN_REQUIRE(!a.half_tiles || a.xcd_groups, "launch_fwd_persist: 32-row groups need the grouped form");
   const int nq = (a.H % 24 == 0) ? 6 : 8, ks = a.H / 128;
   if (nq == 6 && ks == 6) return launch_persist_t<6, 6>(a, st);
   if (nq == 6 && ks == 3) return launch_persist_t<6, 3>(a, st);
diff --git a/include/csn_hip.h b/include/csn_hip.h
--- a/include/csn_hip.h
+++ b/include/csn_hip.h
@@ -48,6 +48,7 @@
 size_t csn_lstm_plan_workspace_bytes(const csnLstmPlan* plan);
 int csn_lstm_plan_path(const csnLstmPlan* plan);
 int csn_lstm_plan_dgates_copies(const csnLstmPlan* plan);
+int csn_lstm_plan_half_tile_launches(const csnLstmPlan* plan, int which);
 const char* csn_lstm_plan_kernel_name(const csnLstmPlan* plan, int which);
 size_t csn_lstm_workspace_bytes(const csnLstmDesc* d, int training);
 
```
